# slyforce/MusicStyleTransfer

Measured on AMD Instinct MI355X. Metric: piano-roll frames/s (VAE train step), higher is better.
Workload: dtype bf16; 1 GPU; BASELINE configs[1]: single-track piano-roll VAE train step, T=256, pitch=128, latent=64, batch=64/GPU, bf16; encoder 256x2x8h, decoder 128x1x8h (scripts/train-vae.sh), dropout 0.2; Xavier-initialised weights; global_batch=64, seq_len=256, pitches=128, latent=64, parallelism=dp1, params=1885440

## Files before the change

### include/mst_hip.h

```cpp
#ifndef MST_HIP_H
#define MST_HIP_H

#include <stdint.h>

#ifdef __cplusplus
extern "C" {
#endif

typedef void* mst_stream_t;

enum mst_status {
  MST_OK = 0,
  MST_ERR_INVALID = -1,
  MST_ERR_LAUNCH = -2,
  MST_ERR_UNSUPPORTED = -3
};

enum mst_dtype { MST_BF16 = 0, MST_F16 = 1, MST_F32 = 2 };

enum mst_act { MST_ACT_NONE = 0, MST_ACT_RELU = 1 };

int mst_version(void);
const char* mst_last_error(void);

int mst_graph_begin(mst_stream_t stream);
int mst_graph_end(mst_stream_t stream, void** graph_exec_out);
int mst_graph_end_counted(mst_stream_t stream, void** graph_exec_out, int32_t* nodes_out, int32_t* kernel_nodes_out);
int mst_graph_launch(void* graph_exec, mst_stream_t stream);
int mst_graph_destroy(void* graph_exec);

int mst_event_create(void** ev_out);
int mst_event_record(void* ev, mst_stream_t stream);
int mst_event_sync(void* ev);
int mst_event_elapsed_ms(void* ev_start, void* ev_stop, float* ms_out);
int mst_event_destroy(void* ev);

typedef struct mst_gemm_args {
  int32_t dtype;
  int32_t c_f32;
  int64_t M, N, K;
  const void* A; int64_t lda;
  const void* B; int64_t ldb;
  void* C; int64_t ldc;
  const float* bias;
  const void* resid; int64_t ldr;
  int32_t act;
  const void* gate; int64_t ldg;
  float alpha;
  const float* rowadd; int64_t ldra; int64_t rowadd_period;
  const float* grpadd; int64_t ldga; const int32_t* grp_index;
  int64_t a_rows_per_group, a_group_stride, a_group_offset;
  int64_t c_rows_per_group, c_group_stride, c_group_offset;
  float dropout_p; uint64_t dropout_seed; uint32_t dropout_site;
  int32_t self_resid;
  const uint64_t* dropout_seed_ptr;
  int32_t a_u8;
  int32_t resid_phys;
} mst_gemm_args;

int mst_gemm_nt(const mst_gemm_args* args, mst_stream_t stream);
int mst_gemm_nt_form(const mst_gemm_args* args);

int mst_gemm_nt_pair(const mst_gemm_args* args0, const mst_gemm_args* args1, mst_stream_t stream);

typedef struct mst_bce_args {
  const uint8_t* labels;
  int64_t T;
  float label_smoothing;
  int32_t downweight;
  float* loss;
  void* probs; int64_t ldp;
  void* logits; int64_t ldl;
  float gscale;
  uint64_t* counts;
} mst_bce_args;
#define MST_ROLL_SLOTS 256
int mst_gemm_sigmoid_bce(const mst_gemm_args* args, const mst_bce_args* bce, mst_stream_t stream);

typedef struct mst_ln_args {
  int32_t mode;
  const float* gamma;
  const float* beta;
  float eps;
  void* out; int64_t ld_out;
  float* mean; float* rstd;
  const void* x; int64_t ld_x;
  float* dgamma; float* dbeta;
  int32_t mask_mode;
  float* partials;
} mst_ln_args;

int mst_gemm_nt_ln(const mst_gemm_args* args, const mst_ln_args* ln, mst_stream_t stream);
int mst_gemm_sigmoid_bce_dgrad_ln(const mst_gemm_args* args, const mst_bce_args* bce, const mst_gemm_args* dgrad,
                                  const mst_ln_args* ln, mst_stream_t stream);
int64_t mst_gemm_nt_ln_parts(int64_t M);
int mst_gemm_sigmoid_bce_form(const mst_gemm_args* args, const mst_bce_args* bce, const mst_gemm_args* dgrad, const mst_ln_args* ln,
                              int64_t* form);

int mst_ffn_ln_fwd(const mst_gemm_args* ff1, const mst_gemm_args* ff2, const mst_ln_args* ln, mst_stream_t stream);
int mst_ffn_ln_bwd(const mst_gemm_args* ff2_dgrad, const mst_gemm_args* ff1_dgrad, const mst_ln_args* ln, mst_stream_t stream);
typedef struct mst_ln_bwd_in {
  const void* dy; int64_t ld_dy;
  const void* x;  int64_t ld_x;
  const float* gamma; const float* mean; const float* rstd;
  void* dx; int64_t ld_dx;
  void* dx_masked; int64_t ld_dxm;
  float* dgamma; float* dbeta; float* partials;
  int32_t mask_mode;
  float dropout_p; uint64_t dropout_seed; const uint64_t* dropout_seed_ptr; uint32_t dropout_site;
} mst_ln_bwd_in;
int mst_ffn_ln_bwd_lead(const mst_ln_bwd_in* lead, const mst_gemm_args* ff2_dgrad, const mst_gemm_args* ff1_dgrad,
                        const mst_ln_args* ln, mst_stream_t stream);
int mst_kqv_ffn_ln_bwd(const mst_gemm_args* kqv_dgrad, const mst_ln_bwd_in* lead, const mst_gemm_args* ff2_dgrad,
                       const mst_gemm_args* ff1_dgrad, const mst_ln_args* ln, mst_stream_t stream);
int mst_kqv_ffn_ln_bwd_form(const mst_gemm_args* kqv_dgrad, const mst_gemm_args* ff2_dgrad, const mst_gemm_args* ff1_dgrad,
                            int64_t* form);
int mst_proj_ffn_ln_fwd(const mst_gemm_args* proj, const mst_ln_args* ln1, const mst_gemm_args* ff1, const mst_gemm_args* ff2,
                        const mst_ln_args* ln2, mst_stream_t stream);
int mst_dec_tail_step(const mst_gemm_args* proj, const mst_ln_args* ln1, const mst_gemm_args* ff1, const mst_gemm_args* ff2,
                      const mst_ln_args* ln3, const mst_gemm_args* out, const mst_bce_args* bce, const mst_gemm_args* out_dgrad,
                      const mst_ln_args* ln3_bwd, const mst_gemm_args* ff2_dgrad, const mst_gemm_args* ff1_dgrad,
                      const mst_ln_args* ln1_bwd, mst_stream_t stream);

typedef struct mst_partial_sum {
  const float* src; int64_t n_parts; int64_t stride; int64_t len;
  float* dst; float scale;
} mst_partial_sum;
int mst_partial_sums(const mst_partial_sum* jobs, int n, mst_stream_t stream);

typedef struct mst_wgrad_args {
  int32_t dtype;
  int64_t M, N, K;
  const void* A; int64_t lda;
  const void* B; int64_t ldb;
  float* dW; int64_t ldw;
  float* db;
  float scale;
  int64_t a_rows_per_group, a_group_stride, a_group_offset;
  int64_t b_rows_per_group, b_group_stride, b_group_offset;
  int32_t a_u8;
} mst_wgrad_args;

typedef struct mst_outer_job {
  const float* L; const void* R; int32_t r_dtype; int64_t r_stride;
  int64_t B, J, I;
  float* out; float* obias;
} mst_outer_job;
int mst_outer_jobs(const mst_outer_job* jobs, int n, mst_stream_t stream);
int mst_gemm_wgrad_batch_flush(const mst_wgrad_args* list, int n, float* scratch, int64_t scratch_bytes,
                               const mst_partial_sum* sums, int n_sums, const mst_outer_job* outers, int n_outers,
                               mst_stream_t stream);
int mst_class_table_grad(const int32_t* classes, const float* tvec, float* dcls, int64_t ld_cls, int64_t B, int64_t Dd,
                         mst_stream_t stream);
int mst_gemm_wgrad_batch_flush_cls(const mst_wgrad_args* list, int n, float* scratch, int64_t scratch_bytes,
                                   const mst_partial_sum* sums, int n_sums, const mst_outer_job* outers, int n_outers,
                                   const int32_t* cls_classes, const float* cls_tvec, float* cls_dcls, int64_t cls_ld,
                                   int64_t cls_B, int64_t cls_Dd, mst_stream_t stream);
int mst_gemm_wgrad_plan(const mst_wgrad_args* list, int n, int64_t scratch_bytes, int64_t* plan);

int mst_embed_fwd(int dtype, int64_t B, int64_t T, int64_t D,
                  const int32_t* tokens, const float* table, int64_t ldt,
                  const int32_t* classes, const float* cls_table, int64_t ldc,
// ... 310 lines not shown
```

### musicstyletransfer_amd/csrc/common.hpp

```cpp
#pragma once
#include <hip/hip_runtime.h>
#include <stdint.h>
#include <stdio.h>
#include "../../include/mst_hip.h"

namespace mst {

void set_error(const char* fmt, ...);

#define MST_CHECK_ARG(cond, ...)                 \
  do {                                           \
    if (!(cond)) {                               \
      ::mst::set_error(__VA_ARGS__);             \
      return MST_ERR_INVALID;                    \
    }                                            \
  } while (0)

#define MST_CHECK_LAUNCH(what)                                                   \
  do {                                                                           \
    hipError_t e__ = hipGetLastError();                                          \
    if (e__ != hipSuccess) {                                                     \
      ::mst::set_error("%s: %s", what, hipGetErrorString(e__));                  \
      return MST_ERR_LAUNCH;                                                     \
    }                                                                            \
  } while (0)

static inline int lds_opt_in(const void* fn, size_t lds, size_t* granted, const char* what) {
  if (lds <= *granted) return MST_OK;
  const hipError_t e = hipFuncSetAttribute(fn, hipFuncAttributeMaxDynamicSharedMemorySize, (int)lds);
  if (e != hipSuccess) { set_error("%s: LDS opt-in of %zu bytes: %s", what, lds, hipGetErrorString(e)); return MST_ERR_LAUNCH; }
  *granted = lds;
  return MST_OK;
}

static inline int64_t cdiv(int64_t a, int64_t b) { return (a + b - 1) / b; }
static inline int64_t roundup(int64_t a, int64_t b) { return cdiv(a, b) * b; }

constexpr int WAVE = 64;

typedef __attribute__((ext_vector_type(4))) float f32x4;
typedef __attribute__((ext_vector_type(16))) float f32x16;
typedef __attribute__((ext_vector_type(8))) __bf16 bf16x8;
typedef __attribute__((ext_vector_type(4))) __bf16 bf16x4;
typedef __attribute__((ext_vector_type(8))) _Float16 f16x8;
typedef __attribute__((ext_vector_type(4))) _Float16 f16x4;
typedef __attribute__((ext_vector_type(4))) short i16x4;
typedef __attribute__((ext_vector_type(8))) short i16x8;
typedef __attribute__((ext_vector_type(4))) uint32_t u32x4;
typedef __attribute__((ext_vector_type(2))) uint32_t u32x2;

template <typename T> struct Act;
template <> struct Act<__bf16> {
  typedef bf16x8 vec8;
  typedef bf16x4 vec4;
  static __device__ __forceinline__ f32x4 mfma16(vec8 a, vec8 b, f32x4 c) {
    return __builtin_amdgcn_mfma_f32_16x16x32_bf16(a, b, c, 0, 0, 0);
  }
  static __device__ __forceinline__ f32x16 mfma32(vec8 a, vec8 b, f32x16 c) {
    return __builtin_amdgcn_mfma_f32_32x32x16_bf16(a, b, c, 0, 0, 0);
  }
};
template <> struct Act<_Float16> {
  typedef f16x8 vec8;
  typedef f16x4 vec4;
  static __device__ __forceinline__ f32x4 mfma16(vec8 a, vec8 b, f32x4 c) {
    return __builtin_amdgcn_mfma_f32_16x16x32_f16(a, b, c, 0, 0, 0);
  }
  static __device__ __forceinline__ f32x16 mfma32(vec8 a, vec8 b, f32x16 c) {
    return __builtin_amdgcn_mfma_f32_32x32x16_f16(a, b, c, 0, 0, 0);
  }
};

template <typename T> __device__ __forceinline__ float to_f32(T x) { return (float)x; }
template <typename T> __device__ __forceinline__ T from_f32(float x) { return (T)x; }

union Pack8 {
  u32x4 u;
  uint16_t h[8];
};

template <typename T> __device__ __forceinline__ float bits_to_f32(uint16_t b) {
  T t;
  __builtin_memcpy(&t, &b, 2);
  return (float)t;
}
template <typename T> __device__ __forceinline__ uint16_t f32_to_bits(float f) {
  T t = (T)f;
  uint16_t b;
  __builtin_memcpy(&b, &t, 2);
  return b;
}

template <typename T> __device__ __forceinline__ u32x4 expand_u8x8(u32x2 raw) {
  Pack8 p;
#pragma unroll
  for (int e = 0; e < 8; ++e) p.h[e] = f32_to_bits<T>((float)((raw[e >> 2] >> (8 * (e & 3))) & 0xFFu));
  return p.u;
}

template <int CTRL> __device__ __forceinline__ float dpp_mov(float v) {
  return __builtin_bit_cast(float, __builtin_amdgcn_update_dpp(0, __builtin_bit_cast(int, v), CTRL, 0xF, 0xF, true));
}
__device__ __forceinline__ float lane_xor16(float v) {
  return __builtin_bit_cast(float, __builtin_amdgcn_ds_swizzle(__builtin_bit_cast(int, v), 0x401F));
}
template <int LANES> __device__ __forceinline__ float group_sum(float v) {
  static_assert(LANES == 4 || LANES == 8 || LANES == 16 || LANES == 32 || LANES == 64, "group size");
  v += dpp_mov<0xB1>(v);
  v += dpp_mov<0x4E>(v);
  if constexpr (LANES >= 8) v += dpp_mov<0x141>(v);
  if constexpr (LANES >= 16) v += dpp_mov<0x140>(v);
  if constexpr (LANES >= 32) v += lane_xor16(v);
  if constexpr (LANES >= 64) v += __shfl_xor(v, 32, 64);
  return v;
}
template <int LANES> __device__ __forceinline__ float group_max(float v) {
  v = fmaxf(v, dpp_mov<0xB1>(v));
  v = fmaxf(v, dpp_mov<0x4E>(v));
  if constexpr (LANES >= 8) v = fmaxf(v, dpp_mov<0x141>(v));
  if constexpr (LANES >= 16) v = fmaxf(v, dpp_mov<0x140>(v));
  if constexpr (LANES >= 32) v = fmaxf(v, lane_xor16(v));
  if constexpr (LANES >= 64) v = fmaxf(v, __shfl_xor(v, 32, 64));
  return v;
}
__device__ __forceinline__ float wave_sum(float v) { return group_sum<64>(v); }
__device__ __forceinline__ float wave_max(float v) { return group_max<64>(v); }

__device__ __forceinline__ int64_t xcd_chunk(int64_t bid, int64_t n) {
  const int64_t q = n / 8, r = n % 8, x = bid % 8, y = bid / 8;
  return (x < r ? x * (q + 1) : r * (q + 1) + (x - r) * q) + y;
}

__device__ __forceinline__ int64_t remap_row(int64_t m, int64_t rpg, int64_t stride, int64_t off) {
  return rpg > 0 ? (m / rpg) * stride + off + (m % rpg) : m;
}

__host__ __device__ __forceinline__ uint32_t dropout_hash(uint64_t seed, uint32_t site, uint64_t idx) {
  uint64_t x = seed ^ (0x9E3779B97F4A7C15ull * (uint64_t)(site + 1)) ^ (idx * 0xD1B54A32D192ED03ull);
  x ^= x >> 32; x *= 0xD6E8FEB86659FD93ull;
  x ^= x >> 32; x *= 0xD6E8FEB86659FD93ull;
  x ^= x >> 32;
  return (uint32_t)x;
}
__host__ __device__ __forceinline__ uint32_t dropout_thr(float p) { return (uint32_t)(p * 65536.0f); }
__host__ __device__ __forceinline__ float dropout_inv_keep(float p) {
// ... 75 lines not shown
```

### musicstyletransfer_amd/csrc/dec_tail.hip

```cpp
#include "ffn_ln.hpp"
#include "gemm_bce.hpp"
#include "gemm_checks.hpp"

namespace mst {

template <typename T>
__device__ __forceinline__ void tile128_load_w(const mst_gemm_args& g, u32x4 (&rw)[2][2]) {
  const T* __restrict__ W = reinterpret_cast<const T*>(g.B);
#pragma unroll
  for (int s = 0; s < 2; ++s)
#pragma unroll
    for (int i = 0; i < 2; ++i) {
      const int c = threadIdx.x + i * 512, row = c / 8, ch = c % 8;
      rw[s][i] = *reinterpret_cast<const u32x4*>(W + (int64_t)row * g.ldb + s * 64 + ch * 8);
    }
}
template <typename T>
__device__ __forceinline__ void tile128_gemm(unsigned char* smem, const T* sA, const u32x4 (&rw)[2][2], f32x4 (&acc)[2][2]) {
  constexpr int BN = 128, LDA = BN + 8, CHUNKS = 8, WTM = 32, WTN = 32, TM = 2, TN = 2, WGN = 4;
  typedef typename Act<T>::vec8 vec8;
  u32x4* sB = reinterpret_cast<u32x4*>(smem);
  const int tid = threadIdx.x, lane = tid & 63, wave = tid >> 6;
  const int wm = wave / WGN, wn = wave % WGN, frow = lane & 15, fq = lane >> 4;
#pragma unroll
  for (int s = 0; s < 2; ++s)
#pragma unroll
    for (int i = 0; i < 2; ++i) {
      const int c = tid + i * 512, row = c / CHUNKS, ch = c % CHUNKS;
      sB[s * BN * CHUNKS + row * CHUNKS + (ch ^ (row & 7))] = rw[s][i];
    }
#pragma unroll
  for (int j = 0; j < TN; ++j)
#pragma unroll
    for (int i = 0; i < TM; ++i) acc[j][i] = f32x4{0.f, 0.f, 0.f, 0.f};
  __syncthreads();
#pragma unroll
  for (int s = 0; s < 2; ++s) {
    const u32x4* cB = sB + s * BN * CHUNKS;
#pragma unroll
    for (int ks = 0; ks < 2; ++ks) {
      vec8 xf[TM], wf[TN];
      const int kc = ks * 4 + fq;
#pragma unroll
      for (int i = 0; i < TM; ++i)
        xf[i] = __builtin_bit_cast(vec8, *reinterpret_cast<const u32x4*>(sA + (wm * WTM + i * 16 + frow) * LDA + s * 64 + kc * 8));
#pragma unroll
      for (int j = 0; j < TN; ++j) {
        const int row = wn * WTN + j * 16 + frow;
        wf[j] = __builtin_bit_cast(vec8, cB[row * CHUNKS + (kc ^ (row & 7))]);
      }
#pragma unroll
      for (int j = 0; j < TN; ++j)
#pragma unroll
        for (int i = 0; i < TM; ++i) acc[j][i] = Act<T>::mfma16(wf[j], xf[i], acc[j][i]);
    }
  }
  __syncthreads();
}

constexpr size_t DEC_TAIL_F = 512;
constexpr size_t DEC_TAIL_BODY_LDS = (size_t)2 * 128 * 64 * 2 + (size_t)2 * 64 * (128 + 8) * 2 + DEC_TAIL_F * 4 + (size_t)6 * 128 * 4;
constexpr size_t DEC_TAIL_LDS = DEC_TAIL_BODY_LDS + ((size_t)128 + 3 * 128 + DEC_TAIL_F + 3 * 128) * 4;
static_assert(DEC_TAIL_LDS <= (size_t)48 * 1024 + (size_t)2 * (64 + 128) * 64 * 2 + (size_t)3 * 128 * 4, "no more LDS than the loss launch takes");

template <typename T, bool CNT>
__global__ __launch_bounds__(512) void dec_tail_kernel(mst_gemm_args proj, mst_ln_args ln1, mst_gemm_args ff1, mst_gemm_args ff2, mst_ln_args ln3,
                                                       mst_gemm_args out, mst_bce_args bce, mst_gemm_args odg, mst_ln_args ln3b,
                                                       mst_gemm_args f2d, mst_gemm_args f1d, mst_ln_args ln1b) {
  constexpr int BM = 64, BN = 128, WGM = 2, WGN = 4, LDA = BN + 8, F = (int)DEC_TAIL_F;
  extern __shared__ __attribute__((aligned(16))) unsigned char smem[];
  __shared__ __attribute__((aligned(16))) float red[bce_red_words(CNT)];
  T* sX = reinterpret_cast<T*>(smem + (size_t)2 * BN * 64 * 2 + (size_t)BM * LDA * 2);
  float* sBiasO = reinterpret_cast<float*>(smem + DEC_TAIL_BODY_LDS);
  float* sPar3 = sBiasO + BN;
  float* sPar4 = sPar3 + 3 * BN;
  const int tid = threadIdx.x;
  for (int i = tid; i < BN; i += 512) {
    sBiasO[i] = out.bias ? out.bias[i] : 0.f;
    sPar3[i] = odg.bias ? odg.bias[i] : 0.f;
    sPar3[BN + i] = ln3b.gamma[i];
    sPar3[2 * BN + i] = 0.f;
    sPar4[F + i] = f1d.bias ? f1d.bias[i] : 0.f;
    sPar4[F + BN + i] = ln1b.gamma[i];
    sPar4[F + 2 * BN + i] = 0.f;
  }
  for (int i = tid; i < F; i += 512) sPar4[i] = f2d.bias ? f2d.bias[i] : 0.f;
  const int64_t m0 = xcd_chunk(blockIdx.x, gridDim.x) * BM;
  const mst_ln_bwd_in no_lead = {};
  u32x4 rw[2][2];
  f32x4 acc[2][2];
  ffn_ln_body<T, BN, WGM, WGN, 1, false, true, true, false, true, false>(smem, ff1, ff2, ln3, no_lead, proj, ln1, nullptr,
                                                                         [&] { tile128_load_w<T>(out, rw); });
  __syncthreads();
  tile128_gemm<T>(smem, sX, rw, acc);
  tile128_load_w<T>(odg, rw);
  {
    float bias8[8];
#pragma unroll
    for (int e = 0; e < 8; ++e) bias8[e] = sBiasO[(tid % (BN / 8)) * 8 + e];
    bce_tile_finish<T, BN, 2, CNT>(out, bce, smem, red, reinterpret_cast<u32x4*>(sX), acc, m0, 0, bias8);
  }
  __syncthreads();
  tile128_gemm<T>(smem, sX, rw, acc);
  gemm_epilogue_ln<T, BM, BN, WGM, WGN, 2>(odg, ln3b, smem, acc, m0, nullptr, 0, sX, LDA, sPar3);
  __syncthreads();
  mst_gemm_args no_gemm = {};
  const mst_ln_args no_ln = {};
  ffn_ln_body<T, BN, WGM, WGN, 2, false, true, false, true, false, true>(smem, f2d, f1d, ln1b, no_lead, no_gemm, no_ln, sPar4, [] {});
}

template <typename T, bool CNT>
static int launch_dec_tail(const mst_gemm_args& proj, const mst_ln_args& ln1, const mst_gemm_args& ff1, const mst_gemm_args& ff2,
                           const mst_ln_args& ln3, const mst_gemm_args& out, const mst_bce_args& bce, const mst_gemm_args& odg,
                           const mst_ln_args& ln3b, const mst_gemm_args& f2d, const mst_gemm_args& f1d, const mst_ln_args& ln1b, hipStream_t s) {
  static size_t granted = 64 * 1024;
  if (const int rc = lds_opt_in(reinterpret_cast<const void*>(&dec_tail_kernel<T, CNT>), DEC_TAIL_LDS, &granted, "dec_tail_kernel")) return rc;
  hipLaunchKernelGGL((dec_tail_kernel<T, CNT>), dim3((unsigned)(out.M / 64)), dim3(512), DEC_TAIL_LDS, s, proj, ln1, ff1, ff2, ln3, out, bce, odg,
                     ln3b, f2d, f1d, ln1b);
  MST_CHECK_LAUNCH("dec_tail_kernel");
  return MST_OK;
}

}

using namespace mst;

extern "C" int mst_dec_tail_step(const mst_gemm_args* proj, const mst_ln_args* ln1, const mst_gemm_args* ff1, const mst_gemm_args* ff2,
                                 const mst_ln_args* ln3, const mst_gemm_args* out, const mst_bce_args* bce, const mst_gemm_args* out_dgrad,
                                 const mst_ln_args* ln3_bwd, const mst_gemm_args* ff2_dgrad, const mst_gemm_args* ff1_dgrad,
                                 const mst_ln_args* ln1_bwd, mst_stream_t stream) {
  const char* who = "mst_dec_tail_step";
  MST_CHECK_ARG(proj && ln1 && ff1 && ff2 && ln3 && out && bce && out_dgrad && ln3_bwd && ff2_dgrad && ff1_dgrad && ln1_bwd, "%s: null args", who);
  const mst_gemm_args &o = *out, &g = *out_dgrad, &d2 = *ff2_dgrad;
  const int64_t T = bce->T;
  MST_CHECK_ARG(ff2->N == 128 && ff1->K == 128 && proj->N == 128 && g.N == 128 && ff1_dgrad->N == 128,
                "%s: the model width must be 128 (got %lld)", who, (long long)ff2->N);
  MST_CHECK_ARG(ff1->N == 512 && d2.N == 512, "%s: the hidden width must be 512 (got %lld)", who, (long long)ff1->N);
  MST_CHECK_ARG(o.N == 128 && o.K == 128 && g.K == 128, "%s: the output layer must have 128 pitches (got %lld)", who, (long long)o.N);
  MST_CHECK_ARG(T > 0 && T % 64 == 0, "%s: T must be a multiple of 64 (got %lld)", who, (long long)T);
  MST_CHECK_ARG(o.M > 0 && o.M % 64 == 0 && o.M % T == 0 && ff1->M == o.M && ff2->M == o.M && proj->M == o.M && g.M == o.M && d2.M == o.M &&
                ff1_dgrad->M == o.M, "%s: every part works on the same whole 64-row tiles (M %lld)", who, (long long)o.M);
  auto groups = [&](int64_t rpg, int64_t stride, int64_t off) { return rpg == T && stride == T + 1 && off == 1; };
  MST_CHECK_ARG(groups(ff1->a_rows_per_group, ff1->a_group_stride, ff1->a_group_offset) &&
                groups(o.a_rows_per_group, o.a_group_stride, o.a_group_offset) &&
                groups(g.c_rows_per_group, g.c_group_stride, g.c_group_offset) &&
                groups(d2.a_rows_per_group, d2.a_group_stride, d2.a_group_offset) && g.a_rows_per_group <= 0,
                "%s: row groups must be (T, T + 1, 1) on all three parts", who);
  MST_CHECK_ARG(ln3_bwd->mode == 2 && ln3_bwd->mask_mode == 2, "%s: the LayerNorm-3 backward takes mask mode 2 (got %d)", who, (int)ln3_bwd->mask_mode);
  MST_CHECK_ARG(o.A == ln3->out && o.lda == ln3->ld_out, "%s: the output layer's A operand must be LayerNorm-3's output", who);
  MST_CHECK_ARG(o.C && g.A == o.C && g.lda == o.ldc, "%s: the output dgrad's A operand must be the logit gradient", who);
  MST_CHECK_ARG(d2.A == g.C && d2.lda == g.ldc, "%s: the A operand of the FF2 dgrad must be the output dgrad's dX_out", who);
  MST_CHECK_ARG(proj->dtype == o.dtype && g.dtype == o.dtype && d2.dtype == o.dtype && ff1->dtype == o.dtype && !g.a_u8,
                "%s: every part must share one activation dtype", who);
  int rc = check_ffn_ln(who, ff1, ff2, ln3, 1, nullptr, proj, ln1);
  if (rc == MST_OK) rc = check_gemm_bce(o, *bce);
  if (rc == MST_OK) rc = check_gemm_ln(g, *ln3_bwd);
  if (rc == MST_OK) rc = check_ffn_ln(who, ff2_dgrad, ff1_dgrad, ln1_bwd, 2);
  if (rc) return rc;
  hipStream_t s = (hipStream_t)stream;
  return dispatch_act(o.dtype, [&](auto tag) -> int {
    typedef decltype(tag) T_;
    if (bce->counts) return launch_dec_tail<T_, true>(*proj, *ln1, *ff1, *ff2, *ln3, o, *bce, g, *ln3_bwd, d2, *ff1_dgrad, *ln1_bwd, s);
    return launch_dec_tail<T_, false>(*proj, *ln1, *ff1, *ff2, *ln3, o, *bce, g, *ln3_bwd, d2, *ff1_dgrad, *ln1_bwd, s);
  });
}
```

### musicstyletransfer_amd/csrc/ffn_ln.hip

```cpp
#include "ffn_ln.hpp"
#include "gemm_checks.hpp"

namespace mst {

template <typename T, int BN, int WGM, int WGN, int MODE, bool LEAD, bool FULL, bool EXTRA = false>
__global__ __launch_bounds__(WGM * WGN * 64) void ffn_ln_kernel(mst_gemm_args g1, mst_gemm_args g2, mst_ln_args ln, mst_ln_bwd_in lead,
                                                                mst_gemm_args gx, mst_ln_args lnx) {
  extern __shared__ __attribute__((aligned(16))) unsigned char smem[];
  ffn_ln_body<T, BN, WGM, WGN, MODE, LEAD, FULL, EXTRA>(smem, g1, g2, ln, lead, gx, lnx, nullptr, [] {});
}

template <typename T, int BN>
static int launch_ffn_ln(const mst_gemm_args& g1, const mst_gemm_args& g2, const mst_ln_args& ln, const mst_ln_bwd_in* lead, hipStream_t s,
                         const mst_gemm_args* gx = nullptr, const mst_ln_args* lnx = nullptr) {
  constexpr int BM = 64;
  const int ex = gx ? 1 : 0;
  const size_t lds_loop = (size_t)2 * BN * 64 * 2 + (size_t)2 * BM * (BN + 8) * 2 + (size_t)g1.N * 4 + (size_t)6 * BN * 4;
  const size_t lds_epi = (size_t)BM * (BN + 4) * 4;
  const size_t lds = lds_loop > lds_epi ? lds_loop : lds_epi;
  const int full = g1.M % BM == 0 ? 1 : 0;
  const int mi = ex ? (ln.mode == 2 ? 8 : 6) + full : (lead ? 2 : (ln.mode == 2 ? 1 : 0)) * 2 + full;
  typedef void (*kern_t)(mst_gemm_args, mst_gemm_args, mst_ln_args, mst_ln_bwd_in, mst_gemm_args, mst_ln_args);
  const kern_t fns[10] = {&ffn_ln_kernel<T, BN, 2, 4, 1, false, false>, &ffn_ln_kernel<T, BN, 2, 4, 1, false, true>,
                         &ffn_ln_kernel<T, BN, 2, 4, 2, false, false>, &ffn_ln_kernel<T, BN, 2, 4, 2, false, true>,
                         &ffn_ln_kernel<T, BN, 2, 4, 2, true, false>, &ffn_ln_kernel<T, BN, 2, 4, 2, true, true>,
                         &ffn_ln_kernel<T, BN, 2, 4, 1, false, false, true>, &ffn_ln_kernel<T, BN, 2, 4, 1, false, true, true>,
                          &ffn_ln_kernel<T, BN, 2, 4, 2, true, false, true>, &ffn_ln_kernel<T, BN, 2, 4, 2, true, true, true>};
  static size_t granted[10] = {64 * 1024, 64 * 1024, 64 * 1024, 64 * 1024, 64 * 1024, 64 * 1024, 64 * 1024, 64 * 1024, 64 * 1024, 64 * 1024};
  if (const int rc = lds_opt_in(reinterpret_cast<const void*>(fns[mi]), lds, &granted[mi], "ffn_ln_kernel")) return rc;
  const mst_ln_bwd_in none = {};
  const mst_gemm_args no_gemm = {};
  const mst_ln_args no_ln = {};
  hipLaunchKernelGGL(fns[mi], dim3((unsigned)cdiv(g1.M, BM)), dim3(512), lds, s, g1, g2, ln, lead ? *lead : none,
                     gx ? *gx : no_gemm, lnx ? *lnx : no_ln);
  MST_CHECK_LAUNCH("ffn_ln_kernel");
  return MST_OK;
}

int check_ffn_ln(const char* who, const mst_gemm_args* first, const mst_gemm_args* second, const mst_ln_args* ln, int mode,
                 const mst_ln_bwd_in* lead, const mst_gemm_args* extra, const mst_ln_args* extra_ln) {
  MST_CHECK_ARG(first != nullptr && second != nullptr && ln != nullptr, "%s: null args", who);
  const mst_gemm_args& a = *first;
  const mst_gemm_args& b = *second;
  const mst_ln_args& l = *ln;
  int rc = check_gemm_common(a);
  if (rc) return rc;
  rc = check_gemm_common(b);
  if (rc) return rc;
  MST_CHECK_ARG(a.dtype == b.dtype && a.M == b.M, "%s: the two GEMMs must share dtype and M", who);
  MST_CHECK_ARG((b.N == 256 || b.N == 128) && a.K == b.N, "%s: the model width (first K = second N) must be 128 or 256 (got %lld, %lld)", who,
                (long long)a.K, (long long)b.N);
  MST_CHECK_ARG(a.N == b.K && a.N % b.N == 0, "%s: the hidden width (first N = second K) must be a multiple of the model width", who);
  MST_CHECK_ARG(b.A == a.C && b.lda == a.ldc, "%s: the second GEMM's A operand must be the first one's output (it is consumed on chip)", who);
  MST_CHECK_ARG(!a.c_f32 && !b.c_f32 && !b.gate && !a.rowadd && !b.rowadd && !a.grpadd && !b.grpadd && !a.resid && !a.self_resid &&
                b.act == MST_ACT_NONE && a.c_rows_per_group <= 0 && b.a_rows_per_group <= 0 && b.c_rows_per_group <= 0,
                "%s: fp32 outputs, row-indexed adds, row remaps, a gate or activation on the second GEMM and a residual on the first are not supported", who);
  MST_CHECK_ARG(a.a_rows_per_group <= 0 || (a.a_rows_per_group % 64 == 0 && a.M % a.a_rows_per_group == 0 && a.a_group_offset >= 0 &&
                                            a.a_group_stride >= a.a_rows_per_group + a.a_group_offset && a.M < (1ll << 31)),
                "%s: row groups must be whole 64-row tiles (rows per group %lld, stride %lld, offset %lld, M %lld)", who,
                (long long)a.a_rows_per_group, (long long)a.a_group_stride, (long long)a.a_group_offset, (long long)a.M);
  MST_CHECK_ARG(a.lda % 8 == 0 && a.ldc % 8 == 0 && a.ldc >= a.N && b.ldc % 8 == 0 && b.ldc >= b.N, "%s: leading dimensions must be multiples of 8", who);
  MST_CHECK_ARG((uint64_t)a.N * (uint64_t)a.ldb < (1ull << 32) && (uint64_t)b.N * (uint64_t)b.ldb < (1ull << 32), "%s: weight matrices too large", who);
  MST_CHECK_ARG(!b.resid || (b.ldr % 8 == 0 && b.ldr >= b.N && (uintptr_t)b.resid % 16 == 0), "%s: bad residual layout", who);
  MST_CHECK_ARG(!a.bias || (uintptr_t)a.bias % 16 == 0, "%s: the first GEMM's bias must be 16-byte aligned", who);
  MST_CHECK_ARG(a.dropout_p == 0.f || a.N % 4 == 0, "%s: dropout needs widths that are multiples of 4", who);
  MST_CHECK_ARG(l.mode == mode && l.gamma && l.mean && l.rstd, "%s: LayerNorm arguments of the wrong form", who);
  if (mode == 1) {
    MST_CHECK_ARG(!a.gate, "%s: a gate belongs to the backward form", who);
    MST_CHECK_ARG(l.beta && l.out && l.ld_out % 8 == 0 && l.ld_out >= b.N && (uintptr_t)l.out % 16 == 0,
                  "%s: the LayerNorm arguments are those of mst_gemm_nt_ln's forward form", who);
  } else {
    MST_CHECK_ARG(a.gate && a.ldg % 8 == 0 && a.ldg >= a.N && (uintptr_t)a.gate % 16 == 0, "%s: the first GEMM needs the forward activation as its gate", who);
    MST_CHECK_ARG(a.act == MST_ACT_NONE && a.dropout_p == 0.f && !b.self_resid, "%s: activation / dropout / self_resid belong to the forward form", who);
    MST_CHECK_ARG(l.x && l.ld_x % 8 == 0 && (uintptr_t)l.x % 16 == 0 && (l.partials || (l.dgamma && l.dbeta)) && (uintptr_t)l.partials % 16 == 0,
                  "%s: backward needs x and dgamma + dbeta (or partials)", who);
    MST_CHECK_ARG(l.mask_mode >= 0 && l.mask_mode <= 2 &&
                  (l.mask_mode != 1 || (l.out && l.ld_out % 8 == 0 && l.ld_out >= b.N && (uintptr_t)l.out % 16 == 0)),
                  "%s: mask_mode must be 0, 1 (with out) or 2", who);
  }
  if (lead) {
    const mst_ln_bwd_in& q = *lead;
    MST_CHECK_ARG(mode == 2, "%s: a leading LayerNorm belongs to the backward form", who);
    const bool dy_on_chip = extra != nullptr;
    MST_CHECK_ARG((q.dy || dy_on_chip) && q.x && q.gamma && q.mean && q.rstd && q.dx && (q.partials || (q.dgamma && q.dbeta)),
                  "%s: leading LayerNorm: null pointer", who);
    MST_CHECK_ARG((dy_on_chip || (q.ld_dy % 8 == 0 && q.ld_dy >= b.N)) && q.ld_x % 8 == 0 && q.ld_dx % 8 == 0 && q.ld_x >= b.N && q.ld_dx >= b.N &&
                  ((uintptr_t)q.dy | (uintptr_t)q.x | (uintptr_t)q.dx | (uintptr_t)q.partials) % 16 == 0, "%s: leading LayerNorm: bad layout", who);
    MST_CHECK_ARG(q.mask_mode == 0 || (q.mask_mode == 1 && q.dx_masked && q.ld_dxm % 8 == 0 && q.ld_dxm >= b.N && (uintptr_t)q.dx_masked % 16 == 0),
                  "%s: leading LayerNorm: mask_mode must be 0 or 1 (with dx_masked)", who);
    MST_CHECK_ARG(q.dropout_p >= 0.f && q.dropout_p < 1.f, "%s: leading LayerNorm: dropout_p must be in [0,1)", who);
    const void* tile = q.mask_mode == 1 ? q.dx_masked : q.dx;
    const int64_t tile_ld = q.mask_mode == 1 ? q.ld_dxm : q.ld_dx;
    MST_CHECK_ARG(a.A == tile && a.lda == tile_ld, "%s: the first GEMM's A operand must be the leading LayerNorm's (masked) output", who);
  }
  if (extra && mode == 2) {
  } else if (extra) {
    const mst_gemm_args& x = *extra;
    rc = check_gemm_common(x);
    if (rc) return rc;
    MST_CHECK_ARG(x.dtype == a.dtype && x.M == a.M && x.N == b.N && x.K == b.N, "%s: the extra GEMM is width x width on the same rows", who);
    MST_CHECK_ARG(!x.c_f32 && !x.gate && !x.rowadd && !x.grpadd && x.act == MST_ACT_NONE && x.a_rows_per_group <= 0 && x.c_rows_per_group <= 0 &&
                  x.ldc % 8 == 0 && x.ldc >= x.N && (uint64_t)x.N * (uint64_t)x.ldb < (1ull << 32),
                  "%s: the extra GEMM takes no gate, activation, row-indexed add or row remap", who);
    MST_CHECK_ARG(mode == 1 && extra_ln != nullptr, "%s: the projection (with its LayerNorm) rides in front of the forward form", who);
    const mst_ln_args& q = *extra_ln;
    MST_CHECK_ARG(q.mode == 1 && q.gamma && q.beta && q.mean && q.rstd && q.out == a.A && q.ld_out == a.lda,
                  "%s: the leading LayerNorm's output must be the first GEMM's A operand", who);
    MST_CHECK_ARG(!x.resid || (x.ldr % 8 == 0 && x.ldr >= x.N && (uintptr_t)x.resid % 16 == 0), "%s: bad residual layout", who);
  }
  return MST_OK;
}

}

using namespace mst;

static int ffn_ln_impl(const char* who, const mst_gemm_args* first, const mst_gemm_args* second, const mst_ln_args* ln, int mode,
                       mst_stream_t stream, const mst_ln_bwd_in* lead = nullptr, const mst_gemm_args* extra = nullptr,
                       const mst_ln_args* extra_ln = nullptr) {
  const int rc = check_ffn_ln(who, first, second, ln, mode, lead, extra, extra_ln);
  if (rc) return rc;
  const mst_gemm_args &a = *first, &b = *second;
  const mst_ln_args& l = *ln;
  hipStream_t s = (hipStream_t)stream;
  return dispatch_act(a.dtype, [&](auto tag) -> int {
    typedef decltype(tag) T;
    if (b.N == 256) return launch_ffn_ln<T, 256>(a, b, l, lead, s, extra, extra_ln);
    return launch_ffn_ln<T, 128>(a, b, l, lead, s, extra, extra_ln);
  });
}

extern "C" int mst_proj_ffn_ln_fwd(const mst_gemm_args* proj, const mst_ln_args* ln1, const mst_gemm_args* ff1, const mst_gemm_args* ff2,
                                   const mst_ln_args* ln2, mst_stream_t stream) {
  MST_CHECK_ARG(proj != nullptr && ln1 != nullptr, "mst_proj_ffn_ln_fwd: null args");
  return ffn_ln_impl("mst_proj_ffn_ln_fwd", ff1, ff2, ln2, 1, stream, nullptr, proj, ln1);
}

extern "C" int mst_ffn_ln_bwd_lead(const mst_ln_bwd_in* lead, const mst_gemm_args* ff2_dgrad, const mst_gemm_args* ff1_dgrad,
                                   const mst_ln_args* ln, mst_stream_t stream) {
  MST_CHECK_ARG(lead != nullptr, "mst_ffn_ln_bwd_lead: null args");
  return ffn_ln_impl("mst_ffn_ln_bwd_lead", ff2_dgrad, ff1_dgrad, ln, 2, stream, lead);
}

static int kqv_head_form(const mst_gemm_args& x, const mst_gemm_args& a, const mst_gemm_args& b) {
  const bool shape = (b.N == 256 || b.N == 128) && x.N == b.N && x.K == 3 * b.N && x.M == a.M && x.dtype == a.dtype;
  const bool plain = !x.c_f32 && !x.a_u8 && !x.bias && !x.gate && !x.rowadd && !x.grpadd && x.act == MST_ACT_NONE && x.alpha == 1.f &&
                     x.dropout_p == 0.f && !x.self_resid && x.a_rows_per_group <= 0 && x.c_rows_per_group <= 0 && a.a_rows_per_group <= 0;
  const bool layout = x.resid && ((uintptr_t)x.A | (uintptr_t)x.B | (uintptr_t)x.resid | (uintptr_t)x.C) % 16 == 0 && x.lda % 8 == 0 &&
                      x.lda >= x.K && x.ldb % 8 == 0 && x.ldb >= x.K && x.ldr % 8 == 0 && x.ldr >= x.N &&
                      (!x.C || (x.ldc % 8 == 0 && x.ldc >= x.N)) && (uint64_t)x.N * (uint64_t)x.ldb < (1ull << 32);
  return shape && plain && layout ? 1 : 0;
}

static int check_kqv_head_call(const char* who, const mst_gemm_args* head, const mst_gemm_args* ff2_dgrad, const mst_gemm_args* ff1_dgrad) {
  MST_CHECK_ARG(head != nullptr && ff2_dgrad != nullptr && ff1_dgrad != nullptr, "%s: null args", who);
  MST_CHECK_ARG(head->M > 0 && head->N > 0 && head->K > 0, "%s: the head's M,N,K must be positive (got %lld,%lld,%lld)", who,
                (long long)head->M, (long long)head->N, (long long)head->K);
  MST_CHECK_ARG(head->A && head->B, "%s: the head's A and B operands are missing", who);
  MST_CHECK_ARG(head->M == ff2_dgrad->M && head->N == ff1_dgrad->N, "%s: the head's result is the block's incoming gradient: M x width (got %lld x %lld)",
                who, (long long)head->M, (long long)head->N);
  return MST_OK;
}

extern "C" int mst_kqv_ffn_ln_bwd_form(const mst_gemm_args* kqv_dgrad, const mst_gemm_args* ff2_dgrad, const mst_gemm_args* ff1_dgrad,
                                       int64_t* form) {
  MST_CHECK_ARG(form != nullptr, "mst_kqv_ffn_ln_bwd_form: null form");
  if (const int rc = check_kqv_head_call("mst_kqv_ffn_ln_bwd_form", kqv_dgrad, ff2_dgrad, ff1_dgrad)) return rc;
  form[0] = kqv_head_form(*kqv_dgrad, *ff2_dgrad, *ff1_dgrad);
  return MST_OK;
}

extern "C" int mst_kqv_ffn_ln_bwd(const mst_gemm_args* kqv_dgrad, const mst_ln_bwd_in* lead, const mst_gemm_args* ff2_dgrad,
                                  const mst_gemm_args* ff1_dgrad, const mst_ln_args* ln, mst_stream_t stream) {
  if (const int rc = check_kqv_head_call("mst_kqv_ffn_ln_bwd", kqv_dgrad, ff2_dgrad, ff1_dgrad)) return rc;
  MST_CHECK_ARG(lead != nullptr, "mst_kqv_ffn_ln_bwd: null args");
  MST_CHECK_ARG(lead->dy == kqv_dgrad->C && (!lead->dy || lead->ld_dy == kqv_dgrad->ldc),
                "mst_kqv_ffn_ln_bwd: lead->dy is the head's C (both NULL: the gradient is not stored)");
  if (kqv_head_form(*kqv_dgrad, *ff2_dgrad, *ff1_dgrad))
    return ffn_ln_impl("mst_kqv_ffn_ln_bwd", ff2_dgrad, ff1_dgrad, ln, 2, stream, lead, kqv_dgrad);
  MST_CHECK_ARG(kqv_dgrad->C != nullptr, "mst_kqv_ffn_ln_bwd: this shape runs the GEMM launch first and needs the head's C");
  if (const int rc = check_ffn_ln("mst_kqv_ffn_ln_bwd", ff2_dgrad, ff1_dgrad, ln, 2, lead)) return rc;
  if (const int f = mst_gemm_nt_form(kqv_dgrad); f < 0) return f;
  if (const int rc = mst_gemm_nt(kqv_dgrad, stream)) return rc;
  return ffn_ln_impl("mst_kqv_ffn_ln_bwd", ff2_dgrad, ff1_dgrad, ln, 2, stream, lead);
}

extern "C" int mst_ffn_ln_fwd(const mst_gemm_args* ff1, const mst_gemm_args* ff2, const mst_ln_args* ln, mst_stream_t stream) {
  return ffn_ln_impl("mst_ffn_ln_fwd", ff1, ff2, ln, 1, stream);
}
extern "C" int mst_ffn_ln_bwd(const mst_gemm_args* ff2_dgrad, const mst_gemm_args* ff1_dgrad, const mst_ln_args* ln, mst_stream_t stream) {
  return ffn_ln_impl("mst_ffn_ln_bwd", ff2_dgrad, ff1_dgrad, ln, 2, stream);
}

#ifdef MST_FFN_STAMPS
extern "C" int mst_debug_ffn_stamps(uint64_t* host_out) {
  return hipMemcpyFromSymbol(host_out, HIP_SYMBOL(mst::g_ffn_stamps), sizeof(uint64_t) * (8 + 48 * 4)) == hipSuccess ? 0 : -1;
}
#endif
```

### musicstyletransfer_amd/csrc/ffn_ln.hpp

```cpp
#pragma once
#include <type_traits>
#include "gemm_ln.hpp"

namespace mst {

template <typename T, int BN, int WGM, int WGN, int MODE, bool LEAD, bool FULL, bool EXTRA, bool X_IN_LDS = false, bool KEEP_OUT = false,
          bool PAR_READY = false, typename Hook>
__device__ __forceinline__ void ffn_ln_body(unsigned char* smem, mst_gemm_args g1, mst_gemm_args g2, const mst_ln_args ln,
                                            const mst_ln_bwd_in lead, mst_gemm_args gx, const mst_ln_args lnx, float* par,
                                            Hook&& before_epilogue) {
  constexpr bool HEAD = EXTRA, FHEAD = EXTRA && MODE == 1, BHEAD = EXTRA && MODE == 2;
  static_assert(!(X_IN_LDS && (LEAD || EXTRA)), "a tile left in LDS is the block's own input");
  static_assert(!BHEAD || LEAD, "the backward form's head computes the gradient tile of the leading LayerNorm backward");
  constexpr int BM = 64, BK = 64, CHUNKS = BK / 8;
  constexpr int NT = WGM * WGN * 64;
  constexpr int WTM = BM / WGM, WTN = BN / WGN, TM = WTM / 16, TN = WTN / 16;
  constexpr int B_CH = BN * CHUNKS / NT;
  constexpr int LDA = BN + 8;
  constexpr int KST = BN / BK;
  constexpr int XST = BHEAD ? 3 * KST : KST;
  static_assert(BN * CHUNKS % NT == 0 && (BM * BN / 8) % NT == 0, "tile/threads mismatch");
  typedef typename Act<T>::vec8 vec8;
  u32x4* sB = reinterpret_cast<u32x4*>(smem);
  T* sH = reinterpret_cast<T*>(smem + (size_t)2 * BN * BK * 2);
  T* sX = sH + BM * LDA;
  float* sBias1 = PAR_READY ? par : reinterpret_cast<float*>(sX + BM * LDA);
  float* sPar = sBias1 + g1.N;
  const int tid = threadIdx.x, lane = tid & 63, wave = tid >> 6;
  const int wm = wave / WGN, wn = wave % WGN, frow = lane & 15, fq = lane >> 4;
  int64_t m0 = xcd_chunk(blockIdx.x, gridDim.x) * BM;
  if (g1.a_rows_per_group > 0) {
    const uint32_t grp = (uint32_t)m0 / (uint32_t)g1.a_rows_per_group;
    m0 += (int64_t)grp * (g1.a_group_stride - g1.a_rows_per_group) + g1.a_group_offset;
    g1.M = g2.M = gx.M = (g1.M / g1.a_rows_per_group) * g1.a_group_stride;
  }
  const int64_t F = g1.N;
  FFN_STAMP(0); FFN_RT(190);
  const int64_t Mg = FULL ? (int64_t)1 << 62 : g1.M;
  if constexpr (!PAR_READY)
  for (int i = tid * 4; i < (int)F; i += NT * 4)
    *reinterpret_cast<f32x4*>(sBias1 + i) = g1.bias ? *reinterpret_cast<const f32x4*>(g1.bias + i) : f32x4{0.f, 0.f, 0.f, 0.f};
  const uint64_t seed2 = g2.dropout_seed ^ ((g2.dropout_p > 0.f && g2.dropout_seed_ptr) ? g2.dropout_seed_ptr[0] : 0ull);
  const uint64_t seedx = FHEAD ? gx.dropout_seed ^ ((gx.dropout_p > 0.f && gx.dropout_seed_ptr) ? gx.dropout_seed_ptr[0] : 0ull) : 0ull;
  if constexpr (!PAR_READY)
  for (int i = tid; i < BN; i += NT) {
    sPar[i] = g2.bias ? g2.bias[i] : 0.f;
    sPar[BN + i] = ln.gamma[i];
    sPar[2 * BN + i] = (MODE == 1) ? ln.beta[i] : 0.f;
    if constexpr (FHEAD) {
      sPar[3 * BN + i] = gx.bias ? gx.bias[i] : 0.f;
      sPar[4 * BN + i] = lnx.gamma[i];
      sPar[5 * BN + i] = lnx.beta[i];
    }
  }
  const int n_chunks = (int)(F / BN);
  const int rot = (int)((blockIdx.x / 8) % (unsigned)n_chunks);
  auto phys = [&](int c) { const int pc = c + rot; return pc >= n_chunks ? pc - n_chunks : pc; };
  const T* __restrict__ W1 = reinterpret_cast<const T*>(g1.B);
  const T* __restrict__ W2 = reinterpret_cast<const T*>(g2.B);
  const T* __restrict__ WX = reinterpret_cast<const T*>(gx.B);

  uint32_t off1[B_CH], off2[B_CH], offx[B_CH];
  int b_lds[B_CH];
#pragma unroll
  for (int i = 0; i < B_CH; ++i) {
    const int c = tid + i * NT;
    const int row = c / CHUNKS, ch = c % CHUNKS;
    off1[i] = (uint32_t)row * (uint32_t)g1.ldb + (uint32_t)ch * 8u;
    off2[i] = (uint32_t)row * (uint32_t)g2.ldb + (uint32_t)ch * 8u;
    offx[i] = EXTRA ? (uint32_t)row * (uint32_t)gx.ldb + (uint32_t)ch * 8u : 0u;
    b_lds[i] = row * CHUNKS + (ch ^ (row & 7));
  }
  constexpr int SPC = 2 * KST;
  constexpr int RING = BN >= 256 ? 4 : 2, AHEAD = RING - 1;
  static_assert(SPC % RING == 0, "ring slots must repeat per chunk");
  u32x4 ring[RING][B_CH];
  auto load_stage = [&](int c, int s, u32x4 (&rb)[B_CH]) {
    if (HEAD && c < 0) {
      const T* base = WX + s * BK;
#pragma unroll
      for (int i = 0; i < B_CH; ++i) rb[i] = *reinterpret_cast<const u32x4*>(base + offx[i]);
    } else if (s < KST) {
      const T* base = W1 + (int64_t)phys(c) * BN * g1.ldb + s * BK;
#pragma unroll
      for (int i = 0; i < B_CH; ++i) rb[i] = *reinterpret_cast<const u32x4*>(base + off1[i]);
    } else {
      const T* base = W2 + (int64_t)phys(c) * BN + (s - KST) * BK;
#pragma unroll
      for (int i = 0; i < B_CH; ++i) rb[i] = *reinterpret_cast<const u32x4*>(base + off2[i]);
    }
  };
  auto load_piece = [&](int c, int s, u32x4 (&rb)[B_CH], auto ic) {
    constexpr int i = decltype(ic)::value;
    const T* base;
    uint32_t off;
    if (HEAD && c < 0) { base = WX + s * BK; off = offx[i]; }
    else if (s < KST) { base = W1 + (int64_t)phys(c) * BN * g1.ldb + s * BK; off = off1[i]; }
    else { base = W2 + (int64_t)phys(c) * BN + (s - KST) * BK; off = off2[i]; }
    rb[i] = *reinterpret_cast<const u32x4*>(base + off);
  };
  auto store_stage = [&](int buf, const u32x4 (&rb)[B_CH]) {
#pragma unroll
    for (int i = 0; i < B_CH; ++i) sB[buf * BN * CHUNKS + b_lds[i]] = rb[i];
  };
  {
    auto pro = [&](auto jc) {
      constexpr int j = decltype(jc)::value;
      if constexpr (HEAD) {
        static_assert(!HEAD || AHEAD <= XST, "the head GEMM's stages cover the prologue");
        if (j < AHEAD) load_stage(-1, j, ring[j % RING]);
      } else {
        if (j < AHEAD && (j < SPC || n_chunks > 1)) load_stage(j / SPC, j % SPC, ring[j % RING]);
      }
    };
    pro(std::integral_constant<int, 0>()); pro(std::integral_constant<int, 1>()); pro(std::integral_constant<int, 2>());
    pro(std::integral_constant<int, 3>()); pro(std::integral_constant<int, 4>()); pro(std::integral_constant<int, 5>());
    pro(std::integral_constant<int, 6>());
    static_assert(AHEAD <= 7, "the prologue list covers seven stages");
  }
  constexpr int L_CPR = BN / 8, L_RSTEP = NT / L_CPR, L_ITERS = BM / L_RSTEP;
  const int lnc = (tid % L_CPR) * 8, lrow0 = tid / L_CPR;
  uint32_t ldkey = 0u, ldthr = 0u;
  float linv_keep = 1.f, gam8[8], dg8[8], db8[8];
  u32x4 dyv[L_ITERS], xv[L_ITERS];
  float mean_r[L_ITERS], rstd_r[L_ITERS];
  u32x4 ha2[L_ITERS], hres[L_ITERS];
  auto lead_loads = [&] {
    constexpr int RSTEP = L_RSTEP, ITERS = L_ITERS;
    const int nc = lnc, row0 = lrow0;
    const bool has_drop = lead.dropout_p > 0.f && lead.mask_mode == 1;
    const uint64_t dseed = lead.dropout_seed ^ ((has_drop && lead.dropout_seed_ptr) ? lead.dropout_seed_ptr[0] : 0ull);
    ldkey = dropout_key(dseed, lead.dropout_site); ldthr = dropout_thr(lead.dropout_p);
    linv_keep = dropout_inv_keep(lead.dropout_p);
#pragma unroll
    for (int e = 0; e < 8; ++e) { gam8[e] = lead.gamma[nc + e]; dg8[e] = 0.f; db8[e] = 0.f; }
#pragma unroll
    for (int it = 0; it < ITERS; ++it) {
      const int64_t m = m0 + row0 + it * RSTEP;
      dyv[it] = u32x4{0u, 0u, 0u, 0u}; xv[it] = dyv[it]; mean_r[it] = 0.f; rstd_r[it] = 0.f;
      if (m < Mg) {
        if constexpr (!BHEAD) dyv[it] = *reinterpret_cast<const u32x4*>(reinterpret_cast<const T*>(lead.dy) + m * lead.ld_dy + nc);
        xv[it] = *reinterpret_cast<const u32x4*>(reinterpret_cast<const T*>(lead.x) + m * lead.ld_x + nc);
        mean_r[it] = lead.mean[m];
        rstd_r[it] = lead.rstd[m];
      }
    }
  };
  auto lead_rows = [&] {
    constexpr int CPR = L_CPR, RSTEP = L_RSTEP, ITERS = L_ITERS;
    const int nc = lnc, row0 = lrow0;
    const float inv_n = 1.f / (float)BN;
    const bool has_drop = lead.dropout_p > 0.f && lead.mask_mode == 1;
    const uint32_t dkey = ldkey, dthr = ldthr;
    const float inv_keep = linv_keep;
    if constexpr (BHEAD) {
#pragma unroll
      for (int it = 0; it < ITERS; ++it) {
        const int row = row0 + it * RSTEP;
        const int64_t m = m0 + row;
        if (m < Mg) {
          dyv[it] = *reinterpret_cast<const u32x4*>(sX + row * LDA + nc);
          if (gx.C) *reinterpret_cast<u32x4*>(reinterpret_cast<T*>(gx.C) + m * gx.ldc + nc) = dyv[it];
        }
      }
    }
#pragma unroll
    for (int it = 0; it < ITERS; ++it) {
      const int row = row0 + it * RSTEP;
      const int64_t m = m0 + row;
      Pack8 db, xb;
      db.u = dyv[it]; xb.u = xv[it];
      float xh[8], g[8], s1 = 0.f, s2 = 0.f;
#pragma unroll
      for (int e = 0; e < 8; ++e) {
        const float d = bits_to_f32<T>(db.h[e]);
        xh[e] = (bits_to_f32<T>(xb.h[e]) - mean_r[it]) * rstd_r[it];
        g[e] = d * gam8[e];
        s1 += g[e];
        s2 += g[e] * xh[e];
        dg8[e] += d * xh[e];
        db8[e] += d;
      }
      s1 = row_sum<CPR>(s1) * inv_n;
      s2 = row_sum<CPR>(s2) * inv_n;
      uint32_t keep8 = 0xFFu;
      if (has_drop) {
        const uint64_t w = (uint64_t)(m * BN + nc) >> 2;
        keep8 = dropout_keep4k(dkey, w, dthr) | (dropout_keep4k(dkey, w + 1, dthr) << 4);
      }
      Pack8 ob, mb;
#pragma unroll
      for (int e = 0; e < 8; ++e) {
        const float o = rstd_r[it] * (g[e] - s1 - xh[e] * s2);
        const float k = has_drop ? (((keep8 >> e) & 1u) ? inv_keep : 0.f) : 1.f;
        ob.h[e] = f32_to_bits<T>(o);
        mb.h[e] = f32_to_bits<T>(o * k);
      }
      if (m < Mg) {
        *reinterpret_cast<u32x4*>(reinterpret_cast<T*>(lead.dx) + m * lead.ld_dx + nc) = ob.u;
        if (lead.mask_mode == 1) *reinterpret_cast<u32x4*>(reinterpret_cast<T*>(lead.dx_masked) + m * lead.ld_dxm + nc) = mb.u;
      }
      *reinterpret_cast<u32x4*>(sX + row * LDA + nc) = (m < Mg) ? (lead.mask_mode == 1 ? mb.u : ob.u) : u32x4{0u, 0u, 0u, 0u};
    }
    float* red = reinterpret_cast<float*>(smem);
    static_assert((size_t)2 * RSTEP * BN * 4 <= (size_t)2 * BN * BK * 2, "reduction scratch must fit the weight stages");
#pragma unroll
    for (int e = 0; e < 8; ++e) {
      red[row0 * BN + nc + e] = dg8[e];
      red[(RSTEP + row0) * BN + nc + e] = db8[e];
    }
    __syncthreads();
    for (int c = tid; c < 2 * BN; c += NT) {
      const int which = c / BN, col = c % BN;
      float sm = 0.f;
      for (int r = 0; r < RSTEP; ++r) sm += red[(which * RSTEP + r) * BN + col];
      if (lead.partials) lead.partials[(int64_t)blockIdx.x * 2 * BN + c] = sm;
      else atomicAdd((which ? lead.dbeta : lead.dgamma) + col, sm);
    }
    __syncthreads();
  };
  if constexpr (BHEAD) {
    constexpr int RSTEP = L_RSTEP, ITERS = L_ITERS;
    const T* HA = reinterpret_cast<const T*>(gx.A);
    const T* HR = reinterpret_cast<const T*>(gx.resid);
    u32x4 ha0[ITERS], ha1[ITERS];
#pragma unroll
    for (int it = 0; it < ITERS; ++it) {
      const int64_t m = m0 + lrow0 + it * RSTEP;
      ha0[it] = u32x4{0u, 0u, 0u, 0u}; ha1[it] = ha0[it]; ha2[it] = ha0[it]; hres[it] = ha0[it];
      if (m < Mg) {
        const T* ap = HA + m * gx.lda + lnc;
        ha0[it] = *reinterpret_cast<const u32x4*>(ap);
        ha1[it] = *reinterpret_cast<const u32x4*>(ap + BN);
        ha2[it] = *reinterpret_cast<const u32x4*>(ap + 2 * BN);
        hres[it] = *reinterpret_cast<const u32x4*>(HR + m * gx.ldr + lnc);
      }
    }
    lead_loads();
#pragma unroll
    for (int it = 0; it < ITERS; ++it) {
      const int row = lrow0 + it * RSTEP;
      *reinterpret_cast<u32x4*>(sX + row * LDA + lnc) = ha0[it];
      *reinterpret_cast<u32x4*>(sH + row * LDA + lnc) = ha1[it];
    }
  } else if constexpr (LEAD) {
    lead_loads();
    lead_rows();
  } else if constexpr (!X_IN_LDS)
  {
    const T* X = reinterpret_cast<const T*>(HEAD ? gx.A : g1.A);
    const int64_t ldx = HEAD ? gx.lda : g1.lda;
    constexpr int CPR = BN / 8;
// ... 66 lines not shown
        if constexpr (t < XST) load_stage(cx, t, ring[t % RING]);
        else if constexpr (HEAD) load_stage(0, t - XST, ring[t % RING]);
        mma_stage(acc1, (((s / KST) & 1) ? sH : sX) + (s % KST) * BK, s & 1, ring[s % RING], no_hook);
        if constexpr (s + 1 < XST) store_stage((s + 1) & 1, ring[(s + 1) % RING]);
        __syncthreads();
        if constexpr (BHEAD && (s == KST - 1 || s == 2 * KST - 1)) {
#pragma unroll
          for (int it = 0; it < L_ITERS; ++it)
            *reinterpret_cast<u32x4*>((s == KST - 1 ? sX : sH) + (lrow0 + it * L_RSTEP) * LDA + lnc) = s == KST - 1 ? ha2[it] : hres[it];
        }
      }
    };
    static_assert(!EXTRA || (XST <= 12 && XST % RING == 0 && XST % 2 == 0), "the extra GEMM stage list / ring slots");
    xstage(std::integral_constant<int, 0>()); xstage(std::integral_constant<int, 1>());
    xstage(std::integral_constant<int, 2>()); xstage(std::integral_constant<int, 3>());
    xstage(std::integral_constant<int, 4>()); xstage(std::integral_constant<int, 5>());
    xstage(std::integral_constant<int, 6>()); xstage(std::integral_constant<int, 7>());
    xstage(std::integral_constant<int, 8>()); xstage(std::integral_constant<int, 9>());
    xstage(std::integral_constant<int, 10>()); xstage(std::integral_constant<int, 11>());
  };
  if constexpr (BHEAD) {
    extra_gemm(-1);
#pragma unroll
    for (int j = 0; j < TN; ++j)
#pragma unroll
      for (int i = 0; i < TM; ++i) {
        const int row = wm * WTM + i * 16 + frow, n = wn * WTN + j * 16 + fq * 4;
        const u32x2 rb = *reinterpret_cast<const u32x2*>(sH + row * LDA + n);
        uint16_t hb[4];
#pragma unroll
        for (int e = 0; e < 4; ++e)
          hb[e] = f32_to_bits<T>(acc1[j][i][e] + bits_to_f32<T>((uint16_t)(rb[e >> 1] >> ((e & 1) * 16))));
        *reinterpret_cast<u32x2*>(sX + row * LDA + n) =
            u32x2{(uint32_t)hb[0] | ((uint32_t)hb[1] << 16), (uint32_t)hb[2] | ((uint32_t)hb[3] << 16)};
      }
    __syncthreads();
    lead_rows();
  }
  if constexpr (FHEAD) {
    extra_gemm(-1);
    gemm_epilogue_ln<T, BM, BN, WGM, WGN, 1>(gx, lnx, smem, acc1, m0, nullptr, 0, sX, LDA, sPar + 3 * BN, &seedx);
    __syncthreads();
  }
  store_stage(0, ring[0]);
  __syncthreads();
  FFN_STAMP(1);
  for (int c = 0; c < n_chunks; ++c) {
    const int pc = phys(c);
#pragma unroll
    for (int j = 0; j < TN; ++j)
#pragma unroll
      for (int i = 0; i < TM; ++i) acc1[j][i] = f32x4{0.f, 0.f, 0.f, 0.f};
    constexpr int OUT_CH = BM * (BN / 8) / NT;
    u32x4 gv[OUT_CH];
    if constexpr (MODE == 2) {
      const T* G = reinterpret_cast<const T*>(g1.gate);
#pragma unroll
      for (int i = 0; i < OUT_CH; ++i) {
        const int cc = tid + i * NT, row = cc / (BN / 8), ch = cc % (BN / 8);
        gv[i] = u32x4{0u, 0u, 0u, 0u};
        if (m0 + row < Mg) gv[i] = *reinterpret_cast<const u32x4*>(G + (m0 + row) * g1.ldg + (int64_t)pc * BN + ch * 8);
      }
    }
    auto stage = [&](auto sc) {
      constexpr int s = decltype(sc)::value;
      if constexpr (s < SPC) {
        constexpr bool IL = BN >= 256 && B_CH <= 2 * TN;
        constexpr int t = s + AHEAD;
        const int tc = t < SPC ? c : (c + 1 < n_chunks ? c + 1 : c);
        const bool more = s + 1 < SPC || c + 1 < n_chunks;
        auto piece = [&](auto kc) {
          constexpr int k = decltype(kc)::value;
          if constexpr (IL && k < B_CH) {
            __builtin_amdgcn_sched_barrier(0);
            load_piece(tc, t % SPC, ring[t % RING], kc);
            if (more) sB[((s + 1) & 1) * BN * CHUNKS + b_lds[k]] = ring[(s + 1) % RING][k];
            __builtin_amdgcn_sched_barrier(0);
          }
        };
        if constexpr (!IL) load_stage(tc, t % SPC, ring[t % RING]);
        FFN_STAMP(8 + (c * SPC + s) * 4);
        if constexpr (s < KST) mma_stage(acc1, sX + s * BK, s & 1, ring[s % RING], piece);
        else mma_stage(acc2, sH + (s - KST) * BK, s & 1, ring[s % RING], piece);
        FFN_STAMP(8 + (c * SPC + s) * 4 + 1);
        if constexpr (s == KST - 1) {
          auto chunk_epilogue = [&](auto step_form) {
            constexpr bool STEP = decltype(step_form)::value;
            const uint32_t cmul = ((uint32_t)pc * (BN / 2) + (uint32_t)((wn * WTN + fq * 4) / 2)) * DROPOUT_MUL;
#pragma unroll
            for (int j = 0; j < TN; ++j) {
              const int n = wn * WTN + j * 16 + fq * 4;
              const int64_t col = (int64_t)pc * BN + n;
              const f32x4 b4 = *reinterpret_cast<const f32x4*>(sBias1 + col);
#pragma unroll
              for (int i = 0; i < TM; ++i) {
                const int row = wm * WTM + i * 16 + frow;
                float tv[4];
                if constexpr (STEP) {
#pragma unroll
                  for (int e = 0; e < 4; ++e) tv[e] = fmaxf(acc1[j][i][e] + b4[e], 0.f);
                  dropout_apply4_pre(dkey1, rowmul[i] + cmul + (uint32_t)(j * 8) * DROPOUT_MUL, dthr1, inv_keep1, tv);
                } else {
#pragma unroll
                  for (int e = 0; e < 4; ++e) {
                    tv[e] = (acc1[j][i][e] + b4[e]) * g1.alpha;
                    if (relu1) tv[e] = fmaxf(tv[e], 0.f);
                  }
                  if (drop1) dropout_apply4(dkey1, (uint64_t)((m0 + row) * F + col) >> 2, dthr1, inv_keep1, tv);
                }
                uint16_t hb[4];
#pragma unroll
                for (int e = 0; e < 4; ++e) hb[e] = f32_to_bits<T>(tv[e]);
                *reinterpret_cast<u32x2*>(sH + row * LDA + n) =
                    u32x2{(uint32_t)hb[0] | ((uint32_t)hb[1] << 16), (uint32_t)hb[2] | ((uint32_t)hb[3] << 16)};
              }
            }
          };
          if (step_form1) chunk_epilogue(std::true_type()); else chunk_epilogue(std::false_type());
        }
        if (!IL && more) store_stage((s + 1) & 1, ring[(s + 1) % RING]);
        FFN_STAMP(8 + (c * SPC + s) * 4 + 2);
        __syncthreads();
        FFN_STAMP(8 + (c * SPC + s) * 4 + 3);
        if constexpr (s == KST - 1) {
          constexpr int CPR = BN / 8;
#pragma unroll
          for (int i = 0; i < BM * CPR / NT; ++i) {
            const int cc = tid + i * NT, row = cc / CPR, ch = cc % CPR;
            u32x4 v = *reinterpret_cast<const u32x4*>(sH + row * LDA + ch * 8);
            if constexpr (MODE == 2) {
              Pack8 pv, pg;
              pv.u = v; pg.u = gv[i];
#pragma unroll
              for (int e = 0; e < 8; ++e)
                if (!(bits_to_f32<T>(pg.h[e]) > 0.f)) pv.h[e] = 0;
              v = pv.u;
              *reinterpret_cast<u32x4*>(sH + row * LDA + ch * 8) = v;
            }
            if (m0 + row < Mg) *reinterpret_cast<u32x4*>(Aout + (m0 + row) * g1.ldc + (int64_t)pc * BN + ch * 8) = v;
          }
          if constexpr (MODE == 2) __syncthreads();
        }
      }
    };
    static_assert(SPC <= 8, "the stage list below covers eight stages per chunk");
    stage(std::integral_constant<int, 0>()); stage(std::integral_constant<int, 1>());
    stage(std::integral_constant<int, 2>()); stage(std::integral_constant<int, 3>());
    stage(std::integral_constant<int, 4>()); stage(std::integral_constant<int, 5>());
    stage(std::integral_constant<int, 6>()); stage(std::integral_constant<int, 7>());
  }
  const bool resid_is_x = g2.resid == g1.A && g2.ldr == g1.lda;
  FFN_STAMP(2);
  before_epilogue();
  gemm_epilogue_ln<T, BM, BN, WGM, WGN, MODE>(g2, ln, smem, acc2, m0, resid_is_x ? sX : nullptr, LDA, KEEP_OUT ? sX : nullptr, KEEP_OUT ? LDA : 0,
                                              sPar, &seed2);
  FFN_STAMP(3); FFN_RT(191);
}

}
```

### musicstyletransfer_amd/csrc/gemm_bce.hip

```cpp
#include "gemm_bce.hpp"
#include "gemm_ln.hpp"
#include "gemm_checks.hpp"

namespace mst {

template <typename T, int BN, bool CNT>
__global__ __launch_bounds__(512) void gemm_bce_kernel(mst_gemm_args a, mst_bce_args q) {
  extern __shared__ __attribute__((aligned(16))) unsigned char smem[];
  __shared__ __attribute__((aligned(16))) float red[bce_red_words(CNT)];
  gemm_bce_tile<T, BN, false, CNT>(a, q, smem, red, nullptr);
}

template <typename T, bool CNT>
__global__ __launch_bounds__(512) void gemm_bce_dgrad_ln_kernel(mst_gemm_args a, mst_bce_args q, mst_gemm_args g2, mst_ln_args l) {
  constexpr int BM = 64, BN = 128, WGM = 2, WGN = 4;
  constexpr size_t OFF2 = 48 * 1024, END2 = OFF2 + (size_t)2 * (BM + BN) * 64 * 2;
  extern __shared__ __attribute__((aligned(16))) unsigned char smem[];
  __shared__ __attribute__((aligned(16))) float red[bce_red_words(CNT)];
  float* sPar = reinterpret_cast<float*>(smem + END2);
  for (int i = threadIdx.x; i < BN; i += 512) {
    sPar[i] = g2.bias ? g2.bias[i] : 0.f;
    sPar[BN + i] = l.gamma[i];
    sPar[2 * BN + i] = 0.f;
  }
  gemm_bce_tile<T, BN, true, CNT>(a, q, smem, red, reinterpret_cast<u32x4*>(smem + OFF2));
  __syncthreads();
  f32x4 acc[(BN / WGN) / 16][(BM / WGM) / 16];
  int64_t m0, n0;
  gemm_mainloop<T, BM, BN, WGM, WGN, 64, true, false, true>(g2, smem + OFF2, acc, m0, n0);
  gemm_epilogue_ln<T, BM, BN, WGM, WGN, 2>(g2, l, smem, acc, m0, nullptr, 0, nullptr, 0, sPar);
}

template <typename T, bool CNT>
static int launch_gemm_bce_dgrad_ln(const mst_gemm_args& a, const mst_bce_args& q, const mst_gemm_args& g2, const mst_ln_args& l, hipStream_t s) {
  const size_t lds = (size_t)48 * 1024 + (size_t)2 * (64 + 128) * 64 * 2 + (size_t)3 * 128 * 4;
  static size_t granted = 64 * 1024;
  if (const int rc = lds_opt_in(reinterpret_cast<const void*>(&gemm_bce_dgrad_ln_kernel<T, CNT>), lds, &granted, "gemm_bce_dgrad_ln_kernel")) return rc;
  hipLaunchKernelGGL((gemm_bce_dgrad_ln_kernel<T, CNT>), dim3((unsigned)cdiv(a.M, 64)), dim3(512), lds, s, a, q, g2, l);
  MST_CHECK_LAUNCH("gemm_bce_dgrad_ln_kernel");
  return MST_OK;
}

template <typename T, int BN, bool CNT>
static int launch_gemm_bce(const mst_gemm_args& a, const mst_bce_args& q, hipStream_t s) {
  const size_t lds_loop = (size_t)2 * (64 + BN) * 64 * 2, lds_epi = (size_t)64 * (BN + 4) * 4;
  const size_t lds = lds_loop > lds_epi ? lds_loop : lds_epi;
  static size_t granted = 64 * 1024;
  if (const int rc = lds_opt_in(reinterpret_cast<const void*>(&gemm_bce_kernel<T, BN, CNT>), lds, &granted, "gemm_bce_kernel")) return rc;
  hipLaunchKernelGGL((gemm_bce_kernel<T, BN, CNT>), dim3((unsigned)(cdiv(a.M, 64) * (a.N / BN))), dim3(512), lds, s, a, q);
  MST_CHECK_LAUNCH("gemm_bce_kernel");
  return MST_OK;
}

int check_gemm_bce(const mst_gemm_args& a, const mst_bce_args& q) {
  MST_CHECK_ARG(a.M > 0 && a.K > 0 && a.K % 8 == 0 && a.lda % 8 == 0 && a.ldb % 8 == 0 && a.A && a.B,
                "mst_gemm_sigmoid_bce: bad GEMM operands");
  MST_CHECK_ARG(((uintptr_t)a.A % 16 == 0) && ((uintptr_t)a.B % 16 == 0), "mst_gemm_sigmoid_bce: operands must be 16-byte aligned");
  MST_CHECK_ARG(a.N == 128 || (a.N > 0 && a.N % 256 == 0), "mst_gemm_sigmoid_bce: the row of pitches must be 128 or a multiple of 256 wide (got %lld): use "
                "mst_gemm_nt + mst_sigmoid_bce for other widths", (long long)a.N);
  MST_CHECK_ARG(a.N <= 256 || !q.downweight, "mst_gemm_sigmoid_bce: the label down-weighting counts a sample's positives in every workgroup — rows wider than "
                "one tile (256) take mst_gemm_nt + mst_sigmoid_bce");
  MST_CHECK_ARG(q.T > 0 && q.T % 64 == 0 && a.M % q.T == 0, "mst_gemm_sigmoid_bce: T must be a multiple of 64 and divide M (a tile holds one sample's rows)");
  MST_CHECK_ARG(!a.c_f32 && !a.resid && !a.gate && !a.rowadd && !a.grpadd && a.act == MST_ACT_NONE && a.dropout_p == 0.f && !a.self_resid &&
                a.c_rows_per_group <= 0 && !a.a_u8, "mst_gemm_sigmoid_bce: only bias, alpha and an A row remap are supported");
  MST_CHECK_ARG(q.labels && q.loss && (uintptr_t)q.labels % 8 == 0, "mst_gemm_sigmoid_bce: labels / loss missing or labels not 8-byte aligned");
  MST_CHECK_ARG(!a.C || (a.ldc % 8 == 0 && a.ldc >= a.N && (uintptr_t)a.C % 16 == 0), "mst_gemm_sigmoid_bce: bad dlogits layout");
  MST_CHECK_ARG(!q.probs || (q.ldp % 8 == 0 && q.ldp >= a.N && (uintptr_t)q.probs % 16 == 0), "mst_gemm_sigmoid_bce: bad probs layout");
  MST_CHECK_ARG(!q.logits || (q.ldl % 8 == 0 && q.ldl >= a.N && (uintptr_t)q.logits % 16 == 0), "mst_gemm_sigmoid_bce: bad logits layout");
  MST_CHECK_ARG((uintptr_t)q.counts % 16 == 0, "mst_gemm_sigmoid_bce: counts must be 16-byte aligned");
  return MST_OK;
}

static bool bce_dgrad_ln_one_launch(const mst_gemm_args& a, const mst_gemm_args& g2, const mst_ln_args& l) {
  return a.N == 128 && g2.N == 128 && g2.K == 128 && g2.M == a.M && a.M % 64 == 0 && l.mode == 2 && a.C && g2.A == a.C &&
         g2.lda == a.ldc && g2.dtype == a.dtype && g2.a_rows_per_group <= 0 && !g2.a_u8;
}

}

using namespace mst;

extern "C" int mst_gemm_sigmoid_bce_form(const mst_gemm_args* args, const mst_bce_args* bce, const mst_gemm_args* dgrad,
                                         const mst_ln_args* ln, int64_t* form) {
  MST_CHECK_ARG(form != nullptr, "mst_gemm_sigmoid_bce_form: null form");
  const bool pair = dgrad != nullptr || ln != nullptr;
  if (pair) MST_CHECK_ARG(args != nullptr && bce != nullptr && dgrad != nullptr && ln != nullptr, "mst_gemm_sigmoid_bce_dgrad_ln: null args");
  else MST_CHECK_ARG(args != nullptr && bce != nullptr, "mst_gemm_sigmoid_bce: null args");
  int rc = check_gemm_bce(*args, *bce);
  if (rc == MST_OK && pair) rc = check_gemm_ln(*dgrad, *ln);
  if (rc) return rc;
  return dispatch_act(args->dtype, [&](auto) -> int {
    const int64_t BN = args->N % 256 == 0 ? 256 : 128;
    form[0] = BN;
    form[1] = args->N / BN;
    form[2] = !pair ? 0 : bce_dgrad_ln_one_launch(*args, *dgrad, *ln) ? 1 : 2;
    return MST_OK;
  });
}

extern "C" int mst_gemm_sigmoid_bce(const mst_gemm_args* args, const mst_bce_args* bce, mst_stream_t stream) {
  MST_CHECK_ARG(args != nullptr && bce != nullptr, "mst_gemm_sigmoid_bce: null args");
  const mst_gemm_args& a = *args;
  const mst_bce_args& q = *bce;
  int rc = check_gemm_bce(a, q);
  if (rc) return rc;
  hipStream_t s = (hipStream_t)stream;
  return dispatch_act(a.dtype, [&](auto tag) -> int {
    typedef decltype(tag) T;
    if (q.counts) return a.N % 256 == 0 ? launch_gemm_bce<T, 256, true>(a, q, s) : launch_gemm_bce<T, 128, true>(a, q, s);
    return a.N % 256 == 0 ? launch_gemm_bce<T, 256, false>(a, q, s) : launch_gemm_bce<T, 128, false>(a, q, s);
  });
}

extern "C" int mst_gemm_sigmoid_bce_dgrad_ln(const mst_gemm_args* args, const mst_bce_args* bce, const mst_gemm_args* dgrad,
                                             const mst_ln_args* ln, mst_stream_t stream) {
  MST_CHECK_ARG(args != nullptr && bce != nullptr && dgrad != nullptr && ln != nullptr, "mst_gemm_sigmoid_bce_dgrad_ln: null args");
// ... 17 lines not shown
```

### musicstyletransfer_amd/csrc/gemm_checks.hpp

```cpp
#pragma once
#include "common.hpp"

namespace mst {

int check_gemm_common(const mst_gemm_args& a);
int check_gemm_ln(const mst_gemm_args& a, const mst_ln_args& l);
int check_gemm_bce(const mst_gemm_args& a, const mst_bce_args& q);
int check_ffn_ln(const char* who, const mst_gemm_args* first, const mst_gemm_args* second, const mst_ln_args* ln, int mode,
                 const mst_ln_bwd_in* lead = nullptr, const mst_gemm_args* extra = nullptr, const mst_ln_args* extra_ln = nullptr);

}
```

### musicstyletransfer_amd/csrc/gemm_ln.hpp

```cpp
#pragma once
#include <math.h>
#include "common.hpp"
#include "gemm_tile.hpp"

namespace mst {

#ifdef MST_FFN_STAMPS
static __device__ uint64_t g_ffn_stamps[8 + 48 * 4];
#define FFN_STAMP(slot) do { if (blockIdx.x == 64 && threadIdx.x == 0 && (slot) < 8 + 48 * 4) g_ffn_stamps[slot] = __builtin_amdgcn_s_memtime(); } while (0)
#define FFN_RT(slot) do { if (blockIdx.x == 64 && threadIdx.x == 0) g_ffn_stamps[slot] = __builtin_amdgcn_s_memrealtime(); } while (0)
#else
#define FFN_STAMP(slot) do { } while (0)
#define FFN_RT(slot) do { } while (0)
#endif

template <int LANES>
__device__ __forceinline__ float row_sum(float v) { return group_sum<LANES>(v); }

template <typename T, int BM, int BN, int WGM, int WGN, int MODE>
__device__ __forceinline__ void gemm_epilogue_ln(const mst_gemm_args& a, const mst_ln_args& l, unsigned char* smem,
                                                 f32x4 (&acc)[(BN / WGN) / 16][(BM / WGM) / 16], int64_t m0,
                                                 const T* lds_resid = nullptr, int lds_resid_ld = 0,
                                                 T* lds_out = nullptr, int lds_out_ld = 0, const float* lds_par = nullptr,
                                                 const uint64_t* dseed_pre = nullptr ) {
  constexpr int NT = WGM * WGN * 64;
  constexpr int WTM = BM / WGM, WTN = BN / WGN;
  constexpr int TM = WTM / 16, TN = WTN / 16;
  constexpr int LDS_F = BN + 4, CPR = BN / 8, RSTEP = NT / CPR, ITERS = BM / RSTEP;
  static_assert(CPR == 32 || CPR == 16, "a row must be a 32- or 16-lane group");
  static_assert(BM % RSTEP == 0, "rows per thread must be whole");
  const int tid = threadIdx.x, lane = tid & 63, wave = tid >> 6;
  const int wm = wave / WGN, wn = wave % WGN;
  const int frow = lane & 15, fq = lane >> 4;
  float* sF = reinterpret_cast<float*>(smem);
#pragma unroll
  for (int i = 0; i < TM; ++i)
#pragma unroll
    for (int j = 0; j < TN; ++j)
      *reinterpret_cast<f32x4*>(sF + (wm * WTM + i * 16 + frow) * LDS_F + wn * WTN + j * 16 + fq * 4) = acc[j][i];
  __syncthreads();
  FFN_STAMP(5);

  const int ch = tid % CPR, nc = ch * 8, row0 = tid / CPR;
  const float inv_n = 1.f / (float)BN;
  const float inv_keep = dropout_inv_keep(a.dropout_p);
  const bool has_drop = a.dropout_p > 0.f;
  const uint64_t dseed = dseed_pre ? *dseed_pre : a.dropout_seed ^ ((has_drop && a.dropout_seed_ptr) ? a.dropout_seed_ptr[0] : 0ull);
  const uint32_t dkey = dropout_key(dseed, a.dropout_site), dthr = dropout_thr(a.dropout_p);
  const T* resid = reinterpret_cast<const T*>(a.resid);
  float bias8[8], gam8[8], bet8[8];
#pragma unroll
  for (int e = 0; e < 8; ++e) {
    if (lds_par) {
      bias8[e] = lds_par[nc + e];
      gam8[e] = lds_par[BN + nc + e];
      bet8[e] = (MODE == 1) ? lds_par[2 * BN + nc + e] : 0.f;
    } else {
      bias8[e] = a.bias ? a.bias[nc + e] : 0.f;
      gam8[e] = l.gamma[nc + e];
      bet8[e] = (MODE == 1) ? l.beta[nc + e] : 0.f;
    }
  }
  float dg8[8], db8[8];
#pragma unroll
  for (int e = 0; e < 8; ++e) { dg8[e] = 0.f; db8[e] = 0.f; }

  u32x4 rv[ITERS], xv[ITERS];
  float mean_r[ITERS], rstd_r[ITERS];
  const bool tile_remap = a.c_rows_per_group <= 0 || a.c_rows_per_group % BM == 0;
  const int64_t pm0 = remap_row(m0, a.c_rows_per_group, a.c_group_stride, a.c_group_offset);
  auto phys_row = [&](int64_t m) { return tile_remap ? pm0 + (m - m0) : remap_row(m, a.c_rows_per_group, a.c_group_stride, a.c_group_offset); };
#pragma unroll
  for (int it = 0; it < ITERS; ++it) {
    const int64_t m = m0 + row0 + it * RSTEP;
    rv[it] = u32x4{0u, 0u, 0u, 0u}; xv[it] = rv[it]; mean_r[it] = 0.f; rstd_r[it] = 0.f;
    if (m < a.M) {
      const int64_t pm = phys_row(m);
      if (lds_resid) rv[it] = *reinterpret_cast<const u32x4*>(lds_resid + (row0 + it * RSTEP) * lds_resid_ld + nc);
      else if (resid) rv[it] = *reinterpret_cast<const u32x4*>(resid + m * a.ldr + nc);
      if (MODE == 2) {
        xv[it] = *reinterpret_cast<const u32x4*>(reinterpret_cast<const T*>(l.x) + pm * l.ld_x + nc);
        mean_r[it] = l.mean[pm];
        rstd_r[it] = l.rstd[pm];
      }
    }
  }
  FFN_STAMP(6);
#pragma unroll
  for (int it = 0; it < ITERS; ++it) {
    const int row = row0 + it * RSTEP;
    const int64_t m = m0 + row;
    if (m < a.M) {
      const int64_t pm = phys_row(m);
      const f32x4 v0 = *reinterpret_cast<const f32x4*>(sF + row * LDS_F + nc);
      const f32x4 v1 = *reinterpret_cast<const f32x4*>(sF + row * LDS_F + nc + 4);
      float t[8] = {v0[0], v0[1], v0[2], v0[3], v1[0], v1[1], v1[2], v1[3]};
#pragma unroll
      for (int e = 0; e < 8; ++e) t[e] = (t[e] + bias8[e]) * a.alpha;
      if (MODE == 1 && (has_drop || a.self_resid)) {
        float u0[4] = {t[0], t[1], t[2], t[3]}, u1[4] = {t[4], t[5], t[6], t[7]};
        if (has_drop) {
          const uint64_t w = (uint64_t)(pm * a.N + nc) >> 2;
          dropout_apply4(dkey, w, dthr, inv_keep, u0);
          dropout_apply4(dkey, w + 1, dthr, inv_keep, u1);
        }
#pragma unroll
        for (int e = 0; e < 4; ++e) {
          t[e] = a.self_resid ? t[e] + u0[e] : u0[e];
          t[4 + e] = a.self_resid ? t[4 + e] + u1[e] : u1[e];
        }
      }
      if (resid || lds_resid) {
        Pack8 p8; p8.u = rv[it];
#pragma unroll
        for (int e = 0; e < 8; ++e) t[e] += bits_to_f32<T>(p8.h[e]);
      }
      Pack8 hb;
#pragma unroll
      for (int e = 0; e < 8; ++e) { hb.h[e] = f32_to_bits<T>(t[e]); t[e] = bits_to_f32<T>(hb.h[e]); }
      if (MODE == 1) {
        *reinterpret_cast<u32x4*>(reinterpret_cast<T*>(a.C) + pm * a.ldc + nc) = hb.u;
        float s = 0.f;
#pragma unroll
        for (int e = 0; e < 8; ++e) s += t[e];
        const float mean = row_sum<CPR>(s) * inv_n;
        float ss = 0.f;
#pragma unroll
        for (int e = 0; e < 8; ++e) { t[e] -= mean; ss += t[e] * t[e]; }
        const float rstd = 1.f / sqrtf(row_sum<CPR>(ss) * inv_n + l.eps);
        Pack8 yb;
#pragma unroll
        for (int e = 0; e < 8; ++e) yb.h[e] = f32_to_bits<T>(t[e] * rstd * gam8[e] + bet8[e]);
        *reinterpret_cast<u32x4*>(reinterpret_cast<T*>(l.out) + pm * l.ld_out + nc) = yb.u;
        if (lds_out) *reinterpret_cast<u32x4*>(lds_out + row * lds_out_ld + nc) = yb.u;
        if (ch == 0) { l.mean[pm] = mean; l.rstd[pm] = rstd; }
      } else {
        const int64_t rid = pm;
        const float mean = mean_r[it], rstd = rstd_r[it];
        Pack8 xb; xb.u = xv[it];
        float xh[8], g[8], s1 = 0.f, s2 = 0.f;
#pragma unroll
        for (int e = 0; e < 8; ++e) {
          xh[e] = (bits_to_f32<T>(xb.h[e]) - mean) * rstd;
          g[e] = t[e] * gam8[e];
          s1 += g[e];
          s2 += g[e] * xh[e];
          dg8[e] += t[e] * xh[e];
          db8[e] += t[e];
        }
        s1 = row_sum<CPR>(s1) * inv_n;
        s2 = row_sum<CPR>(s2) * inv_n;
        uint32_t keep8 = 0xFFu;
        if (l.mask_mode != 0 && has_drop) {
          const uint64_t w = (uint64_t)(rid * BN + nc) >> 2;
          keep8 = dropout_keep4k(dkey, w, dthr) | (dropout_keep4k(dkey, w + 1, dthr) << 4);
        }
        Pack8 ob, mb;
#pragma unroll
        for (int e = 0; e < 8; ++e) {
          float o = rstd * (g[e] - s1 - xh[e] * s2);
          float om = 0.f;
          if (l.mask_mode != 0) {
            const float k = has_drop ? (((keep8 >> e) & 1u) ? inv_keep : 0.f) : 1.f;
            if (l.mask_mode == 1) om = o * k; else o = o * (1.f + k);
          }
// ... 33 lines not shown
```

### musicstyletransfer_amd/csrc/gemm_nt.hip

```cpp
#include <math.h>
#include "common.hpp"
#include "gemm_tile.hpp"
#include "gemm_checks.hpp"
#include "step_begin.hpp"
#include "shadows.hpp"

namespace mst {

template <typename T, int BM, int BN, int WGM, int WGN, bool C_F32, int BK, bool ROWOPS, int PATH, bool DROP, bool AU8 = false>
__global__ __launch_bounds__(WGM * WGN * 64) void gemm_nt_kernel(mst_gemm_args a) {
  extern __shared__ __attribute__((aligned(16))) unsigned char smem[];
  f32x4 acc[(BN / WGN) / 16][(BM / WGM) / 16];
  int64_t m0, n0;
  float bias_pre[8];
  gemm_bias_preload<BM, BN>(a, bias_pre);
  gemm_mainloop<T, BM, BN, WGM, WGN, BK, ROWOPS, AU8, false, PATH == 1 || PATH == 4>(a, smem, acc, m0, n0);
  gemm_epilogue<T, BM, BN, WGM, WGN, C_F32, ROWOPS, PATH, DROP>(a, smem, acc, m0, n0, bias_pre);
}

template <typename T, int BM, int BN, int WGM, int WGN, int BK, int PATH>
__global__ __launch_bounds__(WGM * WGN * 64) void gemm_nt_pair_kernel(mst_gemm_args a0, mst_gemm_args a1, int tiles0, int tiles1, StepBegin sb,
                                                                       int n_begin) {
  extern __shared__ __attribute__((aligned(16))) unsigned char smem[];
  if ((int)blockIdx.x < n_begin) {
// ... 39 lines not shown
}

template <int BM, int BN>
static bool gemm_fast_form(const mst_gemm_args& a) {
  const bool rowops = a.rowadd || a.grpadd || a.a_rows_per_group > 0 || a.c_rows_per_group > 0;
  const int64_t phys_rows = a.c_rows_per_group > 0 ? (a.M / a.c_rows_per_group + 1) * a.c_group_stride + a.c_group_offset : a.M;
  return !a.c_f32 && a.M % BM == 0 && a.N % BN == 0 && a.ldc % 8 == 0 &&
         (a.c_rows_per_group <= 0 || a.c_rows_per_group % BM == 0) &&
         (uint64_t)phys_rows * (uint64_t)a.N < (1ull << 32) &&
         (!a.resid || (a.ldr % 8 == 0 && (uintptr_t)a.resid % 16 == 0)) &&
         (!a.gate || (a.ldg % 8 == 0 && (uintptr_t)a.gate % 16 == 0)) &&
         (!rowops || (a.rowadd_period % BM == 0 && (!a.rowadd || (a.ldra % 4 == 0 && (uintptr_t)a.rowadd % 16 == 0)) &&
                      (!a.grpadd || (a.ldga % 4 == 0 && (uintptr_t)a.grpadd % 16 == 0))));
}

template <int BM, int BN, int BK>
static int gemm_variant(const mst_gemm_args& a) {
  const bool rowops = a.rowadd || a.grpadd || a.a_rows_per_group > 0 || a.c_rows_per_group > 0;
  const bool fast = gemm_fast_form<BM, BN>(a) && a.K % BK == 0;
  const bool drop = a.dropout_p > 0.f || a.self_resid;
  return a.a_u8 ? (fast ? 8 : 9) : (a.c_f32 ? 3 : (fast ? (drop ? 1 : 0) : 2)) + (rowops ? 4 : 0);
}

static int gemm_nt_form(const mst_gemm_args& a) {
  const int64_t big_tiles = cdiv(a.M, 128) * cdiv(a.N, 128);
  const int64_t last_round = big_tiles % 512;
  const bool stub_round = big_tiles > 512 && last_round > 0 && last_round < 128;
  const bool ragged128 = a.M % 128 != 0 && a.M % 64 == 0 && a.N % 128 == 0 && !a.c_f32;
  if (big_tiles > 512 && big_tiles <= 768 && a.N >= 128 && !ragged128 && gemm_3cu_form(a)) return 3 * 16;
  if (big_tiles >= 384 && a.N >= 128 && !stub_round && !ragged128) return 2 * 16 + gemm_variant<128, 128, 64>(a);
  if (a.M <= 64 && a.K >= 512 && a.K % 256 == 0) return 1 * 16 + gemm_variant<64, 64, 256>(a);
  return gemm_variant<64, 64, 64>(a);
}

template <typename T, int BM, int BN, int WGM, int WGN, int BK = 64>
static int launch_gemm(const mst_gemm_args& a, int variant, hipStream_t s) {
  const int64_t tiles = cdiv(a.M, BM) * cdiv(a.N, BN);
  const size_t lds_loop = (size_t)2 * (BM + BN) * BK * 2, lds_epi = (size_t)BM * (BN + 4) * 4;
  const size_t lds = lds_loop > lds_epi ? lds_loop : lds_epi;
  dim3 grid((unsigned)tiles), block(WGM * WGN * 64);
  typedef void (*kern_t)(mst_gemm_args);
  const kern_t fns[10] = {&gemm_nt_kernel<T, BM, BN, WGM, WGN, false, BK, false, 1, false>, &gemm_nt_kernel<T, BM, BN, WGM, WGN, false, BK, false, 1, true>,
                         &gemm_nt_kernel<T, BM, BN, WGM, WGN, false, BK, false, 2, true>, &gemm_nt_kernel<T, BM, BN, WGM, WGN, true, BK, false, 2, true>,
                         &gemm_nt_kernel<T, BM, BN, WGM, WGN, false, BK, true, 1, false>, &gemm_nt_kernel<T, BM, BN, WGM, WGN, false, BK, true, 1, true>,
                         &gemm_nt_kernel<T, BM, BN, WGM, WGN, false, BK, true, 2, true>, &gemm_nt_kernel<T, BM, BN, WGM, WGN, true, BK, true, 2, true>,
                         &gemm_nt_kernel<T, BM, BN, WGM, WGN, false, BK, true, 1, false, true>, &gemm_nt_kernel<T, BM, BN, WGM, WGN, false, BK, true, 2, false, true>};
  static size_t granted[10] = {64 * 1024, 64 * 1024, 64 * 1024, 64 * 1024, 64 * 1024, 64 * 1024, 64 * 1024, 64 * 1024, 64 * 1024, 64 * 1024};
  if (const int rc = lds_opt_in(reinterpret_cast<const void*>(fns[variant]), lds, &granted[variant], "gemm_nt_kernel")) return rc;
  hipLaunchKernelGGL(fns[variant], grid, block, lds, s, a);
  MST_CHECK_LAUNCH("gemm_nt_kernel");
  return MST_OK;
}

int check_gemm_common(const mst_gemm_args& a) {
  MST_CHECK_ARG(a.M > 0 && a.N > 0 && a.K > 0, "mst_gemm_nt: M,N,K must be positive (got %lld,%lld,%lld)",
                (long long)a.M, (long long)a.N, (long long)a.K);
  MST_CHECK_ARG(a.K % 8 == 0 && a.lda % 8 == 0 && a.ldb % 8 == 0,
                "mst_gemm_nt: K, lda, ldb must be multiples of 8 (got %lld,%lld,%lld)", (long long)a.K,
                (long long)a.lda, (long long)a.ldb);
  MST_CHECK_ARG(a.A && a.B && a.C, "mst_gemm_nt: null operand");
  MST_CHECK_ARG(a.dropout_p >= 0.f && a.dropout_p < 1.f, "mst_gemm_nt: dropout_p must be in [0,1)");
  MST_CHECK_ARG(((uintptr_t)a.A % 16 == 0) && ((uintptr_t)a.B % 16 == 0) && ((uintptr_t)a.C % 16 == 0),
                "mst_gemm_nt: operands must be 16-byte aligned");
  return MST_OK;
}

}

using namespace mst;

static int check_gemm_nt(const mst_gemm_args* args) {
  MST_CHECK_ARG(args != nullptr, "mst_gemm_nt: null args");
  const mst_gemm_args& a = *args;
  MST_CHECK_ARG(a.M > 0 && a.N > 0 && a.K > 0, "mst_gemm_nt: M,N,K must be positive (got %lld,%lld,%lld)",
                (long long)a.M, (long long)a.N, (long long)a.K);
  MST_CHECK_ARG(a.K % 8 == 0 && a.lda % 8 == 0 && a.ldb % 8 == 0,
                "mst_gemm_nt: K, lda, ldb must be multiples of 8 (got %lld,%lld,%lld)", (long long)a.K,
                (long long)a.lda, (long long)a.ldb);
  MST_CHECK_ARG(a.ldc % 4 == 0 && a.ldc >= a.N, "mst_gemm_nt: ldc must be a multiple of 4 and >= N");
  MST_CHECK_ARG(a.A && a.B && a.C, "mst_gemm_nt: null operand");
  MST_CHECK_ARG(!a.resid || (a.ldr % 4 == 0 && a.ldr >= a.N), "mst_gemm_nt: ldr must be a multiple of 4 and >= N");
  MST_CHECK_ARG(!a.gate || (a.ldg % 4 == 0 && a.ldg >= a.N), "mst_gemm_nt: ldg must be a multiple of 4 and >= N");
  MST_CHECK_ARG((!a.rowadd && !a.grpadd) || a.rowadd_period > 0, "mst_gemm_nt: rowadd_period must be > 0");
  MST_CHECK_ARG(!a.grpadd || a.grp_index, "mst_gemm_nt: grpadd needs grp_index");
  MST_CHECK_ARG(a.dropout_p >= 0.f && a.dropout_p < 1.f, "mst_gemm_nt: dropout_p must be in [0,1)");
  MST_CHECK_ARG(a.dropout_p == 0.f || a.N % 4 == 0, "mst_gemm_nt: dropout needs N to be a multiple of 4");
  MST_CHECK_ARG(((uintptr_t)a.A % 16 == 0) && ((uintptr_t)a.B % 16 == 0) && ((uintptr_t)a.C % 16 == 0),
                "mst_gemm_nt: operands must be 16-byte aligned");
  MST_CHECK_ARG(!a.a_u8 || (!a.c_f32 && a.dropout_p == 0.f && !a.self_resid),
                "mst_gemm_nt: a uint8 A operand comes with a 16-bit C and without dropout / self_resid");
  if (a.dtype != MST_BF16 && a.dtype != MST_F16) return dispatch_act(a.dtype, [](auto) { return 0; });
  return MST_OK;
}

extern "C" int mst_gemm_nt_form(const mst_gemm_args* args) {
  const int rc = check_gemm_nt(args);
  return rc != MST_OK ? rc : gemm_nt_form(*args);
}

extern "C" int mst_gemm_nt(const mst_gemm_args* args, mst_stream_t stream) {
  const int rc = check_gemm_nt(args);
  if (rc != MST_OK) return rc;
  const mst_gemm_args& a = *args;
  const int form = gemm_nt_form(a), variant = form & 15;
  hipStream_t s = (hipStream_t)stream;
  return dispatch_act(a.dtype, [&](auto tag) -> int {
    typedef decltype(tag) T;
    switch (form >> 4) {
      case 3: return launch_gemm_3cu<T>(a, s);
      case 2: return launch_gemm<T, 128, 128, 2, 2>(a, variant, s);
      case 1: return launch_gemm<T, 64, 64, 2, 2, 256>(a, variant, s);
      default: return launch_gemm<T, 64, 64, 2, 2>(a, variant, s);
    }
  });
}

extern "C" int mst_gemm_nt_pair(const mst_gemm_args* args0, const mst_gemm_args* args1, mst_stream_t stream) {
  return mst_gemm_nt_pair_begin(args0, args1, nullptr, stream);
}

extern "C" int mst_gemm_nt_pair_begin(const mst_gemm_args* args0, const mst_gemm_args* args1, const mst_step_begin_args* begin,
                                      mst_stream_t stream) {
  MST_CHECK_ARG(args0 != nullptr && args1 != nullptr, "mst_gemm_nt_pair: null args");
  const mst_gemm_args &a0 = *args0, &a1 = *args1;
  auto plain = [](const mst_gemm_args& a) {
    return a.a_u8 && !a.c_f32 && a.M > 0 && a.N > 0 && a.K > 0 && a.K % 8 == 0 && a.lda % 8 == 0 && a.ldb % 8 == 0 && a.ldc >= a.N &&
           a.A && a.B && a.C && (uintptr_t)a.A % 16 == 0 && (uintptr_t)a.B % 16 == 0 && (uintptr_t)a.C % 16 == 0 && !a.resid && !a.gate &&
           a.act == 0 && a.dropout_p == 0.f && !a.self_resid && ((!a.rowadd && !a.grpadd) || a.rowadd_period > 0) &&
           (!a.grpadd || a.grp_index) && gemm_fast_form<64, 64>(a) && a.K % 64 == 0 && cdiv(a.M, 64) * cdiv(a.N, 64) < (1 << 20);
  };
  if (a0.dtype != a1.dtype || !plain(a0) || !plain(a1) || (begin && begin->sh_w && begin->sh_dtype != a0.dtype)) {
    int rc = begin ? mst_step_begin(begin, stream) : MST_OK;
    if (rc == MST_OK) rc = mst_gemm_nt(args0, stream);
    return rc != MST_OK ? rc : mst_gemm_nt(args1, stream);
  }
  StepBegin sb = {};
  int n_begin = 0;
  if (begin) {
    int64_t grid = 0;
    int rc = pack_step_begin(*begin, sb, &grid);
    if (rc) return rc;
    if (begin->in_keep) {
      mst_step_begin_args own = *begin;
      own.sh_w = nullptr;
      if ((rc = mst_step_begin(&own, stream)) != MST_OK) return rc;
      StepBegin sh = {};
      sh.sh_w = sb.sh_w; sh.sh_wt16 = sb.sh_wt16; sh.sh_desc = sb.sh_desc; sh.sh_prefix = sb.sh_prefix; sh.sh_n_mat = sb.sh_n_mat; sh.sh_tiles = sb.sh_tiles;
      sb = sh;
    } else {
      n_begin = (int)((grid + 7) / 8 * 8);
    }
  }
  hipStream_t s = (hipStream_t)stream;
  return dispatch_act(a0.dtype, [&](auto tag) -> int {
    typedef decltype(tag) T;
    const int64_t sh_tiles = sb.sh_w ? sb.sh_tiles : 0;
    if (a0.K >= 1024 && a1.K >= 1024 && gemm_fast_form<128, 128>(a0) && gemm_fast_form<128, 128>(a1)) {
      const int t0 = (int)((a0.M / 128) * (a0.N / 128)), t1 = (int)((a1.M / 128) * (a1.N / 128));
      const size_t lds_b = (size_t)2 * (128 + 128) * 64 * 2;
      static size_t granted = 64 * 1024;
      if (const int rc = lds_opt_in(reinterpret_cast<const void*>(&gemm_nt_pair_kernel<T, 128, 128, 2, 2, 64, 4>), lds_b, &granted, "gemm_nt_pair_kernel")) return rc;
      hipLaunchKernelGGL((gemm_nt_pair_kernel<T, 128, 128, 2, 2, 64, 4>), dim3((unsigned)(n_begin + t0 + t1 + sh_tiles)), dim3(256), lds_b, s, a0, a1,
                         t0, t1, sb, n_begin);
      MST_CHECK_LAUNCH("gemm_nt_pair_kernel");
      return MST_OK;
    }
    const int tiles0 = (int)((a0.M / 64) * (a0.N / 64)), tiles1 = (int)((a1.M / 64) * (a1.N / 64));
    const size_t lds = (size_t)2 * (64 + 64) * 64 * 2;
    hipLaunchKernelGGL((gemm_nt_pair_kernel<T, 64, 64, 2, 2, 64, 1>), dim3((unsigned)(n_begin + tiles0 + tiles1 + sh_tiles)), dim3(256), lds, s, a0,
                       a1, tiles0, tiles1, sb, n_begin);
    MST_CHECK_LAUNCH("gemm_nt_pair_kernel");
    return MST_OK;
  });
}
```

### musicstyletransfer_amd/csrc/row_tail.hip

```cpp
#include <math.h>
#include "common.hpp"
#include "gemm_tile.hpp"
#include "shadows.hpp"

namespace mst {

#ifndef MST_TAIL_SPIN_TICKS
#define MST_TAIL_SPIN_TICKS 20000000ull
#endif

__device__ __forceinline__ void grid_sync(uint32_t* ctr, uint32_t target, uint32_t* status, uint32_t spin_bit) {
  asm volatile("s_waitcnt vmcnt(0)" ::: "memory");
  __syncthreads();
  if (threadIdx.x == 0) {
    __hip_atomic_fetch_add(ctr, 1u, __ATOMIC_RELAXED, __HIP_MEMORY_SCOPE_AGENT);
    const uint64_t t0 = __builtin_amdgcn_s_memrealtime();
    uint32_t spins = 0;
    while (__hip_atomic_load(ctr, __ATOMIC_RELAXED, __HIP_MEMORY_SCOPE_AGENT) < target) {
      __builtin_amdgcn_s_sleep(1);
      if ((++spins & 255u) == 0u) {
        if (status && __hip_atomic_load(status, __ATOMIC_RELAXED, __HIP_MEMORY_SCOPE_AGENT) != 0u) break;
        if (__builtin_amdgcn_s_memrealtime() - t0 > MST_TAIL_SPIN_TICKS) {
          if (status) __hip_atomic_fetch_or(status, spin_bit, __ATOMIC_RELAXED, __HIP_MEMORY_SCOPE_AGENT);
          break;
// ... 628 lines not shown
  uint32_t ride_seen = 0u;
  if constexpr (RIDE != 0) { if (tid == 0) load4_sc1_nowait(ride_seen, ride_queue); }

  {
    raw_t rdy[RPW], rx[RPW];
#pragma unroll
    for (int i = 0; i < RPW; ++i) {
      const int r = wave + TAIL_WAVES * i, rc = r < B ? r : B - 1;
      if constexpr (E == 4) load8_l2_nowait(rdy[i], dx1 + (int64_t)rc * q.rs_c + lane * 4);
      else load4_l2_nowait(rdy[i], dx1 + (int64_t)rc * q.rs_c + lane * 2);
      rx[i] = *reinterpret_cast<const raw_t*>(h1 + (int64_t)rc * q.rs_d + lane * E);
    }
    l2_wait(rdy);
    ln_bwd_rows(rdy, rx, q.mean1, q.rstd1, sGam + D, q.site0, dh1, q.rs_dh1, false, dh1m, q.rs_c, q.dg1, q.db1);
  }
  TAIL_STAMP(6);
  {
    f32x4 part = {0.f, 0.f, 0.f, 0.f};
#pragma unroll
    for (int ks = 0; ks < KQ1; ++ks) {
      const vec8 xf = __builtin_bit_cast(vec8, *reinterpret_cast<const u32x4*>(sA + m * LDX + 32 * (KQ1 * wq + ks) + 8 * lq));
      part = Act<T>::mfma16(wpf[ks], xf, part);
    }
    const f32x4 acc = quarter_sum(sP, part, wq, m, lq);
    if (wq == 0 && m_ok) {
      uint16_t hb[4];
#pragma unroll
      for (int e = 0; e < 4; ++e) hb[e] = f32_to_bits<T>(acc[e]);
      *reinterpret_cast<u32x2*>(datt + (int64_t)m * q.rs_datt + n2 + 4 * lq) =
          u32x2{(uint32_t)hb[0] | ((uint32_t)hb[1] << 16), (uint32_t)hb[2] | ((uint32_t)hb[3] << 16)};
    }
  }
  TAIL_STAMP(7);
  if constexpr (RIDE != 0) {
    __syncthreads();
    tail_drain<T, RIDE>(ride, ride_tiles, ride_queue, ride_seen, tail_smem, TailShadow{});
  }
}

}

using namespace mst;

#ifdef MST_TAIL_STAMPS
extern "C" int mst_debug_tail_stamps(uint32_t* host_out) {
  return hipMemcpyFromSymbol(host_out, HIP_SYMBOL(mst::g_tail_stamps), sizeof(uint32_t) * 32) == hipSuccess ? 0 : -1;
}
#endif

static int check_rider(const char* who, const mst_gemm_args& g, int dtype) {
  MST_CHECK_ARG(g.dtype == dtype && g.M > 0 && g.N > 0 && g.K > 0 && g.A && g.B && g.C, "%s: rider: bad GEMM", who);
  MST_CHECK_ARG(g.M % 128 == 0 && g.N % 128 == 0 && g.K % 64 == 0 && g.lda % 8 == 0 && g.ldb % 8 == 0 && g.ldc % 8 == 0 && g.M * (g.N / 128) < (1ll << 30),
                "%s: rider: M and N must be multiples of 128, K of 64 (got %lld, %lld, %lld)", who, (long long)g.M, (long long)g.N, (long long)g.K);
  MST_CHECK_ARG(!g.c_f32 && !g.a_u8 && !g.gate && !g.rowadd && !g.grpadd && g.act == MST_ACT_NONE && g.dropout_p == 0.f && !g.self_resid,
                "%s: rider: bias, alpha, a residual and row remaps only", who);
  MST_CHECK_ARG((g.a_rows_per_group <= 0 || g.a_rows_per_group % 128 == 0) && (g.c_rows_per_group <= 0 || g.c_rows_per_group % 128 == 0),
                "%s: rider: row-remap groups must be whole 128-row tiles", who);
  const int64_t phys_rows = g.c_rows_per_group > 0 ? (g.M / g.c_rows_per_group) * g.c_group_stride + g.c_group_offset : g.M;
  MST_CHECK_ARG((uint64_t)phys_rows * (uint64_t)g.N < (1ull << 32) && (!g.resid || (g.ldr % 8 == 0 && (uintptr_t)g.resid % 16 == 0)) &&
                ((uintptr_t)g.A | (uintptr_t)g.B | (uintptr_t)g.C) % 16 == 0 && (!g.bias || (uintptr_t)g.bias % 16 == 0),
                "%s: rider: operands must be 16-byte aligned and the output below 2^32 elements", who);
  return MST_OK;
}
static unsigned ride_grid(int64_t G, int tiles) {
  int64_t over = (((int64_t)tiles * 8 + 6) / 7 + G - 1) / G + 1;
  if (over < 9) over = 9;
  if (over > 16) over = 16;
  return (unsigned)(G * over);
}
static void ride_shape(const mst_gemm_args& g, int& tiles_signed, size_t& lds) {
  const int64_t t128 = (g.M / 128) * (g.N / 128);
  const bool big = t128 > 7 * 32 - 16 && g.M % 256 == 0 && (g.a_rows_per_group <= 0 || g.a_rows_per_group % 256 == 0) &&
                   (g.c_rows_per_group <= 0 || g.c_rows_per_group % 256 == 0);
  if (big) { tiles_signed = -(int)((g.M / 256) * (g.N / 128)); lds = (size_t)2 * (256 + 128) * 64 * 2; }
  else { tiles_signed = (int)t128; lds = (size_t)128 * (128 + 4) * 4; }
}

struct TailForm { int kernel, ride_rows, tiles; unsigned grid; size_t lds; int tickets; };
static int tail_form_common(const char* who, const char* who_ride, int dtype, int64_t D, const mst_gemm_args* rider, TailForm& f) {
  MST_CHECK_ARG(D == 128 || D == 256, "%s: width must be 128 or 256 (got %lld)", who, (long long)D);
  if (const int rc = dispatch_act(dtype, [](auto) -> int { return MST_OK; })) return rc;
  f = TailForm{D == 256 ? 0 : 1, 0, 0, (unsigned)((D / 16) * TAIL_OVERSUBSCRIBE), 0, 0};
  if (rider) {
    if (const int rc = check_rider(who_ride, *rider, dtype)) return rc;
    int tiles;
    ride_shape(*rider, tiles, f.lds);
    f.ride_rows = tiles < 0 ? 256 : 128;
    f.tiles = tiles < 0 ? -tiles : tiles;
    f.kernel += tiles < 0 ? 4 : 2;
    f.grid = ride_grid(D / 16, f.tiles);
  }
  return MST_OK;
}
static int row_tail_fwd_form(int dtype, int64_t D, const mst_gemm_args* rider, int64_t sh_tiles, TailForm& f) {
  if (const int rc = tail_form_common("mst_row_tail_fwd", "mst_row_tail_fwd_ride", dtype, D, rider, f)) return rc;
  MST_CHECK_ARG(sh_tiles == 0 || (rider && sh_tiles > 0 && sh_tiles < (1ll << 30)), "mst_row_tail_fwd_ride_shadows: shadow tiles need a rider (got %lld)",
                (long long)sh_tiles);
  f.tickets = (int)((sh_tiles + 15) / 16);
  if (f.tickets > 0 && f.lds < (size_t)16 * 32 * 33 * 4) f.lds = (size_t)16 * 32 * 33 * 4;
  return MST_OK;
}
static int row_tail_bwd_form(int dtype, int64_t D, const mst_gemm_args* rider, TailForm& f) {
  if (const int rc = tail_form_common("mst_row_tail_bwd", "mst_row_tail_bwd_ride", dtype, D, rider, f)) return rc;
  const size_t lds = (size_t)2 * 64 * ((size_t)D + 8) * 2 + (size_t)16 * 2 * D * 4 + (size_t)4 * 64 * 16 * 4 + (size_t)2 * D * 4;
  if (lds > f.lds) f.lds = lds;
  return MST_OK;
}
// ... 93 lines not shown
```

### musicstyletransfer_amd/csrc/runtime.hip

```cpp
#include <stdarg.h>
#include <string.h>
#include "common.hpp"

namespace mst {
static thread_local char g_err[512] = "";
void set_error(const char* fmt, ...) {
  va_list ap;
  va_start(ap, fmt);
  vsnprintf(g_err, sizeof(g_err), fmt, ap);
  va_end(ap);
}
}

using namespace mst;

extern "C" int mst_version(void) { return 122; }
extern "C" const char* mst_last_error(void) { return g_err; }

#define HIP_TRY(expr)                                             \
  do {                                                            \
    hipError_t e__ = (expr);                                      \
    if (e__ != hipSuccess) {                                      \
      set_error("%s: %s", #expr, hipGetErrorString(e__));         \
      return MST_ERR_LAUNCH;                                      \
    }                                                             \
  } while (0)

extern "C" int mst_graph_begin(mst_stream_t stream) {
  HIP_TRY(hipStreamBeginCapture((hipStream_t)stream, hipStreamCaptureModeThreadLocal));
  return MST_OK;
}
static hipError_t count_nodes(hipGraph_t g, int32_t* nodes_out, int32_t* kernel_nodes_out) {
  size_t n = 0;
  hipError_t e = hipGraphGetNodes(g, nullptr, &n);
  if (e != hipSuccess) return e;
  int32_t kernels = 0;
  if (n > 0 && kernel_nodes_out) {
    hipGraphNode_t* nodes = new hipGraphNode_t[n];
    e = hipGraphGetNodes(g, nodes, &n);
    for (size_t i = 0; e == hipSuccess && i < n; ++i) {
      hipGraphNodeType t;
      e = hipGraphNodeGetType(nodes[i], &t);
      kernels += (e == hipSuccess && t == hipGraphNodeTypeKernel);
    }
    delete[] nodes;
    if (e != hipSuccess) return e;
  }
  if (nodes_out) *nodes_out = (int32_t)n;
  if (kernel_nodes_out) *kernel_nodes_out = kernels;
  return hipSuccess;
}

extern "C" int mst_graph_end(mst_stream_t stream, void** graph_exec_out) {
  return mst_graph_end_counted(stream, graph_exec_out, nullptr, nullptr);
}
extern "C" int mst_graph_end_counted(mst_stream_t stream, void** graph_exec_out, int32_t* nodes_out, int32_t* kernel_nodes_out) {
  MST_CHECK_ARG(graph_exec_out != nullptr, "mst_graph_end: null output");
  hipGraph_t g = nullptr;
  HIP_TRY(hipStreamEndCapture((hipStream_t)stream, &g));
  hipError_t ec = (nodes_out || kernel_nodes_out) ? count_nodes(g, nodes_out, kernel_nodes_out) : hipSuccess;
  if (ec != hipSuccess) {
    (void)hipGraphDestroy(g);
    set_error("hipGraphGetNodes: %s", hipGetErrorString(ec));
    return MST_ERR_LAUNCH;
  }
  hipGraphExec_t ge = nullptr;
  hipError_t e = hipGraphInstantiate(&ge, g, nullptr, nullptr, 0);
  (void)hipGraphDestroy(g);
  if (e != hipSuccess) {
// ... 138 lines not shown
```

### musicstyletransfer_amd/engine.py

```python
import contextlib
import math
import os
import warnings
from collections import OrderedDict, namedtuple

import numpy as np
import torch

from . import ops as o
from ._lib import CE_MAX_WORKGROUPS, ROLL_SLOTS
from .ops import roundup


class VAEConfig:

    def __init__(self, kind, in_dim, out_dim, num_classes, latent_dim, e_model, e_layers, e_heads, d_model, d_layers,
                 d_heads, e_dropout=0.0, d_dropout=0.0, d_causal=False):
        assert kind in ("token", "pianoroll")
        assert e_model % e_heads == 0 and d_model % d_heads == 0
        self.kind = kind
        self.in_dim, self.out_dim = in_dim, out_dim
        self.num_classes, self.latent_dim = num_classes, latent_dim
        self.e_model, self.e_layers, self.e_heads = e_model, e_layers, e_heads
        self.d_model, self.d_layers, self.d_heads = d_model, d_layers, d_heads
# ... 352 lines not shown
                names.add(key)
        return names

    def as_consumed_numpy(self):
        w = self.to_numpy("w")
        w16 = self.w16.detach().float().cpu().numpy()
        for n in self.shadowed_names():
            s = self.shapes[n]
            w[n] = w16[self.offsets[n]: self.offsets[n] + int(np.prod(s))].reshape(s).copy()
        return w

    def load_ema_numpy(self, params_np=None):
        self.enable_ema()
        if params_np is None:
            self.ema.copy_(self.w)
            return
        host = np.zeros(self.n, np.float32)
        for name, shape in self.shapes.items():
            a = np.asarray(params_np[name], np.float32)
            assert tuple(a.shape) == tuple(shape), f"{name}: expected {shape}, got {a.shape}"
            host[self.offsets[name]: self.offsets[name] + a.size] = a.reshape(-1)
        self.ema.copy_(torch.from_numpy(host))

    def refresh_shadows(self):
        o.cast_to_act(self.w, self.w16)
        o.transpose_shadows(self.w, self.wt16, self.t_desc, self.t_prefix, len(self.t_specs), self.t_tiles)


class _Layer:
    pass


Dense = namedtuple("Dense", "w b t dw db")
Norm = namedtuple("Norm", "gamma beta dgamma dbeta site")
LayerParams = namedtuple("LayerParams", "kqv proj ff1 ff2 ln1 ln2 self_resid mask_mode")

Rows = namedtuple("Rows", "view c_remap ln")
ALL_ROWS = Rows(lambda buf: buf, (0, 0, 0), {})


def position0_rows(B, S):
    return Rows(lambda buf: buf.view(B, S, -1)[:, 0, :], (1, S, 0), dict(M=B, row_id_stride=S))


class Dropout(namedtuple("Dropout", "p seed_ptr site0")):

    def at(self, k):
        return dict(dropout_p=self.p, dropout_site=self.site0 + k, dropout_seed_ptr=self.seed_ptr) if self.p > 0 else {}


NO_DROPOUT = Dropout(0.0, None, 0)


def row_block_fwd(P, L, x_in, rows, drop, form, row_groups=None, tail=None, launch=True):
    D, v = P.proj.w.shape[0], rows.view
    if form == "tail":
        o.row_tail_fwd(v(L.att), v(x_in), P.proj.w, P.proj.b, P.ln1.gamma, P.ln1.beta, P.ff1.w, P.ff1.b, P.ff2.w, P.ff2.b, P.ln2.gamma,
                       P.ln2.beta, v(L.h1), v(L.x1), v(L.a), v(L.h2), v(L.x2), L.mean1, L.rstd1, L.mean2, L.rstd2, dropout_p=drop.p,
                       dropout_seed_ptr=drop.seed_ptr, site0=drop.site0, **tail)
        return L.x2
    proj = dict(N=D, K=D, bias=P.proj.b, resid=v(x_in), **drop.at(0))
    ff1 = dict(K=D, bias=P.ff1.b, act=o.ACT_RELU, **drop.at(1))
    ff2 = dict(K=4 * D, bias=P.ff2.b, **drop.at(2))
    ff2.update(dict(self_resid=True) if P.self_resid else dict(resid=v(L.x1)))
    if form == "fused":
        head = dict(att=L.att, W=P.proj.w, h1=L.h1, gamma=P.ln1.gamma, beta=P.ln1.beta, mean=L.mean1, rstd=L.rstd1, **proj)
        kw = dict(x=L.x1, W1=P.ff1.w, a_out=L.a, W2=P.ff2.w, h_out=L.h2, gamma=P.ln2.gamma, beta=P.ln2.beta, y_out=L.x2, mean=L.mean2,
                  rstd=L.rstd2, ff1=ff1, ff2=ff2, proj=head, row_groups=row_groups)
        if not launch:
            return kw
        o.ffn_ln_fwd(**kw)
        return L.x2
    o.gemm_nt(v(L.att), P.proj.w, L.h1, c_remap=rows.c_remap, **proj)
    o.layernorm_fwd(v(L.h1), P.ln1.gamma, P.ln1.beta, v(L.x1), L.mean1, L.rstd1, D=D, **rows.ln)
    o.gemm_nt(v(L.x1), P.ff1.w, L.a, c_remap=rows.c_remap, **ff1)
    o.gemm_nt(v(L.a), P.ff2.w, L.h2, c_remap=rows.c_remap, **ff2)
    o.layernorm_fwd(v(L.h2), P.ln2.gamma, P.ln2.beta, v(L.x2), L.mean2, L.rstd2, D=D, **rows.ln)
    return L.x2


def _lead_mask(P, t, drop):
    if P.mask_mode == 2:
        return dict(mask_mode=2, **drop.at(2))
    return dict(mask_mode=1, dx_masked=t.dhm, **drop.at(2)) if drop.p > 0 else {}


def no_partials(norm, parts):
    return None


def ffn_bwd_parts(L, row_groups=None):
    M = L.h1.shape[0]
    return o.gemm_nt_ln_parts(M if row_groups is None else M // row_groups[1] * row_groups[0])


def ffn_bwd_kw(P, L, t, drop, partials_buf, row_groups=None):
    dff = t.dhm if (drop.p > 0 and not P.self_resid) else t.dh
    ln1 = dict(dx_masked=t.dh1m, mask_mode=1, **drop.at(0)) if drop.p > 0 else {}
    return dict(dff=dff, W2t=P.ff2.t, dpre_out=t.dpre, gate=L.a, W1t=P.ff1.t, dx_out=t.dh1, x=L.h1, gamma=P.ln1.gamma, mean=L.mean1,
                rstd=L.rstd1, dgamma=P.ln1.dgamma, dbeta=P.ln1.dbeta, alpha=1.0 / (1.0 - drop.p) if drop.p > 0 else 1.0,
                resid=None if P.self_resid else t.dh, partials=partials_buf, row_groups=row_groups, **ln1)


def row_block_bwd(P, L, t, dy, rows, drop, form, partials, dy_done=False, row_groups=None, tail=None, launch=True, proj_dgrad=True,
                  head=None):
    D, v = P.proj.w.shape[0], rows.view
    if form == "tail":
        o.row_tail_bwd(v(dy), v(L.h2), v(L.h1), v(L.a), L.mean1, L.rstd1, L.mean2, L.rstd2, P.ln1.gamma, P.ln2.gamma, P.ff2.t, P.ff1.t,
                       P.proj.t, t.dh, t.dhm, t.dx1, t.dh1m, t.dpre, v(t.dh1), v(t.datt), P.ln1.dgamma, P.ln1.dbeta, P.ln2.dgamma,
                       P.ln2.dbeta, dropout_p=drop.p, dropout_seed_ptr=drop.seed_ptr, site0=drop.site0, **tail)
        return t.dhm, t.dh1m
    M = L.h1.shape[0]
    lead = None
    if not dy_done and form == "fused" and P.mask_mode == 1:
        lead = dict(dy=None if head is not None else dy, x=L.h2, gamma=P.ln2.gamma, mean=L.mean2, rstd=L.rstd2, dx=t.dh,
                    dgamma=P.ln2.dgamma, dbeta=P.ln2.dbeta,
                    partials=partials(P.ln2, o.gemm_nt_ln_parts(M)), **_lead_mask(P, t, drop))
    elif not dy_done:
        mask = _lead_mask(P, t, drop)
        if P.mask_mode == 2:
            mask["dropout_site"] = drop.site0 + 2
        o.layernorm_bwd(v(L.h2), P.ln2.gamma, L.mean2, L.rstd2, v(dy), t.dh, P.ln2.dgamma, P.ln2.dbeta, D=D,
                        partials=partials(P.ln2, o.layernorm_bwd_parts(M, D)), **rows.ln, **mask)
    dff = t.dhm if (drop.p > 0 and not P.self_resid) else t.dh
    resid_ff = None if P.self_resid else t.dh
    inv_keep = 1.0 / (1.0 - drop.p) if drop.p > 0 else 1.0
    ln1 = dict(dx_masked=t.dh1m, mask_mode=1, **drop.at(0)) if drop.p > 0 else {}
    if form == "fused":
        buf = partials(P.ln1, ffn_bwd_parts(L, row_groups))
        if head is not None and (lead is None or not launch):
            raise ValueError("row_block_bwd(head=) needs the one launch that starts with the leading LayerNorm backward")
        if launch:
            o.ffn_ln_bwd(lead=lead, head=head, **ffn_bwd_kw(P, L, t, drop, buf, row_groups))
        elif lead is not None:
            raise ValueError("row_block_bwd(launch=False) needs dy_done: the block that ran elsewhere has no leading LayerNorm backward")
    else:
        o.gemm_nt(dff, P.ff2.t, t.dpre, N=4 * D, K=D, gate=v(L.a), alpha=inv_keep)
        if form == "ln_fused":
            o.gemm_nt_ln_bwd(t.dpre, P.ff1.t, t.dh1, L.h1, P.ln1.gamma, L.mean1, L.rstd1, P.ln1.dgamma, P.ln1.dbeta, N=D, K=4 * D,
                             resid=resid_ff, partials=partials(P.ln1, o.gemm_nt_ln_parts(M)), **ln1)
        else:
            o.gemm_nt(t.dpre, P.ff1.t, t.dx1, N=D, K=4 * D, resid=resid_ff)
            o.layernorm_bwd(v(L.h1), P.ln1.gamma, L.mean1, L.rstd1, t.dx1, v(t.dh1), P.ln1.dgamma, P.ln1.dbeta, D=D,
                            partials=partials(P.ln1, o.layernorm_bwd_parts(M, D)), **rows.ln, **ln1)
    dproj = t.dh1m if drop.p > 0 else v(t.dh1)
    if proj_dgrad:
        o.gemm_nt(dproj, P.proj.t, t.datt, N=D, K=D, c_remap=rows.c_remap)
    return dff, dproj


def layer_wgrads(P, L, t, x_in, dff, dproj, rows):
    D, v = P.proj.w.shape[0], rows.view
    return [o.wgrad_problem(dff, v(L.a), P.ff2.dw, P.ff2.db, N=D, K=4 * D),
            o.wgrad_problem(t.dpre, v(L.x1), P.ff1.dw, P.ff1.db, N=4 * D, K=D),
            o.wgrad_problem(dproj, v(L.att), P.proj.dw, P.proj.db, N=D, K=D),
            o.wgrad_problem(t.dqkv, x_in, P.kqv.dw, P.kqv.db, N=3 * D, K=D)]


def row_tail_selfcheck(store, B=64, S=2):
    store.tail_checked = True
    cfg, dev, adt = store.cfg, store.device, store.act_dtype
    D, F = cfg.e_model, 4 * cfg.e_model
    if not (o.can_row_tail(B, D) and store.tail_fused and cfg.e_layers >= 1):
        return True
    f32 = dict(dtype=torch.float32, device=dev)
    P = store.layer("encoder", cfg.e_layers - 1)
    scratch = lambda n: n._replace(dgamma=torch.zeros(D, **f32), dbeta=torch.zeros(D, **f32))
    P = P._replace(ln1=scratch(P.ln1), ln2=scratch(P.ln2))

    def rnd(n, width, site):
        a = torch.zeros(n, width, **f32)
        o.randn(a, seed=0x7A11, site=site)
        t = torch.zeros(n, width, dtype=adt, device=dev)
        o.cast_to_act(a, t)
        return t

    z = lambda n, w: torch.zeros(n, w, dtype=adt, device=dev)
    att, xin = rnd(B * S, D, 1), rnd(B * S, D, 2)
    status = torch.zeros(2, dtype=torch.int32, device=dev)
    sync = torch.zeros(8, dtype=torch.int32, device=dev)
    rows = position0_rows(B, S)

    def fbufs():
        L = _Layer()
        L.att, L.h1, L.x1, L.a, L.h2, L.x2 = att, z(B * S, D), z(B * S, D), z(B * S, F), z(B * S, D), z(B * S, D)
        L.mean1, L.rstd1, L.mean2, L.rstd2 = (torch.zeros(B * S, **f32) for _ in range(4))
        return L

    u, f = fbufs(), fbufs()
    tail = dict(stat_stride=S, phys_stride=S, status=status[0:1])
    row_block_fwd(P, u, xin, rows, NO_DROPOUT, "launches")
    row_block_fwd(P, f, xin, rows, NO_DROPOUT, "tail", tail=dict(tail, sync=sync[0:3]))
    dy = rnd(B * S, D, 3)

    def bbufs():
        t = _Layer()
        t.dh, t.dhm, t.dx1, t.dh1m, t.dpre, t.dh1, t.datt = z(B, D), z(B, D), z(B, D), z(B, D), z(B, F), z(B * S, D), z(B * S, D)
        return t

    ub, fb = bbufs(), bbufs()
    row_block_bwd(P, u, ub, dy, rows, NO_DROPOUT, "launches", no_partials)
    row_block_bwd(P, u, fb, dy, rows, NO_DROPOUT, "tail", no_partials, tail=dict(tail, sync=sync[4:7]))
    torch.cuda.current_stream().synchronize()
    want_f, want_b = o.row_tail_barriers(D)
    sy, stv = sync.cpu().tolist(), status.cpu().tolist()
    why = []
    if stv[0]:
        why.append(f"status flags {stv[0]:#x}")
    if sy[0] != want_f or sy[4] != want_b:
        why.append(f"barrier counters {sy[0]} / {sy[4]} instead of {want_f} / {want_b}")
    ulp = 2.0 ** -7 if adt == torch.bfloat16 else 2.0 ** -10
    host = lambda t: t.float().cpu().numpy()
    for k in ("h1", "x1", "a", "h2", "x2"):
        a, b = host(rows.view(getattr(f, k))), host(rows.view(getattr(u, k)))
        if not np.all(np.abs(a - b) <= 4 * ulp * np.maximum(np.abs(b), 1.0)):
            why.append(f"forward {k}: max difference {np.abs(a - b).max():.3g}")
    for k in ("dh", "dpre", "dx1", "dh1", "datt"):
        a, b = host(getattr(fb, k)), host(getattr(ub, k))
        if not np.abs(a - b).max() <= 4 * ulp * max(float(np.abs(b).max()), 1e-6) + 1e-6:
            why.append(f"backward {k}: max difference {np.abs(a - b).max():.3g} (scale {np.abs(b).max():.3g})")
    if why:
        store.tail_fused = False
        warnings.warn("the one-launch position-0 tail failed its start-up check on this device (" + "; ".join(why) +
                      "): using the five-launch form", RuntimeWarning)
    return not why


Forms = namedtuple("Forms", "tails riders shadows fuse_bce bce_dgrad skip_row0 cls_fold ffn_e ffn_d ln_bwd_e ln_bwd_d sched dec_tail gnorm ema "
                            "attn_proj_e attn_proj_d kqv_head_e in_drop")


def roll_scores(tp, pred, pos, cells):
    nan = float("nan")
    return dict(precision=tp / pred if pred else nan, recall=tp / pos if pos else nan,
                f1=2 * tp / (pred + pos) if pred + pos else nan,
                cell_acc=(cells - pred - pos + 2 * tp) / cells if cells else nan)


def latent_scores(acc, threshold=0.01):
    acc = np.asarray(acc, np.float64)
    if acc.ndim != 3 or acc.shape[1] != 5:
        raise ValueError(f"latent_scores takes [C, 5, Z] sums, not {acc.shape}")
    nan = float("nan")
    with np.errstate(divide="ignore", invalid="ignore"):
        n_c = acc[:, 0]
        n, s_mu, s_mu2, s_s2, s_kl = acc.sum(0)
        m = s_mu / n
        var = s_mu2 / n - m * m
        kl_dims = s_kl / n
        active = var > threshold
        m_c = acc[:, 1] / n_c
        between = np.where(n_c > 0, n_c / n * (m_c - m) ** 2, 0.0).sum(0)
        eta2 = np.minimum(between / var, 1.0)
    seen = n > 0
    classes_seen = int((n_c.sum(1) > 0).sum())
    leak = float(eta2[active].max()) if active.any() and classes_seen >= 2 else nan
    return dict(active_units=int(active.sum()), kl_dims=kl_dims, kl_dim_max=float(kl_dims[seen].max()) if seen.any() else nan,
                kl_dims_used=int((kl_dims > threshold).sum()),
                sigma_rms=float(np.sqrt((s_s2[seen] / n[seen]).mean())) if seen.any() else nan, class_leak=leak)


def iw_scores(acc, cells):
    acc = np.asarray(acc, np.float64).reshape(-1)
    if acc.size != 6:
        raise ValueError(f"iw_scores takes the six sums of mst_iw_finish, not {acc.size} values")
    if not cells > 0:
        raise ValueError(f"cells per piece must be positive, not {cells!r}")
    pieces, nan = acc[4], float("nan")
    nll = -acc[0] / pieces if pieces > 0 else nan
    elbo_nll = -acc[1] / pieces if pieces > 0 else nan
    return dict(iw_nll=float(nll), iw_elbo_nll=float(elbo_nll), iw_gap=float(elbo_nll - nll),
                iw_ess=float(acc[2] / pieces) if pieces > 0 else nan, iw_bits_per_cell=float(nll / (cells * math.log(2.0))),
                iw_invalid=int(acc[5]))


def check_iw(samples):
    if isinstance(samples, bool) or not isinstance(samples, (int, np.integer)) or samples < 1:
        raise ValueError(f"iw_samples must be an integer >= 1, not {samples!r}")


def check_schedule(kl_warmup_steps=0, kl_cycle_steps=0, kl_free_bits=0.0, lr_warmup_steps=0):
    for name, val in (("kl_warmup_steps", kl_warmup_steps), ("kl_cycle_steps", kl_cycle_steps), ("lr_warmup_steps", lr_warmup_steps)):
# ... 50 lines not shown

class StepPlan:

    def __init__(self, store, B, T, lr=3e-4, clip_gradient=1.0, kl_weight=1.0, label_smoothing=0.0,
                 negative_label_downscaling=False, global_batch=None, gscale=None, want_probs=False, seed=0,
                 internal_eps=False, optimizer_params=None, sample_offset=0, site_base=0,
                 kl_warmup_steps=0, kl_cycle_steps=0, kl_free_bits=0.0, lr_warmup_steps=0, clip_global_norm=0.0, ema_decay=0.0,
                 d_input_dropout=0.0):
        cfg = store.cfg
        self.store, self.cfg, self.B, self.T = store, cfg, B, T
        self.dev, self.adt = store.device, store.act_dtype
        self.lr, self.clip, self.kl_weight = lr, clip_gradient, kl_weight
        check_schedule(kl_warmup_steps, kl_cycle_steps, kl_free_bits, lr_warmup_steps)
        self.schedule = dict(kl_warmup_steps=int(kl_warmup_steps), kl_cycle_steps=int(kl_cycle_steps), kl_free_bits=float(kl_free_bits),
                             lr_warmup_steps=int(lr_warmup_steps))
        self.scheduled = any(self.schedule.values())
        check_clip(clip_global_norm)
        self.clip_global_norm = float(clip_global_norm)
        self.grad_parts = store.grad_parts() if self.clip_global_norm > 0 else None
        check_ema(ema_decay)
        self.ema_decay = float(ema_decay)
        if self.ema_decay > 0:
            store.enable_ema()
        check_input_dropout(d_input_dropout)
        self.d_input_dropout = float(d_input_dropout)
        self._infer = self._tick_adam = False
        self.ls, self.nld = label_smoothing, negative_label_downscaling
        self.global_batch = global_batch or B
        self.sample_offset, self.site_base = int(sample_offset), int(site_base)
        if (self.sample_offset * cfg.latent_dim) % 2:
            raise ValueError("sample_offset * latent_dim must be even (eps is drawn in Box-Muller pairs)")
        self.gscale = gscale if gscale is not None else (1024.0 if self.adt == torch.float16 else 1.0)
        self.gscale_enc = 1.0
        self.want_probs, self.internal_eps = want_probs, internal_eps
        self.opt = dict(beta1=0.9, beta2=0.999, eps=1e-8, wd=0.0)
        if optimizer_params:
            for k_src, k_dst in (("beta1", "beta1"), ("beta2", "beta2"), ("epsilon", "eps"), ("wd", "wd")):
                if k_src in optimizer_params:
                    self.opt[k_dst] = float(optimizer_params[k_src])
        dev, adt = self.dev, self.adt
        De, Dd, Z = cfg.e_model, cfg.d_model, cfg.latent_dim
        Se, Sd = T, T + 1
        self.Me, self.Md = B * Se, B * Sd
        f32 = dict(dtype=torch.float32, device=dev)

        def act(rows, width):
            return torch.zeros(rows, roundup(width, 8), dtype=adt, device=dev)

        self.ride = (cfg.kind != "token" and cfg.d_layers >= 1 and cfg.e_layers >= 1 and Dd in (128, 256) and
                     o.can_ride(B * T, 3 * Dd, Dd, T) and o.can_ride(B * T, Dd, 3 * Dd, T))
        self.shadows_on_tail = True
        self.dec_tail = True
        self.kqv_head = True
        self.n_cu = torch.cuda.get_device_properties(self.dev).multi_processor_count if self.dev.type == "cuda" else 0
        self.forms = self._resolve_forms()
        if cfg.kind == "token":
            seg = [("tokens", B * T * 4), ("labels", B * T * 4)]
        else:
            self.ld_roll = roundup(cfg.in_dim + (cfg.num_classes if self.forms.cls_fold else 0), 8)
            seg = [("roll", B * T * self.ld_roll), ("labels", B * T * cfg.out_dim)]
        seg += [("seq_lens", B * 4), ("classes", B * 4)]
        self.in_layout, off = {}, 0
        for name, nbytes in seg:
            self.in_layout[name] = (off, nbytes)
            off = roundup(off + nbytes, 16)
        self.own_inbuf = torch.zeros(off, dtype=torch.uint8, device=dev)
        self.bind_inputs(self.own_inbuf)
        self.in_keep = self.roll_d = None
        if self.d_input_dropout > 0:
            self.in_keep = torch.zeros(B * T, dtype=torch.uint8, device=dev)
            if cfg.kind != "token":
                self.roll_d = torch.zeros(B * T, roundup(cfg.in_dim, 8), dtype=torch.uint8, device=dev)
        self.eps = torch.zeros(B, Z, **f32)
        self.rng_state = store.rng_state(seed)
        self._outers = []
        self._cls_job = None

        self.pos_e = torch.from_numpy(positional_table(De, Se)).to(dev)
        self.pos_d = torch.from_numpy(positional_table(Dd, Sd)).to(dev)
        self.keymask_e = torch.zeros(B, Se, dtype=torch.uint8, device=dev)
        self.keymask_d = torch.zeros(B, Sd, dtype=torch.uint8, device=dev)

        def layers(n, M, D, H, S):
            out = []
            for _ in range(n):
                L = _Layer()
                L.qkv, L.att, L.h1, L.x1 = act(M, 3 * D), act(M, D), act(M, D), act(M, D)
                L.a, L.h2, L.x2 = act(M, 4 * D), act(M, D), act(M, D)
                L.lse = torch.zeros(2, B, H, S, **f32)
                L.mean1, L.rstd1 = torch.zeros(M, **f32), torch.zeros(M, **f32)
                L.mean2, L.rstd2 = torch.zeros(M, **f32), torch.zeros(M, **f32)
                out.append(L)
            return out

        self.x0_e = act(self.Me, De)
        self.enc = layers(cfg.e_layers, self.Me, De, cfg.e_heads, Se)
        self.x0_d = act(self.Md, Dd)
        self.dec = layers(cfg.d_layers, self.Md, Dd, cfg.d_heads, Sd)
        self.mu, self.sigma, self.z = torch.zeros(B, Z, **f32), torch.zeros(B, Z, **f32), torch.zeros(B, Z, **f32)
        self.kl, self.total = torch.zeros(B, **f32), torch.zeros(B, **f32)
        nb4 = (B + 3) // 4 * 4
        self._recon_buf = torch.zeros(nb4 + 8 + 24 + 64, **f32)
        self.recon = self._recon_buf[:B]
        self.sync_words = self._recon_buf[nb4: nb4 + 8].view(torch.int32)
        self.ride_queues = self._recon_buf[nb4 + 32:].view(torch.int32)
        self.metric_acc = store.metric_acc
        self.track_token_metrics = False
        self.track_roll_metrics = False
        self.track_latent_stats = False
        self.logits =None if self.forms.fuse_bce else act(B * T, cfg.out_dim)
        self.dlogits = act(B * T, cfg.out_dim)
        if cfg.kind == "token":
            self.probs = torch.zeros(B * T, cfg.out_dim, **f32) if want_probs else None
        else:
            self.probs = act(B * T, cfg.out_dim) if want_probs else None
        self.npos = torch.zeros(B, dtype=torch.int32, device=dev)

        def bwd_bufs(M, D, H, S):
            t = _Layer()
            t.dx_a, t.dx_b = act(M, D), act(M, D)
            t.dh, t.dhm = act(M, D), act(M, D)
            t.dh1, t.dh1m = act(M, D), act(M, D)
            t.dpre, t.dx1 = act(M, 4 * D), act(M, D)
            t.datt, t.dqkv = act(M, D), act(M, 3 * D)
            t.delta = torch.zeros(B, H, S, **f32)
            return t

        self.be_l = [bwd_bufs(self.Me, De, cfg.e_heads, Se) for _ in range(cfg.e_layers)]
        self.bd_l = [bwd_bufs(self.Md, Dd, cfg.d_heads, Sd) for _ in range(cfg.d_layers)]
        self._wgrads = []
        self.wgrad_scratch = store.wgrad_scratch()
        self._ln_part, self._psums = {}, []
        for side, n_l, M, D in (("encoder", cfg.e_layers, self.Me, De), ("decoder", cfg.d_layers, self.Md, Dd)):
            rows = max(o.layernorm_bwd_parts(M, D), o.gemm_nt_ln_parts(M))
            for i in range(n_l):
                for ln in ("ln1", "ln2" if side == "encoder" else "ln3"):
                    self._ln_part[f"{side}.layer{i}.{ln}"] = torch.zeros(rows, 2 * D, **f32)
        self.lat_scratch = torch.zeros(B * (Dd + 2 * Z), **f32)
        self.d_dec_out = act(self.Md, Dd)
        self.d_enc_out = act(self.Me, De)
        c = _Layer()
        c.dh, c.dhm, c.dx1, c.dh1m = act(B, De), act(B, De), act(B, De), act(B, De)
        c.dpre = act(B, 4 * De)
        self.sp_dh1 = c.dh1 = act(self.Me, De)
        self.sp_datt = c.datt = act(self.Me, De)
        c.dqkv, c.delta = self.be_l[-1].dqkv, self.be_l[-1].delta
        self.top = c
        self.graph = None
        self.graph_late = None
        self.graph_opt = None
        self._tick_adam = False
        self._infer = False
        self._tail_used = dict(fwd=False, bwd=False)
        if o.can_row_tail(B, De) and store.tail_fused and not store.tail_checked:
            row_tail_selfcheck(store)

    @property
    def e_p(self):
        return 0.0 if self._infer else self.cfg.e_dropout

    @property
    def d_p(self):
        return 0.0 if self._infer else self.cfg.d_dropout

    def _resolve_forms(self, with_grad=False):
        cfg, st, B, T = self.cfg, self.store, self.B, self.T
        De, Dd = cfg.e_model, cfg.d_model
        roll = cfg.kind == "pianoroll"
        tails = bool(o.can_row_tail(B, De) and st.tail_fused)
        riders = bool(self.ride and tails)
        shadows = "own" if not st.shadows_deferred else ("tail" if self.shadows_on_tail and riders else "begin")
        fuse_bce = roll and o.can_fuse_bce(cfg.out_dim, T, self.nld) and o.bce_fusion_pays(cfg.out_dim)
        ffn_d, ln_bwd_d = o.ffn_fusion_pays(Dd, 4 * Dd), o.ln_bwd_fusion_pays(Dd)
        bce_dgrad = fuse_bce and ln_bwd_d
        skip_row0 = cfg.d_layers > 0 and T % 64 == 0 and ffn_d
        return Forms(
            tails=tails, riders=riders, shadows=shadows, fuse_bce=fuse_bce,
            bce_dgrad=bce_dgrad,
            skip_row0=skip_row0,
            dec_tail=bool(with_grad and not self._infer and self.dec_tail and bce_dgrad and ffn_d and skip_row0 and
                          o.dec_tail_pays(Dd, 4 * Dd, cfg.out_dim, T, B * T // 64, self.n_cu)),
            cls_fold=(roll and cfg.in_dim % 8 == 0 and roundup(cfg.in_dim + cfg.num_classes, 256) == roundup(cfg.in_dim, 256) and
                      st.offsets["encoder.class2hid.weight"] == st.offsets["encoder.embedding.weight"] + cfg.in_dim * De),
            ffn_e=o.ffn_fusion_pays(De, 4 * De), ffn_d=ffn_d, ln_bwd_e=o.ln_bwd_fusion_pays(De), ln_bwd_d=ln_bwd_d,
            sched=self.scheduled,
            gnorm=self.clip_global_norm > 0,
            ema=self.ema_decay > 0,
            attn_proj_e=self._attn_proj(T, cfg.e_heads, De), attn_proj_d=not cfg.d_causal and self._attn_proj(T + 1, cfg.d_heads, Dd),
            kqv_head_e=bool(self.kqv_head and cfg.e_layers >= 2 and o.ffn_fusion_pays(De, 4 * De) and not o.ln_bwd_fusion_pays(De) and
                            o.kqv_head_pays(self.adt, B * T, De)),
            in_drop=self.d_input_dropout > 0 and self._tick_adam and not self._infer)

    def _attn_proj(self, S, H, D):
        return bool(o.attn_bwd_form(self.adt, self.B, S, H, D // H, 0, D, 2 * D, 3 * D, D, 3 * D, proj=True)["proj"])

    def _guard(self):
        fwd, bwd = o.row_tail_barriers(self.cfg.e_model)
        exp = []
        if self._tail_used["fwd"]:
            exp.append((self.sync_words[0:1], fwd))
        if self._tail_used["bwd"]:
            exp.append((self.sync_words[4:5], bwd))
        g = dict(status=self.store.step_status, expect=exp)
        if self.global_batch == self.B:
            g["finite"] = (self.recon, self.kl)
        return g

    def bind_inputs(self, buf):
        cfg, B, T = self.cfg, self.B, self.T
        need = max(a + n for a, n in self.in_layout.values())
        if not (buf.dtype == torch.uint8 and buf.is_contiguous() and buf.is_cuda and buf.data_ptr() % 16 == 0 and buf.numel() >= need):
            raise ValueError("bind_inputs: need a contiguous, 16-byte aligned device uint8 blob of pack_batch()'s size")
        self.inbuf = buf

        def inview(name, dtype, *shape):
            a, n = self.in_layout[name]
            return buf[a: a + n].view(dtype).view(*shape)

        if cfg.kind == "token":
            self.tokens = inview("tokens", torch.int32, B, T)
            self.labels = inview("labels", torch.int32, B, T)
        else:
            self.roll_cls = inview("roll", torch.uint8, B * T, self.ld_roll)
            self.roll = self.roll_cls[:, : roundup(cfg.in_dim, 8)]
            self.labels = inview("labels", torch.uint8, B * T, cfg.out_dim)
        self.seq_lens = inview("seq_lens", torch.int32, B)
        self.classes = inview("classes", torch.int32, B)

    def load_batch(self, x, seq_lens, classes, labels, eps=None):
        def dev(a, dtype):
            t = torch.as_tensor(np.asarray(a)) if not torch.is_tensor(a) else a
            return t.to(device=self.dev, dtype=dtype, non_blocking=True)

        cfg, B, T = self.cfg, self.B, self.T
        if cfg.kind == "token":
            self.tokens.copy_(dev(x, torch.int32).view(B, T))
            self.labels.copy_(dev(labels, torch.int32).view(B, T))
        else:
            self.roll[:, : cfg.in_dim].copy_(dev(x, torch.uint8).view(B * T, cfg.in_dim))
            self.labels.copy_(dev(labels, torch.uint8).view(B * T, cfg.out_dim))
        self.seq_lens.copy_(dev(seq_lens, torch.int32))
# ... 43 lines not shown

    def _drop(self, p, site):
        return dict(dropout_p=p, dropout_site=site, dropout_seed_ptr=self.rng_state) if p > 0 else {}

    def _dropout(self, p, site0):
        return Dropout(p, self.rng_state if p > 0 else None, site0)

    def _site_e(self, i):
        return self.site_base + 3 * i

    def _site_d(self, i):
        return self.site_base + 3 * (self.cfg.e_layers + i)

    def _late_shadows(self):
        st = self.store
        return dict(w=st.w, wt16=st.wt16, desc=st.t_desc_late, prefix=st.t_prefix_late, n_mat=st.t_n_late, tiles=st.t_tiles_late)

    def _top_encoder_layer_fwd(self, i, L, x_in):
        cfg, st, B, S, F = self.cfg, self.store, self.B, self.T, self.forms
        D, H = cfg.e_model, cfg.e_heads
        P = st.layer("encoder", i)
        o.attn_qkv_fwd(x_in, P.kqv.w, P.kqv.b, L.qkv, self.keymask_e, L.lse, L.att, B, S, H, D // H, 0, D, 2 * D, q_limit=1)
        self._tail_used["fwd"] = F.tails
        tail = None
        if F.tails:
            tail = dict(sync=self.sync_words[0:3], stat_stride=S, phys_stride=S, status=st.step_status[0:1], queue=self.ride_queues[0:1])
            if F.riders:
                Pd, Dd, Sd = st.layer("decoder", 0), cfg.d_model, S + 1
                tail["rider"] = dict(A=self.x0_d, B=Pd.kqv.w, C_out=self.dec[0].qkv, M=B * S, N=3 * Dd, K=Dd, bias=Pd.kqv.b,
                                     a_remap=(S, Sd, 1), c_remap=(S, Sd, 1))
                if F.shadows == "tail":
                    tail["shadows"] = self._late_shadows()
        return row_block_fwd(P, L, x_in, position0_rows(B, S), self._dropout(self.e_p, self._site_e(i)),
                             "tail" if F.tails else "launches", tail=tail)

    def _layer_fwd(self, side, i, L, x_in, keymask, D, H, S, p, site0):
        F = self.forms
        dh = D // H
        if side == "encoder" and i == self.cfg.e_layers - 1:
            return self._top_encoder_layer_fwd(i, L, x_in)
        P = self.store.layer(side, i)
        causal = side == "decoder" and self.cfg.d_causal
        if side == "decoder" and i == 0 and F.riders:
            (o.attn_causal_fwd if causal else o.attn_fwd)(L.qkv, keymask, L.lse, L.att, self.B, S, H, dh, 0, D, 2 * D)
        elif causal:
            o.gemm_nt(x_in, P.kqv.w, L.qkv, N=3 * D, K=D, bias=P.kqv.b)
            o.attn_causal_fwd(L.qkv, keymask, L.lse, L.att, self.B, S, H, dh, 0, D, 2 * D)
        else:
            o.attn_qkv_fwd(x_in, P.kqv.w, P.kqv.b, L.qkv, keymask, L.lse, L.att, self.B, S, H, dh, 0, D, 2 * D)
        fused = F.ffn_e if side == "encoder" else F.ffn_d
        if F.dec_tail and side == "decoder" and i == self.cfg.d_layers - 1:
            return L.x2
        return row_block_fwd(P, L, x_in, ALL_ROWS, self._dropout(p, site0), "fused" if fused else "launches",
                             row_groups=self._row0_groups(side, i))

    def _row0_groups(self, side, i):
        if side == "decoder" and i == self.cfg.d_layers - 1 and self.forms.skip_row0:
            return (self.T, self.T + 1, 1)
        return None

    def forward(self, inference=False, upto=None, with_grad=False, start=None):
        if with_grad and (inference or upto or start):
            raise ValueError("forward(with_grad=True) is the forward pass of a training step")
        if start not in (None, "latent") or (start and (not inference or upto)):
            raise ValueError("forward(start=...) takes 'latent', in inference mode and without upto")
        if start and getattr(self, "enc_out", None) is None:
            raise RuntimeError("forward(start='latent') needs the encoder output of a preceding full forward(inference=True) of this plan")
        if upto not in (None, "latent") or (upto and not inference):
            raise ValueError("forward(upto=...) takes 'latent', in inference mode only")
        cfg, st, B, T = self.cfg, self.store, self.B, self.T
        self._infer = bool(inference)
        F = self.forms = self._resolve_forms(with_grad)
        self._tail_used = dict(fwd=False, bwd=False)
        De, Dd = cfg.e_model, cfg.d_model
        Se, Sd = T, T + 1
        sq_e, sq_d = math.sqrt(float(De)), math.sqrt(float(Dd))
        self._wgrads, self._psums, self._outers, self._cls_job = [], [], [], None
        need_rng = self.e_p > 0 or self.d_p > 0 or self.internal_eps or F.in_drop
        rng = st.rng_state_inference() if self._infer else self.rng_state
        tick = self._tick_adam and not self._infer
        begin = dict(rng_state=rng if need_rng else None,
                     adam_state=st.step_state if tick else None, lr=self.lr, beta1=self.opt["beta1"],
                     beta2=self.opt["beta2"], eps_out=self.eps if self.internal_eps else None,
                     eps_index0=self.sample_offset * cfg.latent_dim, lens=self.seq_lens,
                     mask_e=self.keymask_e if cfg.kind != "token" else None, add_e=0, mask_d=self.keymask_d, add_d=1,
                     zero_a=self._recon_buf, zero_b=st.g if tick else None)
        if F.shadows == "begin":
            begin["shadows"] = self._late_shadows()
        if F.sched and tick:
            begin["schedule"] = dict(block=st.sched, kl_weight=self.kl_weight, **self.schedule)
        roll_d = keep_d = None
        if F.in_drop:
            begin["input_drop"] = dict(keep=self.in_keep, p=self.d_input_dropout, index0=self.sample_offset * T)
            keep_d = self.in_keep
            if cfg.kind != "token":
                roll_d = self.roll_d
                begin["input_drop"].update(src=self.roll, dst=roll_d)
        ride = cfg.kind != "token" and not start
        if start:
            o.step_begin(rng_state=begin["rng_state"], eps_out=begin["eps_out"], eps_index0=begin["eps_index0"], zero_a=self._recon_buf)
        elif not ride:
            o.step_begin(**begin)
        if start:
            pass
        elif cfg.kind == "token":
            o.embed_fwd(self.tokens, st.p("encoder.embedding.weight"), self.pos_e, self.x0_e.view(B, Se, -1), 0, sq_e,
                        classes=self.classes, cls_table=st.p("encoder.class2hid.weight"), keymask=self.keymask_e)
# ... 54 lines not shown
                             **self._out_ln_bwd("decoder", last, self.dec[last], cfg.d_dropout, self._site_d(0) + 3 * last,
                                                self.bd_l[last], B * T))
            loss = dict(A=self.dec_out, B=self.store.h("decoder.output_layer.weight"), labels=self.labels, loss=self.recon, T=T,
                        dlogits=dl, probs=self.probs, label_smoothing=ls, downweight=nld, gscale=self.gscale, M=B * T,
                        K=cfg.d_model, bias=self.store.p("decoder.output_layer.bias"), a_remap=(T, T + 1, 1), counts=counts)
            if F.dec_tail:
                L, t, P = self.dec[last], self.bd_l[last], self.store.layer("decoder", last)
                drop, groups = self._dropout(self.d_p, self._site_d(0) + 3 * last), self._row0_groups("decoder", last)
                x_in = self.dec[last - 1].x2 if last > 0 else self.x0_d
                o.dec_tail_step(row_block_fwd(P, L, x_in, ALL_ROWS, drop, "fused", row_groups=groups, launch=False), loss, dgrad,
                                ffn_bwd_kw(P, L, t, drop, self._ln_partials_buf(P.ln1, ffn_bwd_parts(L, groups)), groups))
            else:
                o.gemm_sigmoid_bce(dgrad=dgrad, **loss)
        else:
            o.sigmoid_bce(self.logits, self.labels, self.recon, B, T, cfg.out_dim, label_smoothing=ls,
                          downweight=nld, npos=self.npos, probs=self.probs, dlogits=dl, gscale=self.gscale,
                          pre_zeroed=True, counts=counts)
        if combine:
            o.loss_combine(self.recon, self.kl, self.kl_weight, self.total, self.metric_acc, guard=self._guard())

    LN_PARTIALS_MIN = 32

    def _ln_partials_buf(self, norm, parts):
        return self._ln_part[norm.site] if parts >= self.LN_PARTIALS_MIN else None

    def _ln_partials(self, norm, parts):
        buf, dg, db = self._ln_partials_buf(norm, parts), norm.dgamma, norm.dbeta
        if buf is None:
            return None
        D = dg.numel()
        if db.data_ptr() == dg.data_ptr() + 4 * D:
            self._psums.append(o.partial_sum_job(buf, parts, dg, length=2 * D))
        else:
            self._psums += [o.partial_sum_job(buf, parts, dg, length=D), o.partial_sum_job(buf, parts, db, col_off=D, length=D)]
        return buf

    def _flush_grads(self):
        o.gemm_wgrad_batch(self._wgrads, scratch=self.wgrad_scratch, sums=self._psums, outers=self._outers, cls=self._cls_job)
        self.last_wgrad_launch = (self._wgrads, self._psums)
        self._wgrads, self._psums, self._outers, self._cls_job = [], [], [], None

    def _out_ln_bwd(self, side, i, L, p, site0, t, M):
        P = self.store.layer(side, i)
        return dict(x=L.h2, gamma=P.ln2.gamma, mean=L.mean2, rstd=L.rstd2, dgamma=P.ln2.dgamma, dbeta=P.ln2.dbeta,
                    partials=self._ln_partials(P.ln2, o.gemm_nt_ln_parts(M)), **_lead_mask(P, t, self._dropout(p, site0)))

    def _layer_bwd(self, side, i, L, x_in, dy, dx_in, keymask, D, H, S, p, site0, t, dy_done=False, next_ln=None, ride=False, head=None):
        F, P = self.forms, self.store.layer(side, i)
        ffn, ln = (F.ffn_e, F.ln_bwd_e) if side == "encoder" else (F.ffn_d, F.ln_bwd_d)
        in_loss = F.dec_tail and side == "decoder" and i == self.cfg.d_layers - 1
        proj = F.attn_proj_e if side == "encoder" else F.attn_proj_d
        dff, dproj = row_block_bwd(P, L, t, dy, ALL_ROWS, self._dropout(p, site0), "fused" if ffn else ("ln_fused" if ln else "launches"),
                                   self._ln_partials, dy_done=dy_done, row_groups=self._row0_groups(side, i), launch=not in_loss,
                                   proj_dgrad=not proj, head=head)
        if side == "decoder" and self.cfg.d_causal:
            o.attn_causal_bwd(L.qkv, keymask, L.lse, t.datt, t.dqkv, t.delta, self.B, S, H, D // H, 0, D, 2 * D)
        elif proj:
            o.attn_proj_bwd(L.qkv, keymask, L.lse, dproj, P.proj.t, t.dqkv, t.delta, self.B, S, H, D // H, 0, D, 2 * D)
        else:
            o.attn_bwd(L.qkv, keymask, L.lse, t.datt, t.dqkv, t.delta, self.B, S, H, D // H, 0, D, 2 * D)
        handed = None
        if next_ln is not None:
            kw, t_below = next_ln
            o.gemm_nt_ln_bwd(t.dqkv, P.kqv.t, t_below.dh, N=D, K=3 * D, resid=t.dh1, **kw)
        elif side == "encoder" and i > 0 and F.kqv_head_e:
            handed = dict(A=t.dqkv, B=P.kqv.t, resid=t.dh1, N=D, K=3 * D)
        elif ride:
            T_ = self.T
            handed = (dict(A=t.dqkv, B=P.kqv.t, C_out=dx_in, M=self.B * T_, N=D, K=3 * D, resid=t.dh1, resid_phys=True,
                           a_remap=(T_, T_ + 1, 1), c_remap=(T_, T_ + 1, 1)),
                      (t.dqkv.view(self.B, S, -1), P.kqv.t, t.dh1.view(self.B, S, -1)))
        else:
            o.gemm_nt(t.dqkv, P.kqv.t, dx_in, N=D, K=3 * D, resid=t.dh1)
        self._wgrads += layer_wgrads(P, L, t, x_in, dff, dproj, ALL_ROWS)
        return handed

    def _top_encoder_layer_bwd(self, i, L, x_in, dx_in, next_ln=None, rider=None):
        cfg, st, B, S, F = self.cfg, self.store, self.B, self.T, self.forms
        D, H = cfg.e_model, cfg.e_heads
        self._kqv_head = None
        P, c, rows = st.layer("encoder", i), self.top, position0_rows(B, S)
        self._tail_used["bwd"] = F.tails
        tail = None
        if F.tails:
            tail = dict(sync=self.sync_words[4:7], stat_stride=S, phys_stride=S, status=st.step_status[0:1], rider=rider,
                        queue=self.ride_queues[32:33])
        dff, dproj = row_block_bwd(P, L, c, self.d_enc_out, rows, self._dropout(cfg.e_dropout, self._site_e(i)),
                                   "tail" if F.tails else "launches", no_partials, tail=tail)
        o.attn_bwd(L.qkv, self.keymask_e, L.lse, c.datt, c.dqkv, c.delta, B, S, H, D // H, 0, D, 2 * D, q_limit=1)
        if next_ln is not None:
            kw, t_below = next_ln
            o.gemm_nt_ln_bwd(c.dqkv, P.kqv.t, t_below.dh, N=D, K=3 * D, resid=c.dh1, **kw)
        elif i > 0 and F.kqv_head_e:
            self._kqv_head = dict(A=c.dqkv, B=P.kqv.t, resid=c.dh1, N=D, K=3 * D)
        else:
            o.gemm_nt(c.dqkv, P.kqv.t, dx_in, N=D, K=3 * D, resid=c.dh1)
        self._wgrads += layer_wgrads(P, L, c, x_in, dff, dproj, rows)

    def backward(self):
        self.backward_early(flush=False)
        self.backward_late()

    def grad_cut(self):
        cfg, st = self.cfg, self.store
        if cfg.e_layers < 2:
            return 0
        return st.offsets[f"encoder.layer{cfg.e_layers - 1}.att.W_k.weight"]
# ... 269 lines not shown
```

### musicstyletransfer_amd/ops.py

```python
import ctypes as C
import math

import torch

from . import _lib
from ._lib import LnArgs, LnBwdIn, PartialSum, OuterJob, StepBeginArgs, StepMetrics, ACT_NONE, ACT_RELU, MST_BF16, MST_F16, GemmArgs, WgradArgs, call

_DT = {torch.bfloat16: MST_BF16, torch.float16: MST_F16}


def dt(x):
    try:
        return _DT[x if isinstance(x, torch.dtype) else x.dtype]
    except KeyError:
        raise TypeError(f"activation dtype must be bfloat16 or float16, got {x}") from None


def ptr(t):
    if t is None:
        return None
    assert t.is_cuda, "mst ops need device tensors (there is no CPU fallback)"
    if t.device.index != torch.cuda.current_device():
        raise RuntimeError(f"tensor on cuda:{t.device.index} but the current device is cuda:{torch.cuda.current_device()}: "
                           "call torch.cuda.set_device() for this rank's GPU first")
# ... 154 lines not shown
    q.logits, q.ldl = ptr(logits), (ld(logits) if logits is not None else 0)
    q.gscale = gscale
    q.counts = _roll_counts(counts)
    return g, q


def gemm_sigmoid_bce(A, B, labels, loss, T, dgrad=None, **kw):
    g, q = _gemm_bce_args(A, B, labels, loss, T, **kw)
    if dgrad is None:
        call("mst_gemm_sigmoid_bce", C.byref(g), C.byref(q), stream())
    else:
        g2, l = _gemm_ln_bwd_args(**dgrad)
        call("mst_gemm_sigmoid_bce_dgrad_ln", C.byref(g), C.byref(q), C.byref(g2), C.byref(l), stream())


def gemm_sigmoid_bce_form(g, q, g2=None, l=None):
    form = (C.c_int64 * 4)()
    call("mst_gemm_sigmoid_bce_form", C.byref(g), C.byref(q), C.byref(g2) if g2 is not None else None, C.byref(l) if l is not None else None,
         form)
    return dict(BN=form[0], col_tiles=form[1], launches=form[2])


def can_fuse_ln(D):
    return D in (128, 256)


def ln_bwd_fusion_pays(D):
    return D == 128


def gemm_nt_ln_fwd(A, B, H_out, gamma, beta, Y_out, mean, rstd, eps=1e-5, **kw):
    g = _gemm_args(A, B, H_out, **kw)
    l = LnArgs()
    l.mode, l.gamma, l.beta, l.eps = 1, ptr(gamma), ptr(beta), eps
    l.out, l.ld_out = ptr(Y_out), ld(Y_out)
    l.mean, l.rstd = ptr(mean), ptr(rstd)
    call("mst_gemm_nt_ln", C.byref(g), C.byref(l), stream())


def can_fuse_ffn(D, F):
    return D in (128, 256) and F % D == 0


def ffn_fusion_pays(D, F):
    return can_fuse_ffn(D, F)


def _row_groups(n_rows, row_groups):
    rpg, stride, off = row_groups
    assert n_rows % stride == 0 and rpg % 64 == 0 and off + rpg <= stride
    return (n_rows // stride) * rpg, (rpg, stride, off)


def ffn_ln_fwd(x, W1, a_out, W2, h_out, gamma, beta, y_out, mean, rstd, eps=1e-5, ff1=None, ff2=None, proj=None, row_groups=None):
    g0, l0, g1, g2, l = _ffn_ln_fwd_args(x, W1, a_out, W2, h_out, gamma, beta, y_out, mean, rstd, eps, ff1, ff2, proj, row_groups)
    if proj is None:
        call("mst_ffn_ln_fwd", C.byref(g1), C.byref(g2), C.byref(l), stream())
    else:
        call("mst_proj_ffn_ln_fwd", C.byref(g0), C.byref(l0), C.byref(g1), C.byref(g2), C.byref(l), stream())


def _ffn_ln_fwd_args(x, W1, a_out, W2, h_out, gamma, beta, y_out, mean, rstd, eps=1e-5, ff1=None, ff2=None, proj=None, row_groups=None):
    ff1, ff2 = dict(ff1 or {}), dict(ff2 or {})
    if row_groups is not None:
        M, remap = _row_groups(x.shape[0], row_groups)
        ff1.update(M=M, a_remap=remap)
        ff2.update(M=M)
        if proj is not None:
            proj = dict(proj, M=M)
    g1 = _gemm_args(x, W1, a_out, **ff1)
    g2 = _gemm_args(a_out, W2, h_out, **ff2)
    l = LnArgs()
    l.mode, l.gamma, l.beta, l.eps = 1, ptr(gamma), ptr(beta), eps
    l.out, l.ld_out = ptr(y_out), ld(y_out)
    l.mean, l.rstd = ptr(mean), ptr(rstd)
    if proj is None:
        return None, None, g1, g2, l
    kw = {k: v for k, v in proj.items() if k not in ("att", "W", "h1", "gamma", "beta", "mean", "rstd")}
    g0 = _gemm_args(proj["att"], proj["W"], proj["h1"], **kw)
    l0 = LnArgs()
    l0.mode, l0.gamma, l0.beta, l0.eps = 1, ptr(proj["gamma"]), ptr(proj["beta"]), eps
    l0.out, l0.ld_out = ptr(x), ld(x)
    l0.mean, l0.rstd = ptr(proj["mean"]), ptr(proj["rstd"])
    return g0, l0, g1, g2, l


def _ffn_ln_bwd_args(dff, W2t, dpre_out, gate, W1t, dx_out, x, gamma, mean, rstd, dgamma, dbeta, alpha=1.0, dx_masked=None, mask_mode=0,
                     partials=None, row_groups=None, **kw):
    rg = {}
    if row_groups is not None:
        M, remap = _row_groups(dff.shape[0], row_groups)
        rg, kw = dict(M=M, a_remap=remap), dict(kw, M=M)
    g1 = _gemm_args(dff, W2t, dpre_out, gate=gate, alpha=alpha, **rg)
    g2 = _gemm_args(dpre_out, W1t, dx_out, **kw)
    l = LnArgs()
    l.mode, l.gamma = 2, ptr(gamma)
    l.mean, l.rstd = ptr(mean), ptr(rstd)
    l.x, l.ld_x = ptr(x), ld(x)
    l.dgamma, l.dbeta = ptr(dgamma), ptr(dbeta)
    l.out, l.ld_out = ptr(dx_masked), (ld(dx_masked) if dx_masked is not None else 0)
    l.mask_mode = mask_mode
    l.partials = ptr(partials)
    if partials is not None:
        assert partials.shape[0] >= gemm_nt_ln_parts(g1.M) and partials.shape[1] == 2 * g2.N and partials.is_contiguous()
    return g1, g2, l


def can_dec_tail(D, F, P, T):
    return D == 128 and F == 512 and P == 128 and T > 0 and T % 64 == 0


def dec_tail_pays(D, F, P, T, tiles, n_cu=256):
    return can_dec_tail(D, F, P, T) and 0 < tiles <= n_cu


def dec_tail_step(fwd, loss, dgrad, bwd):
    g0, l0, g1, g2, l3 = _ffn_ln_fwd_args(**fwd)
    go, q = _gemm_bce_args(**loss)
    gd, l3b = _gemm_ln_bwd_args(**dgrad)
    b1, b2, l1b = _ffn_ln_bwd_args(**bwd)
    call("mst_dec_tail_step", C.byref(g0), C.byref(l0), C.byref(g1), C.byref(g2), C.byref(l3), C.byref(go), C.byref(q), C.byref(gd),
         C.byref(l3b), C.byref(b1), C.byref(b2), C.byref(l1b), stream())


def _kqv_head_args(A, B, C_out=None, **kw):
    g = _gemm_args(A, B, A if C_out is None else C_out, **kw)
    if C_out is None:
        g.C, g.ldc = None, 0
    return g


def ffn_ln_bwd_head_form(head, dff, W2t, dpre_out, gate, W1t, dx_out, row_groups=None):
    rg = {}
    if row_groups is not None:
        M, remap = _row_groups(dff.shape[0], row_groups)
        rg = dict(M=M, a_remap=remap)
    g1 = _gemm_args(dff, W2t, dpre_out, gate=gate, **rg)
    g2 = _gemm_args(dpre_out, W1t, dx_out, **({"M": rg["M"]} if rg else {}))
    form = (C.c_int64 * 1)()
    call("mst_kqv_ffn_ln_bwd_form", C.byref(_kqv_head_args(**head)), C.byref(g1), C.byref(g2), form)
    return int(form[0])


def kqv_head_pays(dtype, M, D):
    g = lambda m, n, k, lda, ldb, ldc: _plain_gemm_args(dtype, m, n, k, lda, ldb, ldc)
    head = g(M, D, 3 * D, 3 * D, 3 * D, 0)
    head.C, head.resid, head.ldr = None, 4096, D
    form = (C.c_int64 * 1)()
    call("mst_kqv_ffn_ln_bwd_form", C.byref(head), C.byref(g(M, 4 * D, D, D, D, 4 * D)), C.byref(g(M, D, 4 * D, 4 * D, 4 * D, D)), form)
    return bool(form[0])


def _plain_gemm_args(dtype, M, N, K, lda, ldb, ldc):
    g = GemmArgs()
    g.dtype, g.M, g.N, g.K, g.alpha = dt(dtype), M, N, K, 1.0
    g.A, g.lda, g.B, g.ldb, g.C, g.ldc = 4096, lda, 4096, ldb, 4096, ldc
    return g


def ffn_ln_bwd(dff, W2t, dpre_out, gate, W1t, dx_out, x, gamma, mean, rstd, dgamma, dbeta, alpha=1.0, dx_masked=None, mask_mode=0,
               partials=None, lead=None, row_groups=None, head=None, **kw):
    g1, g2, l = _ffn_ln_bwd_args(dff, W2t, dpre_out, gate, W1t, dx_out, x, gamma, mean, rstd, dgamma, dbeta, alpha, dx_masked, mask_mode,
                                 partials, row_groups, **kw)
    if lead is None:
        if head is not None:
            raise ValueError("ffn_ln_bwd(head=) computes lead's incoming gradient: it needs lead=")
        call("mst_ffn_ln_bwd", C.byref(g1), C.byref(g2), C.byref(l), stream())
        return
    q = LnBwdIn()
    dy = lead.get("dy") if head is None else head.get("C_out")
    q.dy, q.ld_dy = ptr(dy), (ld(dy) if dy is not None else 0)
    q.x, q.ld_x = ptr(lead["x"]), ld(lead["x"])
    q.gamma, q.mean, q.rstd = ptr(lead["gamma"]), ptr(lead["mean"]), ptr(lead["rstd"])
    q.dx, q.ld_dx = ptr(lead["dx"]), ld(lead["dx"])
    dxm = lead.get("dx_masked")
    q.dx_masked, q.ld_dxm = ptr(dxm), (ld(dxm) if dxm is not None else 0)
    q.dgamma, q.dbeta, q.partials = ptr(lead.get("dgamma")), ptr(lead.get("dbeta")), ptr(lead.get("partials"))
    q.mask_mode = 1 if dxm is not None else 0
    q.dropout_p, q.dropout_seed = lead.get("dropout_p", 0.0), lead.get("dropout_seed", 0)
    q.dropout_seed_ptr, q.dropout_site = ptr(lead.get("dropout_seed_ptr")), lead.get("dropout_site", 0)
    if lead.get("partials") is not None:
        assert lead["partials"].shape[0] >= gemm_nt_ln_parts(g1.M) and lead["partials"].shape[1] == 2 * g2.N
    if head is not None:
        call("mst_kqv_ffn_ln_bwd", C.byref(_kqv_head_args(**head)), C.byref(q), C.byref(g1), C.byref(g2), C.byref(l), stream())
        return
    call("mst_ffn_ln_bwd_lead", C.byref(q), C.byref(g1), C.byref(g2), C.byref(l), stream())


def gemm_nt_ln_bwd(A, B, dX_out, x, gamma, mean, rstd, dgamma, dbeta, dx_masked=None, mask_mode=0, partials=None, **kw):
    g, l = _gemm_ln_bwd_args(A, B, dX_out, x, gamma, mean, rstd, dgamma, dbeta, dx_masked, mask_mode, partials, **kw)
    call("mst_gemm_nt_ln", C.byref(g), C.byref(l), stream())


def _gemm_ln_bwd_args(A, B, dX_out, x, gamma, mean, rstd, dgamma, dbeta, dx_masked=None, mask_mode=0, partials=None, **kw):
    g = _gemm_args(A, B, dX_out, **kw)
    l = LnArgs()
    l.mode, l.gamma = 2, ptr(gamma)
    l.mean, l.rstd = ptr(mean), ptr(rstd)
    l.x, l.ld_x = ptr(x), ld(x)
    l.dgamma, l.dbeta = ptr(dgamma), ptr(dbeta)
    l.out, l.ld_out = ptr(dx_masked), (ld(dx_masked) if dx_masked is not None else 0)
    l.mask_mode = mask_mode
    l.partials = ptr(partials)
    if partials is not None:
        assert partials.shape[0] >= gemm_nt_ln_parts(g.M) and partials.shape[1] == 2 * g.N and partials.is_contiguous()
    return g, l


def gemm_nt_ln_parts(M):
    return int(_lib.load().mst_gemm_nt_ln_parts(M))


def layernorm_bwd_parts(M, D):
    return int(_lib.load().mst_layernorm_bwd_parts(M, D))


def layernorm_form(backward, dtype, M, D):
    form = (C.c_int64 * 5)()
    call("mst_layernorm_form", 1 if backward else 0, dt(dtype), M, D, form)
    return dict(nv=form[0], r=form[1], grid=form[2], waves=form[3], lds=form[4])


PARTIAL_SUM_MAX_JOBS = 20


def partial_sum_job(src, n_parts, dst, scale=1.0, col_off=0, length=None):
    j = PartialSum()
# ... 632 lines not shown
```

Before: 27.38 million frames/s.

## Store FFN ReLU gate as packed bits and keep lead dx in registers

The fused FFN forward now packs the ReLU gate (sign/nonzero of the FF1 activation) into one bit per element, written to a new per-layer uint8 buffer or kept in LDS for the decoder tail. The backward reads these bits instead of re-reading the bf16 activation as the gate, which cuts gate traffic by roughly 16x. A second change lets the leading LayerNorm backward keep its dx tile in registers and reuse it as the residual, skipping the dx global write and re-read when a masked copy exists. This adds kernel variants, an LDS bit buffer and more argument checks, and it raises register pressure.

```diff
diff --git a/include/mst_hip.h b/include/mst_hip.h
--- a/include/mst_hip.h
+++ b/include/mst_hip.h
@@ -56,6 +56,7 @@
   const uint64_t* dropout_seed_ptr;
   int32_t a_u8;
   int32_t resid_phys;
+  uint8_t* gate_bits; int64_t ldgb;
 } mst_gemm_args;
 
 int mst_gemm_nt(const mst_gemm_args* args, mst_stream_t stream);
@@ -108,6 +109,7 @@
   float* dgamma; float* dbeta; float* partials;
   int32_t mask_mode;
   float dropout_p; uint64_t dropout_seed; const uint64_t* dropout_seed_ptr; uint32_t dropout_site;
+  int32_t resid_is_dx;
 } mst_ln_bwd_in;
 int mst_ffn_ln_bwd_lead(const mst_ln_bwd_in* lead, const mst_gemm_args* ff2_dgrad, const mst_gemm_args* ff1_dgrad,
                         const mst_ln_args* ln, mst_stream_t stream);
diff --git a/musicstyletransfer_amd/csrc/common.hpp b/musicstyletransfer_amd/csrc/common.hpp
--- a/musicstyletransfer_amd/csrc/common.hpp
+++ b/musicstyletransfer_amd/csrc/common.hpp
@@ -2,6 +2,7 @@
 #include <hip/hip_runtime.h>
 #include <stdint.h>
 #include <stdio.h>
+#include <type_traits>
 #include "../../include/mst_hip.h"
 
 namespace mst {
@@ -91,6 +92,18 @@
   return b;
 }
 
+template <typename T> __device__ __forceinline__ uint32_t gate_byte(const u32x4& v) {
+  constexpr uint32_t INF = std::is_same<T, __bf16>::value ? 0x7F80u : 0x7C00u, NAN_ADD = (0x7FFFu - INF) * 0x00010001u;
+  uint32_t f[4];
+#pragma unroll
+  for (int k = 0; k < 4; ++k) {
+    const uint32_t m = v[k] & 0x7FFF7FFFu, z = m + 0x7FFF7FFFu;
+    f[k] = z & ~((m + NAN_ADD) | v[k]);
+  }
+  const uint32_t lo = __builtin_amdgcn_perm(f[1], f[0], 0x07050301u) & 0x80808080u, hi = __builtin_amdgcn_perm(f[3], f[2], 0x07050301u) & 0x80808080u;
+  return __builtin_amdgcn_udot4(hi, 0x80402010u, __builtin_amdgcn_udot4(lo, 0x08040201u, 0u, false), false) >> 7;
+}
+
 template <typename T> __device__ __forceinline__ u32x4 expand_u8x8(u32x2 raw) {
   Pack8 p;
 #pragma unroll
diff --git a/musicstyletransfer_amd/csrc/dec_tail.hip b/musicstyletransfer_amd/csrc/dec_tail.hip
--- a/musicstyletransfer_amd/csrc/dec_tail.hip
+++ b/musicstyletransfer_amd/csrc/dec_tail.hip
@@ -60,7 +60,9 @@
 
 constexpr size_t DEC_TAIL_F = 512;
 constexpr size_t DEC_TAIL_BODY_LDS = (size_t)2 * 128 * 64 * 2 + (size_t)2 * 64 * (128 + 8) * 2 + DEC_TAIL_F * 4 + (size_t)6 * 128 * 4;
-constexpr size_t DEC_TAIL_LDS = DEC_TAIL_BODY_LDS + ((size_t)128 + 3 * 128 + DEC_TAIL_F + 3 * 128) * 4;
+constexpr size_t DEC_TAIL_PAR_LDS = ((size_t)128 + 3 * 128 + DEC_TAIL_F + 3 * 128) * 4;
+constexpr size_t DEC_TAIL_BITS_LDS = (size_t)64 * DEC_TAIL_F / 8;
+constexpr size_t DEC_TAIL_LDS = DEC_TAIL_BODY_LDS + DEC_TAIL_PAR_LDS + DEC_TAIL_BITS_LDS;
 static_assert(DEC_TAIL_LDS <= (size_t)48 * 1024 + (size_t)2 * (64 + 128) * 64 * 2 + (size_t)3 * 128 * 4, "no more LDS than the loss launch takes");
 
 template <typename T, bool CNT>
@@ -74,6 +76,7 @@
   float* sBiasO = reinterpret_cast<float*>(smem + DEC_TAIL_BODY_LDS);
   float* sPar3 = sBiasO + BN;
   float* sPar4 = sPar3 + 3 * BN;
+  unsigned char* sBits = smem + DEC_TAIL_BODY_LDS + DEC_TAIL_PAR_LDS;
   const int tid = threadIdx.x;
   for (int i = tid; i < BN; i += 512) {
     sBiasO[i] = out.bias ? out.bias[i] : 0.f;
@@ -89,8 +92,8 @@
   const mst_ln_bwd_in no_lead = {};
   u32x4 rw[2][2];
   f32x4 acc[2][2];
-  ffn_ln_body<T, BN, WGM, WGN, 1, false, true, true, false, true, false>(smem, ff1, ff2, ln3, no_lead, proj, ln1, nullptr,
-                                                                         [&] { tile128_load_w<T>(out, rw); });
+  ffn_ln_body<T, BN, WGM, WGN, 1, false, true, true, false, true, false, 2>(smem, ff1, ff2, ln3, no_lead, proj, ln1, nullptr,
+                                                                            [&] { tile128_load_w<T>(out, rw); }, sBits);
   __syncthreads();
   tile128_gemm<T>(smem, sX, rw, acc);
   tile128_load_w<T>(odg, rw);
@@ -106,7 +109,7 @@
   __syncthreads();
   mst_gemm_args no_gemm = {};
   const mst_ln_args no_ln = {};
-  ffn_ln_body<T, BN, WGM, WGN, 2, false, true, false, true, false, true>(smem, f2d, f1d, ln1b, no_lead, no_gemm, no_ln, sPar4, [] {});
+  ffn_ln_body<T, BN, WGM, WGN, 2, false, true, false, true, false, true, 2>(smem, f2d, f1d, ln1b, no_lead, no_gemm, no_ln, sPar4, [] {}, sBits);
 }
 
 template <typename T, bool CNT>
@@ -146,6 +149,7 @@
                 groups(g.c_rows_per_group, g.c_group_stride, g.c_group_offset) &&
                 groups(d2.a_rows_per_group, d2.a_group_stride, d2.a_group_offset) && g.a_rows_per_group <= 0,
                 "%s: row groups must be (T, T + 1, 1) on all three parts", who);
+  MST_CHECK_ARG(!ff1->gate_bits && !d2.gate_bits, "%s: the gate bits stay on chip here: gate_bits must be NULL", who);
   MST_CHECK_ARG(ln3_bwd->mode == 2 && ln3_bwd->mask_mode == 2, "%s: the LayerNorm-3 backward takes mask mode 2 (got %d)", who, (int)ln3_bwd->mask_mode);
   MST_CHECK_ARG(o.A == ln3->out && o.lda == ln3->ld_out, "%s: the output layer's A operand must be LayerNorm-3's output", who);
   MST_CHECK_ARG(o.C && g.A == o.C && g.lda == o.ldc, "%s: the output dgrad's A operand must be the logit gradient", who);
diff --git a/musicstyletransfer_amd/csrc/ffn_ln.hip b/musicstyletransfer_amd/csrc/ffn_ln.hip
--- a/musicstyletransfer_amd/csrc/ffn_ln.hip
+++ b/musicstyletransfer_amd/csrc/ffn_ln.hip
@@ -3,11 +3,11 @@
 
 namespace mst {
 
-template <typename T, int BN, int WGM, int WGN, int MODE, bool LEAD, bool FULL, bool EXTRA = false>
+template <typename T, int BN, int WGM, int WGN, int MODE, bool LEAD, bool FULL, bool EXTRA = false, int GB = 0>
 __global__ __launch_bounds__(WGM * WGN * 64) void ffn_ln_kernel(mst_gemm_args g1, mst_gemm_args g2, mst_ln_args ln, mst_ln_bwd_in lead,
                                                                 mst_gemm_args gx, mst_ln_args lnx) {
   extern __shared__ __attribute__((aligned(16))) unsigned char smem[];
-  ffn_ln_body<T, BN, WGM, WGN, MODE, LEAD, FULL, EXTRA>(smem, g1, g2, ln, lead, gx, lnx, nullptr, [] {});
+  ffn_ln_body<T, BN, WGM, WGN, MODE, LEAD, FULL, EXTRA, false, false, false, GB>(smem, g1, g2, ln, lead, gx, lnx, nullptr, [] {});
 }
 
 template <typename T, int BN>
@@ -15,18 +15,25 @@
                          const mst_gemm_args* gx = nullptr, const mst_ln_args* lnx = nullptr) {
   constexpr int BM = 64;
   const int ex = gx ? 1 : 0;
-  const size_t lds_loop = (size_t)2 * BN * 64 * 2 + (size_t)2 * BM * (BN + 8) * 2 + (size_t)g1.N * 4 + (size_t)6 * BN * 4;
+  const size_t lds_loop = (size_t)2 * BN * 64 * 2 + (size_t)2 * BM * (BN + 8) * 2 + (size_t)g1.N * 4 + (size_t)6 * BN * 4 +
+                          (g1.gate_bits && ln.mode == 1 ? (size_t)BM * g1.N / 8 : 0);
   const size_t lds_epi = (size_t)BM * (BN + 4) * 4;
   const size_t lds = lds_loop > lds_epi ? lds_loop : lds_epi;
   const int full = g1.M % BM == 0 ? 1 : 0;
-  const int mi = ex ? (ln.mode == 2 ? 8 : 6) + full : (lead ? 2 : (ln.mode == 2 ? 1 : 0)) * 2 + full;
+  const int mi = (ex ? (ln.mode == 2 ? 8 : 6) + full : (lead ? 2 : (ln.mode == 2 ? 1 : 0)) * 2 + full) + (g1.gate_bits ? 10 : 0);
   typedef void (*kern_t)(mst_gemm_args, mst_gemm_args, mst_ln_args, mst_ln_bwd_in, mst_gemm_args, mst_ln_args);
-  const kern_t fns[10] = {&ffn_ln_kernel<T, BN, 2, 4, 1, false, false>, &ffn_ln_kernel<T, BN, 2, 4, 1, false, true>,
+  const kern_t fns[20] = {&ffn_ln_kernel<T, BN, 2, 4, 1, false, false>, &ffn_ln_kernel<T, BN, 2, 4, 1, false, true>,
                          &ffn_ln_kernel<T, BN, 2, 4, 2, false, false>, &ffn_ln_kernel<T, BN, 2, 4, 2, false, true>,
                          &ffn_ln_kernel<T, BN, 2, 4, 2, true, false>, &ffn_ln_kernel<T, BN, 2, 4, 2, true, true>,
                          &ffn_ln_kernel<T, BN, 2, 4, 1, false, false, true>, &ffn_ln_kernel<T, BN, 2, 4, 1, false, true, true>,
-                          &ffn_ln_kernel<T, BN, 2, 4, 2, true, false, true>, &ffn_ln_kernel<T, BN, 2, 4, 2, true, true, true>};
-  static size_t granted[10] = {64 * 1024, 64 * 1024, 64 * 1024, 64 * 1024, 64 * 1024, 64 * 1024, 64 * 1024, 64 * 1024, 64 * 1024, 64 * 1024};
+                         &ffn_ln_kernel<T, BN, 2, 4, 2, true, false, true>, &ffn_ln_kernel<T, BN, 2, 4, 2, true, true, true>,
+                         &ffn_ln_kernel<T, BN, 2, 4, 1, false, false, false, 1>, &ffn_ln_kernel<T, BN, 2, 4, 1, false, true, false, 1>,
+                         &ffn_ln_kernel<T, BN, 2, 4, 2, false, false, false, 1>, &ffn_ln_kernel<T, BN, 2, 4, 2, false, true, false, 1>,
+                         &ffn_ln_kernel<T, BN, 2, 4, 2, true, false, false, 1>, &ffn_ln_kernel<T, BN, 2, 4, 2, true, true, false, 1>,
+                         &ffn_ln_kernel<T, BN, 2, 4, 1, false, false, true, 1>, &ffn_ln_kernel<T, BN, 2, 4, 1, false, true, true, 1>,
+                         &ffn_ln_kernel<T, BN, 2, 4, 2, true, false, true, 1>, &ffn_ln_kernel<T, BN, 2, 4, 2, true, true, true, 1>};
+  static size_t granted[20] = {64 * 1024, 64 * 1024, 64 * 1024, 64 * 1024, 64 * 1024, 64 * 1024, 64 * 1024, 64 * 1024, 64 * 1024, 64 * 1024,
+                               64 * 1024, 64 * 1024, 64 * 1024, 64 * 1024, 64 * 1024, 64 * 1024, 64 * 1024, 64 * 1024, 64 * 1024, 64 * 1024};
   if (const int rc = lds_opt_in(reinterpret_cast<const void*>(fns[mi]), lds, &granted[mi], "ffn_ln_kernel")) return rc;
   const mst_ln_bwd_in none = {};
   const mst_gemm_args no_gemm = {};
@@ -43,10 +50,12 @@
   const mst_gemm_args& a = *first;
   const mst_gemm_args& b = *second;
   const mst_ln_args& l = *ln;
-  int rc = check_gemm_common(a);
+  int rc = check_gemm_common(a, true);
   if (rc) return rc;
   rc = check_gemm_common(b);
   if (rc) return rc;
+  MST_CHECK_ARG(!a.gate_bits || (a.ldgb >= a.N / 8 && a.ldgb % 16 == 0 && (uintptr_t)a.gate_bits % 16 == 0),
+                "%s: gate_bits holds a row's N / 8 bytes in 16-byte pieces (ldgb %lld, N %lld)", who, (long long)a.ldgb, (long long)a.N);
   MST_CHECK_ARG(a.dtype == b.dtype && a.M == b.M, "%s: the two GEMMs must share dtype and M", who);
   MST_CHECK_ARG((b.N == 256 || b.N == 128) && a.K == b.N, "%s: the model width (first K = second N) must be 128 or 256 (got %lld, %lld)", who,
                 (long long)a.K, (long long)b.N);
@@ -82,9 +91,12 @@
     const mst_ln_bwd_in& q = *lead;
     MST_CHECK_ARG(mode == 2, "%s: a leading LayerNorm belongs to the backward form", who);
     const bool dy_on_chip = extra != nullptr;
-    MST_CHECK_ARG((q.dy || dy_on_chip) && q.x && q.gamma && q.mean && q.rstd && q.dx && (q.partials || (q.dgamma && q.dbeta)),
+    MST_CHECK_ARG((q.dy || dy_on_chip) && q.x && q.gamma && q.mean && q.rstd && (q.dx || q.resid_is_dx) && (q.partials || (q.dgamma && q.dbeta)),
                   "%s: leading LayerNorm: null pointer", who);
-    MST_CHECK_ARG((dy_on_chip || (q.ld_dy % 8 == 0 && q.ld_dy >= b.N)) && q.ld_x % 8 == 0 && q.ld_dx % 8 == 0 && q.ld_x >= b.N && q.ld_dx >= b.N &&
+    MST_CHECK_ARG(!q.resid_is_dx || (a.gate_bits && a.M % 64 == 0 && !b.self_resid && (b.resid ? (b.resid == q.dx && b.ldr == q.ld_dx) : true) &&
+                                     (q.dx || q.mask_mode == 1)),
+                  "%s: leading LayerNorm: resid_is_dx needs gate_bits, whole 64-row tiles, a residual that is NULL or dx itself, and (dx NULL) the masked copy", who);
+    MST_CHECK_ARG((dy_on_chip || (q.ld_dy % 8 == 0 && q.ld_dy >= b.N)) && q.ld_x % 8 == 0 && q.ld_x >= b.N && (!q.dx || (q.ld_dx % 8 == 0 && q.ld_dx >= b.N)) &&
                   ((uintptr_t)q.dy | (uintptr_t)q.x | (uintptr_t)q.dx | (uintptr_t)q.partials) % 16 == 0, "%s: leading LayerNorm: bad layout", who);
     MST_CHECK_ARG(q.mask_mode == 0 || (q.mask_mode == 1 && q.dx_masked && q.ld_dxm % 8 == 0 && q.ld_dxm >= b.N && (uintptr_t)q.dx_masked % 16 == 0),
                   "%s: leading LayerNorm: mask_mode must be 0 or 1 (with dx_masked)", who);
@@ -145,7 +157,7 @@
 static int kqv_head_form(const mst_gemm_args& x, const mst_gemm_args& a, const mst_gemm_args& b) {
   const bool shape = (b.N == 256 || b.N == 128) && x.N == b.N && x.K == 3 * b.N && x.M == a.M && x.dtype == a.dtype;
   const bool plain = !x.c_f32 && !x.a_u8 && !x.bias && !x.gate && !x.rowadd && !x.grpadd && x.act == MST_ACT_NONE && x.alpha == 1.f &&
-                     x.dropout_p == 0.f && !x.self_resid && x.a_rows_per_group <= 0 && x.c_rows_per_group <= 0 && a.a_rows_per_group <= 0;
+                     x.dropout_p == 0.f && !x.self_resid && !x.gate_bits && x.a_rows_per_group <= 0 && x.c_rows_per_group <= 0 && a.a_rows_per_group <= 0;
   const bool layout = x.resid && ((uintptr_t)x.A | (uintptr_t)x.B | (uintptr_t)x.resid | (uintptr_t)x.C) % 16 == 0 && x.lda % 8 == 0 &&
                       x.lda >= x.K && x.ldb % 8 == 0 && x.ldb >= x.K && x.ldr % 8 == 0 && x.ldr >= x.N &&
                       (!x.C || (x.ldc % 8 == 0 && x.ldc >= x.N)) && (uint64_t)x.N * (uint64_t)x.ldb < (1ull << 32);
diff --git a/musicstyletransfer_amd/csrc/ffn_ln.hpp b/musicstyletransfer_amd/csrc/ffn_ln.hpp
--- a/musicstyletransfer_amd/csrc/ffn_ln.hpp
+++ b/musicstyletransfer_amd/csrc/ffn_ln.hpp
@@ -5,10 +5,11 @@
 namespace mst {
 
 template <typename T, int BN, int WGM, int WGN, int MODE, bool LEAD, bool FULL, bool EXTRA, bool X_IN_LDS = false, bool KEEP_OUT = false,
-          bool PAR_READY = false, typename Hook>
+          bool PAR_READY = false, int GB = 0, typename Hook>
 __device__ __forceinline__ void ffn_ln_body(unsigned char* smem, mst_gemm_args g1, mst_gemm_args g2, const mst_ln_args ln,
                                             const mst_ln_bwd_in lead, mst_gemm_args gx, const mst_ln_args lnx, float* par,
-                                            Hook&& before_epilogue) {
+                                            Hook&& before_epilogue, unsigned char* lds_bits = nullptr) {
+  constexpr bool RRES = LEAD && GB == 1 && FULL;
   constexpr bool HEAD = EXTRA, FHEAD = EXTRA && MODE == 1, BHEAD = EXTRA && MODE == 2;
   static_assert(!(X_IN_LDS && (LEAD || EXTRA)), "a tile left in LDS is the block's own input");
   static_assert(!BHEAD || LEAD, "the backward form's head computes the gradient tile of the leading LayerNorm backward");
@@ -26,6 +27,7 @@
   T* sX = sH + BM * LDA;
   float* sBias1 = PAR_READY ? par : reinterpret_cast<float*>(sX + BM * LDA);
   float* sPar = sBias1 + g1.N;
+  unsigned char* sBits = GB == 2 ? lds_bits : reinterpret_cast<unsigned char*>(sPar + 6 * BN);
   const int tid = threadIdx.x, lane = tid & 63, wave = tid >> 6;
   const int wm = wave / WGN, wn = wave % WGN, frow = lane & 15, fq = lane >> 4;
   int64_t m0 = xcd_chunk(blockIdx.x, gridDim.x) * BM;
@@ -125,6 +127,7 @@
   u32x4 dyv[L_ITERS], xv[L_ITERS];
   float mean_r[L_ITERS], rstd_r[L_ITERS];
   u32x4 ha2[L_ITERS], hres[L_ITERS];
+  u32x4 dxr[RRES ? L_ITERS : 1];
   auto lead_loads = [&] {
     constexpr int RSTEP = L_RSTEP, ITERS = L_ITERS;
     const int nc = lnc, row0 = lrow0;
@@ -196,8 +199,9 @@
         ob.h[e] = f32_to_bits<T>(o);
         mb.h[e] = f32_to_bits<T>(o * k);
       }
+      if constexpr (RRES) dxr[it] = ob.u;
       if (m < Mg) {
-        *reinterpret_cast<u32x4*>(reinterpret_cast<T*>(lead.dx) + m * lead.ld_dx + nc) = ob.u;
+        if (!RRES || lead.dx) *reinterpret_cast<u32x4*>(reinterpret_cast<T*>(lead.dx) + m * lead.ld_dx + nc) = ob.u;
         if (lead.mask_mode == 1) *reinterpret_cast<u32x4*>(reinterpret_cast<T*>(lead.dx_masked) + m * lead.ld_dxm + nc) = mb.u;
       }
       *reinterpret_cast<u32x4*>(sX + row * LDA + nc) = (m < Mg) ? (lead.mask_mode == 1 ? mb.u : ob.u) : u32x4{0u, 0u, 0u, 0u};
@@ -370,8 +374,17 @@
 #pragma unroll
       for (int i = 0; i < TM; ++i) acc1[j][i] = f32x4{0.f, 0.f, 0.f, 0.f};
     constexpr int OUT_CH = BM * (BN / 8) / NT;
-    u32x4 gv[OUT_CH];
-    if constexpr (MODE == 2) {
+    u32x4 gv[GB == 0 ? OUT_CH : 1];
+    uint32_t gb[OUT_CH];
+    if constexpr (MODE == 2 && GB == 1) {
+      const uint8_t* Gb = g1.gate_bits;
+#pragma unroll
+      for (int i = 0; i < OUT_CH; ++i) {
+        const int cc = tid + i * NT, row = cc / (BN / 8), ch = cc % (BN / 8);
+        gb[i] = 0u;
+        if (m0 + row < Mg) gb[i] = Gb[(m0 + row) * g1.ldgb + pc * (BN / 8) + ch];
+      }
+    } else if constexpr (MODE == 2 && GB == 0) {
       const T* G = reinterpret_cast<const T*>(g1.gate);
 #pragma unroll
       for (int i = 0; i < OUT_CH; ++i) {
@@ -442,16 +455,42 @@
         FFN_STAMP(8 + (c * SPC + s) * 4 + 3);
         if constexpr (s == KST - 1) {
           constexpr int CPR = BN / 8;
+          if constexpr (MODE == 1 && GB != 0) {
+            u32x4 pv4[OUT_CH];
+#pragma unroll
+            for (int i = 0; i < OUT_CH; ++i) {
+              const int cc = tid + i * NT, row = cc / CPR, ch = cc % CPR;
+              pv4[i] = *reinterpret_cast<const u32x4*>(sH + row * LDA + ch * 8);
+            }
+#pragma unroll
+            for (int i = 0; i < OUT_CH; ++i) {
+              const int cc = tid + i * NT, row = cc / CPR, ch = cc % CPR;
+              sBits[row * (int)(F >> 3) + pc * (BN / 8) + ch] = (unsigned char)gate_byte<T>(pv4[i]);
+            }
+#pragma unroll
+            for (int i = 0; i < OUT_CH; ++i) {
+              const int cc = tid + i * NT, row = cc / CPR, ch = cc % CPR;
+              if (m0 + row < Mg) *reinterpret_cast<u32x4*>(Aout + (m0 + row) * g1.ldc + (int64_t)pc * BN + ch * 8) = pv4[i];
+            }
+          } else
 #pragma unroll
           for (int i = 0; i < BM * CPR / NT; ++i) {
             const int cc = tid + i * NT, row = cc / CPR, ch = cc % CPR;
             u32x4 v = *reinterpret_cast<const u32x4*>(sH + row * LDA + ch * 8);
             if constexpr (MODE == 2) {
               Pack8 pv, pg;
-              pv.u = v; pg.u = gv[i];
-#pragma unroll
-              for (int e = 0; e < 8; ++e)
-                if (!(bits_to_f32<T>(pg.h[e]) > 0.f)) pv.h[e] = 0;
+              pv.u = v;
+              if constexpr (GB == 0) {
+                pg.u = gv[i];
+#pragma unroll
+                for (int e = 0; e < 8; ++e)
+                  if (!(bits_to_f32<T>(pg.h[e]) > 0.f)) pv.h[e] = 0;
+              } else {
+                const uint32_t b8 = GB == 2 ? (uint32_t)sBits[row * (int)(F >> 3) + pc * (BN / 8) + ch] : gb[i];
+#pragma unroll
+                for (int e = 0; e < 8; ++e)
+                  if (!((b8 >> e) & 1u)) pv.h[e] = 0;
+              }
               v = pv.u;
               *reinterpret_cast<u32x4*>(sH + row * LDA + ch * 8) = v;
             }
@@ -467,11 +506,19 @@
     stage(std::integral_constant<int, 4>()); stage(std::integral_constant<int, 5>());
     stage(std::integral_constant<int, 6>()); stage(std::integral_constant<int, 7>());
   }
+  if constexpr (MODE == 1 && GB == 1) {
+    const int ppr = (int)(F >> 7);
+    for (int i = tid; i < BM * ppr; i += NT) {
+      const int row = i / ppr, pch = i % ppr;
+      if (m0 + row < Mg)
+        *reinterpret_cast<u32x4*>(g1.gate_bits + (m0 + row) * g1.ldgb + pch * 16) = *reinterpret_cast<const u32x4*>(sBits + row * (int)(F >> 3) + pch * 16);
+    }
+  }
   const bool resid_is_x = g2.resid == g1.A && g2.ldr == g1.lda;
   FFN_STAMP(2);
   before_epilogue();
   gemm_epilogue_ln<T, BM, BN, WGM, WGN, MODE>(g2, ln, smem, acc2, m0, resid_is_x ? sX : nullptr, LDA, KEEP_OUT ? sX : nullptr, KEEP_OUT ? LDA : 0,
-                                              sPar, &seed2);
+                                              sPar, &seed2, RRES ? dxr : nullptr, RRES && lead.resid_is_dx != 0);
   FFN_STAMP(3); FFN_RT(191);
 }
 
diff --git a/musicstyletransfer_amd/csrc/gemm_bce.hip b/musicstyletransfer_amd/csrc/gemm_bce.hip
--- a/musicstyletransfer_amd/csrc/gemm_bce.hip
+++ b/musicstyletransfer_amd/csrc/gemm_bce.hip
@@ -61,7 +61,7 @@
   MST_CHECK_ARG(a.N <= 256 || !q.downweight, "mst_gemm_sigmoid_bce: the label down-weighting counts a sample's positives in every workgroup — rows wider than "
                 "one tile (256) take mst_gemm_nt + mst_sigmoid_bce");
   MST_CHECK_ARG(q.T > 0 && q.T % 64 == 0 && a.M % q.T == 0, "mst_gemm_sigmoid_bce: T must be a multiple of 64 and divide M (a tile holds one sample's rows)");
-  MST_CHECK_ARG(!a.c_f32 && !a.resid && !a.gate && !a.rowadd && !a.grpadd && a.act == MST_ACT_NONE && a.dropout_p == 0.f && !a.self_resid &&
+  MST_CHECK_ARG(!a.c_f32 && !a.resid && !a.gate && !a.gate_bits && !a.rowadd && !a.grpadd && a.act == MST_ACT_NONE && a.dropout_p == 0.f && !a.self_resid &&
                 a.c_rows_per_group <= 0 && !a.a_u8, "mst_gemm_sigmoid_bce: only bias, alpha and an A row remap are supported");
   MST_CHECK_ARG(q.labels && q.loss && (uintptr_t)q.labels % 8 == 0, "mst_gemm_sigmoid_bce: labels / loss missing or labels not 8-byte aligned");
   MST_CHECK_ARG(!a.C || (a.ldc % 8 == 0 && a.ldc >= a.N && (uintptr_t)a.C % 16 == 0), "mst_gemm_sigmoid_bce: bad dlogits layout");
diff --git a/musicstyletransfer_amd/csrc/gemm_checks.hpp b/musicstyletransfer_amd/csrc/gemm_checks.hpp
--- a/musicstyletransfer_amd/csrc/gemm_checks.hpp
+++ b/musicstyletransfer_amd/csrc/gemm_checks.hpp
@@ -3,7 +3,7 @@
 
 namespace mst {
 
-int check_gemm_common(const mst_gemm_args& a);
+int check_gemm_common(const mst_gemm_args& a, bool gate_bits_ok = false);
 int check_gemm_ln(const mst_gemm_args& a, const mst_ln_args& l);
 int check_gemm_bce(const mst_gemm_args& a, const mst_bce_args& q);
 int check_ffn_ln(const char* who, const mst_gemm_args* first, const mst_gemm_args* second, const mst_ln_args* ln, int mode,
diff --git a/musicstyletransfer_amd/csrc/gemm_ln.hpp b/musicstyletransfer_amd/csrc/gemm_ln.hpp
--- a/musicstyletransfer_amd/csrc/gemm_ln.hpp
+++ b/musicstyletransfer_amd/csrc/gemm_ln.hpp
@@ -22,7 +22,8 @@
                                                  f32x4 (&acc)[(BN / WGN) / 16][(BM / WGM) / 16], int64_t m0,
                                                  const T* lds_resid = nullptr, int lds_resid_ld = 0,
                                                  T* lds_out = nullptr, int lds_out_ld = 0, const float* lds_par = nullptr,
-                                                 const uint64_t* dseed_pre = nullptr ) {
+                                                 const uint64_t* dseed_pre = nullptr ,
+                                                 const u32x4* reg_resid = nullptr, bool use_reg_resid = false) {
   constexpr int NT = WGM * WGN * 64;
   constexpr int WTM = BM / WGM, WTN = BN / WGN;
   constexpr int TM = WTM / 16, TN = WTN / 16;
@@ -76,7 +77,8 @@
     rv[it] = u32x4{0u, 0u, 0u, 0u}; xv[it] = rv[it]; mean_r[it] = 0.f; rstd_r[it] = 0.f;
     if (m < a.M) {
       const int64_t pm = phys_row(m);
-      if (lds_resid) rv[it] = *reinterpret_cast<const u32x4*>(lds_resid + (row0 + it * RSTEP) * lds_resid_ld + nc);
+      if (reg_resid && use_reg_resid) rv[it] = reg_resid[it];
+      else if (lds_resid) rv[it] = *reinterpret_cast<const u32x4*>(lds_resid + (row0 + it * RSTEP) * lds_resid_ld + nc);
       else if (resid) rv[it] = *reinterpret_cast<const u32x4*>(resid + m * a.ldr + nc);
       if (MODE == 2) {
         xv[it] = *reinterpret_cast<const u32x4*>(reinterpret_cast<const T*>(l.x) + pm * l.ld_x + nc);
@@ -110,7 +112,7 @@
           t[4 + e] = a.self_resid ? t[4 + e] + u1[e] : u1[e];
         }
       }
-      if (resid || lds_resid) {
+      if (resid || lds_resid || (reg_resid && use_reg_resid)) {
         Pack8 p8; p8.u = rv[it];
 #pragma unroll
         for (int e = 0; e < 8; ++e) t[e] += bits_to_f32<T>(p8.h[e]);
diff --git a/musicstyletransfer_amd/csrc/gemm_nt.hip b/musicstyletransfer_amd/csrc/gemm_nt.hip
--- a/musicstyletransfer_amd/csrc/gemm_nt.hip
+++ b/musicstyletransfer_amd/csrc/gemm_nt.hip
@@ -115,7 +115,8 @@
   return MST_OK;
 }
 
-int check_gemm_common(const mst_gemm_args& a) {
+int check_gemm_common(const mst_gemm_args& a, bool gate_bits_ok) {
+  MST_CHECK_ARG(gate_bits_ok || !a.gate_bits, "mst_gemm_nt: gate_bits belongs to the feed-forward block's launches (mst_ffn_ln_fwd / _bwd and their heads)");
   MST_CHECK_ARG(a.M > 0 && a.N > 0 && a.K > 0, "mst_gemm_nt: M,N,K must be positive (got %lld,%lld,%lld)",
                 (long long)a.M, (long long)a.N, (long long)a.K);
   MST_CHECK_ARG(a.K % 8 == 0 && a.lda % 8 == 0 && a.ldb % 8 == 0,
@@ -144,6 +145,7 @@
   MST_CHECK_ARG(a.A && a.B && a.C, "mst_gemm_nt: null operand");
   MST_CHECK_ARG(!a.resid || (a.ldr % 4 == 0 && a.ldr >= a.N), "mst_gemm_nt: ldr must be a multiple of 4 and >= N");
   MST_CHECK_ARG(!a.gate || (a.ldg % 4 == 0 && a.ldg >= a.N), "mst_gemm_nt: ldg must be a multiple of 4 and >= N");
+  MST_CHECK_ARG(!a.gate_bits, "mst_gemm_nt: gate_bits belongs to the feed-forward block's launches (mst_ffn_ln_fwd / _bwd and their heads)");
   MST_CHECK_ARG((!a.rowadd && !a.grpadd) || a.rowadd_period > 0, "mst_gemm_nt: rowadd_period must be > 0");
   MST_CHECK_ARG(!a.grpadd || a.grp_index, "mst_gemm_nt: grpadd needs grp_index");
   MST_CHECK_ARG(a.dropout_p >= 0.f && a.dropout_p < 1.f, "mst_gemm_nt: dropout_p must be in [0,1)");
@@ -188,7 +190,7 @@
   const mst_gemm_args &a0 = *args0, &a1 = *args1;
   auto plain = [](const mst_gemm_args& a) {
     return a.a_u8 && !a.c_f32 && a.M > 0 && a.N > 0 && a.K > 0 && a.K % 8 == 0 && a.lda % 8 == 0 && a.ldb % 8 == 0 && a.ldc >= a.N &&
-           a.A && a.B && a.C && (uintptr_t)a.A % 16 == 0 && (uintptr_t)a.B % 16 == 0 && (uintptr_t)a.C % 16 == 0 && !a.resid && !a.gate &&
+           a.A && a.B && a.C && (uintptr_t)a.A % 16 == 0 && (uintptr_t)a.B % 16 == 0 && (uintptr_t)a.C % 16 == 0 && !a.resid && !a.gate && !a.gate_bits &&
            a.act == 0 && a.dropout_p == 0.f && !a.self_resid && ((!a.rowadd && !a.grpadd) || a.rowadd_period > 0) &&
            (!a.grpadd || a.grp_index) && gemm_fast_form<64, 64>(a) && a.K % 64 == 0 && cdiv(a.M, 64) * cdiv(a.N, 64) < (1 << 20);
   };
diff --git a/musicstyletransfer_amd/csrc/row_tail.hip b/musicstyletransfer_amd/csrc/row_tail.hip
--- a/musicstyletransfer_amd/csrc/row_tail.hip
+++ b/musicstyletransfer_amd/csrc/row_tail.hip
@@ -704,7 +704,7 @@
   MST_CHECK_ARG(g.dtype == dtype && g.M > 0 && g.N > 0 && g.K > 0 && g.A && g.B && g.C, "%s: rider: bad GEMM", who);
   MST_CHECK_ARG(g.M % 128 == 0 && g.N % 128 == 0 && g.K % 64 == 0 && g.lda % 8 == 0 && g.ldb % 8 == 0 && g.ldc % 8 == 0 && g.M * (g.N / 128) < (1ll << 30),
                 "%s: rider: M and N must be multiples of 128, K of 64 (got %lld, %lld, %lld)", who, (long long)g.M, (long long)g.N, (long long)g.K);
-  MST_CHECK_ARG(!g.c_f32 && !g.a_u8 && !g.gate && !g.rowadd && !g.grpadd && g.act == MST_ACT_NONE && g.dropout_p == 0.f && !g.self_resid,
+  MST_CHECK_ARG(!g.c_f32 && !g.a_u8 && !g.gate && !g.gate_bits && !g.rowadd && !g.grpadd && g.act == MST_ACT_NONE && g.dropout_p == 0.f && !g.self_resid,
                 "%s: rider: bias, alpha, a residual and row remaps only", who);
   MST_CHECK_ARG((g.a_rows_per_group <= 0 || g.a_rows_per_group % 128 == 0) && (g.c_rows_per_group <= 0 || g.c_rows_per_group % 128 == 0),
                 "%s: rider: row-remap groups must be whole 128-row tiles", who);
diff --git a/musicstyletransfer_amd/csrc/runtime.hip b/musicstyletransfer_amd/csrc/runtime.hip
--- a/musicstyletransfer_amd/csrc/runtime.hip
+++ b/musicstyletransfer_amd/csrc/runtime.hip
@@ -14,7 +14,7 @@
 
 using namespace mst;
 
-extern "C" int mst_version(void) { return 122; }
+extern "C" int mst_version(void) { return 123; }
 extern "C" const char* mst_last_error(void) { return g_err; }
 
 #define HIP_TRY(expr)                                             \
diff --git a/musicstyletransfer_amd/engine.py b/musicstyletransfer_amd/engine.py
--- a/musicstyletransfer_amd/engine.py
+++ b/musicstyletransfer_amd/engine.py
@@ -428,7 +428,7 @@
 NO_DROPOUT = Dropout(0.0, None, 0)
 
 
-def row_block_fwd(P, L, x_in, rows, drop, form, row_groups=None, tail=None, launch=True):
+def row_block_fwd(P, L, x_in, rows, drop, form, row_groups=None, tail=None, launch=True, gate_bits=None):
     D, v = P.proj.w.shape[0], rows.view
     if form == "tail":
         o.row_tail_fwd(v(L.att), v(x_in), P.proj.w, P.proj.b, P.ln1.gamma, P.ln1.beta, P.ff1.w, P.ff1.b, P.ff2.w, P.ff2.b, P.ln2.gamma,
@@ -445,7 +445,7 @@
                   rstd=L.rstd2, ff1=ff1, ff2=ff2, proj=head, row_groups=row_groups)
         if not launch:
             return kw
-        o.ffn_ln_fwd(**kw)
+        o.ffn_ln_fwd(gate_bits=gate_bits, **kw)
         return L.x2
     o.gemm_nt(v(L.att), P.proj.w, L.h1, c_remap=rows.c_remap, **proj)
     o.layernorm_fwd(v(L.h1), P.ln1.gamma, P.ln1.beta, v(L.x1), L.mean1, L.rstd1, D=D, **rows.ln)
@@ -479,7 +479,7 @@
 
 
 def row_block_bwd(P, L, t, dy, rows, drop, form, partials, dy_done=False, row_groups=None, tail=None, launch=True, proj_dgrad=True,
-                  head=None):
+                  head=None, gate_bits=None, lead_dx_regs=False):
     D, v = P.proj.w.shape[0], rows.view
     if form == "tail":
         o.row_tail_bwd(v(dy), v(L.h2), v(L.h1), v(L.a), L.mean1, L.rstd1, L.mean2, L.rstd2, P.ln1.gamma, P.ln2.gamma, P.ff2.t, P.ff1.t,
@@ -507,7 +507,12 @@
         if head is not None and (lead is None or not launch):
             raise ValueError("row_block_bwd(head=) needs the one launch that starts with the leading LayerNorm backward")
         if launch:
-            o.ffn_ln_bwd(lead=lead, head=head, **ffn_bwd_kw(P, L, t, drop, buf, row_groups))
+            kw = ffn_bwd_kw(P, L, t, drop, buf, row_groups)
+            if lead_dx_regs and lead is not None and gate_bits is not None and kw["resid"] is t.dh and o.ffn_bwd_rows(M, row_groups) % 64 == 0:
+                lead["resid_is_dx"] = True
+                if lead.get("dx_masked") is not None:
+                    lead["dx"], kw["resid"] = None, None
+            o.ffn_ln_bwd(lead=lead, head=head, gate_bits=gate_bits, **kw)
         elif lead is not None:
             raise ValueError("row_block_bwd(launch=False) needs dy_done: the block that ran elsewhere has no leading LayerNorm backward")
     else:
@@ -603,7 +608,7 @@
 
 
 Forms = namedtuple("Forms", "tails riders shadows fuse_bce bce_dgrad skip_row0 cls_fold ffn_e ffn_d ln_bwd_e ln_bwd_d sched dec_tail gnorm ema "
-                            "attn_proj_e attn_proj_d kqv_head_e in_drop")
+                            "attn_proj_e attn_proj_d kqv_head_e gate_bits lead_dx_regs in_drop")
 
 
 def roll_scores(tp, pred, pos, cells):
@@ -760,6 +765,8 @@
         self.shadows_on_tail = True
         self.dec_tail = True
         self.kqv_head = True
+        self.gate_bits = True
+        self.lead_dx_regs = True
         self.n_cu = torch.cuda.get_device_properties(self.dev).multi_processor_count if self.dev.type == "cuda" else 0
         self.forms = self._resolve_forms()
         if cfg.kind == "token":
@@ -795,6 +802,7 @@
                 L = _Layer()
                 L.qkv, L.att, L.h1, L.x1 = act(M, 3 * D), act(M, D), act(M, D), act(M, D)
                 L.a, L.h2, L.x2 = act(M, 4 * D), act(M, D), act(M, D)
+                L.gbits = torch.zeros(M, 4 * D // 8, dtype=torch.uint8, device=dev) if o.ffn_fusion_pays(D, 4 * D) else None
                 L.lse = torch.zeros(2, B, H, S, **f32)
                 L.mean1, L.rstd1 = torch.zeros(M, **f32), torch.zeros(M, **f32)
                 L.mean2, L.rstd2 = torch.zeros(M, **f32), torch.zeros(M, **f32)
@@ -895,6 +903,8 @@
             gnorm=self.clip_global_norm > 0,
             ema=self.ema_decay > 0,
             attn_proj_e=self._attn_proj(T, cfg.e_heads, De), attn_proj_d=not cfg.d_causal and self._attn_proj(T + 1, cfg.d_heads, Dd),
+            gate_bits=bool(with_grad and not self._infer and self.gate_bits),
+            lead_dx_regs=bool(with_grad and not self._infer and self.gate_bits and self.lead_dx_regs),
             kqv_head_e=bool(self.kqv_head and cfg.e_layers >= 2 and o.ffn_fusion_pays(De, 4 * De) and not o.ln_bwd_fusion_pays(De) and
                             o.kqv_head_pays(self.adt, B * T, De)),
             in_drop=self.d_input_dropout > 0 and self._tick_adam and not self._infer)
@@ -1044,7 +1054,7 @@
         if F.dec_tail and side == "decoder" and i == self.cfg.d_layers - 1:
             return L.x2
         return row_block_fwd(P, L, x_in, ALL_ROWS, self._dropout(p, site0), "fused" if fused else "launches",
-                             row_groups=self._row0_groups(side, i))
+                             row_groups=self._row0_groups(side, i), gate_bits=L.gbits if fused and F.gate_bits else None)
 
     def _row0_groups(self, side, i):
         if side == "decoder" and i == self.cfg.d_layers - 1 and self.forms.skip_row0:
@@ -1205,7 +1215,8 @@
         proj = F.attn_proj_e if side == "encoder" else F.attn_proj_d
         dff, dproj = row_block_bwd(P, L, t, dy, ALL_ROWS, self._dropout(p, site0), "fused" if ffn else ("ln_fused" if ln else "launches"),
                                    self._ln_partials, dy_done=dy_done, row_groups=self._row0_groups(side, i), launch=not in_loss,
-                                   proj_dgrad=not proj, head=head)
+                                   proj_dgrad=not proj, head=head, gate_bits=L.gbits if ffn and F.gate_bits and not in_loss else None,
+                                   lead_dx_regs=F.lead_dx_regs)
         if side == "decoder" and self.cfg.d_causal:
             o.attn_causal_bwd(L.qkv, keymask, L.lse, t.datt, t.dqkv, t.delta, self.B, S, H, D // H, 0, D, 2 * D)
         elif proj:
diff --git a/musicstyletransfer_amd/ops.py b/musicstyletransfer_amd/ops.py
--- a/musicstyletransfer_amd/ops.py
+++ b/musicstyletransfer_amd/ops.py
@@ -230,8 +230,21 @@
     return (n_rows // stride) * rpg, (rpg, stride, off)
 
 
-def ffn_ln_fwd(x, W1, a_out, W2, h_out, gamma, beta, y_out, mean, rstd, eps=1e-5, ff1=None, ff2=None, proj=None, row_groups=None):
+def _gate_bits(g, gate_bits):
+    if gate_bits is not None:
+        assert gate_bits.dtype == torch.uint8 and gate_bits.dim() == 2 and gate_bits.stride(1) == 1 and gate_bits.shape[1] * 8 >= g.N
+        assert gate_bits.stride(0) % 16 == 0, "rows of gate bits are stored in 16-byte pieces"
+        g.gate_bits, g.ldgb = ptr(gate_bits), gate_bits.stride(0)
+
+
+def ffn_bwd_rows(n_rows, row_groups=None):
+    return n_rows if row_groups is None else _row_groups(n_rows, row_groups)[0]
+
+
+def ffn_ln_fwd(x, W1, a_out, W2, h_out, gamma, beta, y_out, mean, rstd, eps=1e-5, ff1=None, ff2=None, proj=None, row_groups=None,
+               gate_bits=None):
     g0, l0, g1, g2, l = _ffn_ln_fwd_args(x, W1, a_out, W2, h_out, gamma, beta, y_out, mean, rstd, eps, ff1, ff2, proj, row_groups)
+    _gate_bits(g1, gate_bits)
     if proj is None:
         call("mst_ffn_ln_fwd", C.byref(g1), C.byref(g2), C.byref(l), stream())
     else:
@@ -337,9 +350,10 @@
 
 
 def ffn_ln_bwd(dff, W2t, dpre_out, gate, W1t, dx_out, x, gamma, mean, rstd, dgamma, dbeta, alpha=1.0, dx_masked=None, mask_mode=0,
-               partials=None, lead=None, row_groups=None, head=None, **kw):
+               partials=None, lead=None, row_groups=None, head=None, gate_bits=None, **kw):
     g1, g2, l = _ffn_ln_bwd_args(dff, W2t, dpre_out, gate, W1t, dx_out, x, gamma, mean, rstd, dgamma, dbeta, alpha, dx_masked, mask_mode,
                                  partials, row_groups, **kw)
+    _gate_bits(g1, gate_bits)
     if lead is None:
         if head is not None:
             raise ValueError("ffn_ln_bwd(head=) computes lead's incoming gradient: it needs lead=")
@@ -350,7 +364,9 @@
     q.dy, q.ld_dy = ptr(dy), (ld(dy) if dy is not None else 0)
     q.x, q.ld_x = ptr(lead["x"]), ld(lead["x"])
     q.gamma, q.mean, q.rstd = ptr(lead["gamma"]), ptr(lead["mean"]), ptr(lead["rstd"])
-    q.dx, q.ld_dx = ptr(lead["dx"]), ld(lead["dx"])
+    dx = lead.get("dx")
+    q.dx, q.ld_dx = ptr(dx), (ld(dx) if dx is not None else 0)
+    q.resid_is_dx = 1 if lead.get("resid_is_dx") else 0
     dxm = lead.get("dx_masked")
     q.dx_masked, q.ld_dxm = ptr(dxm), (ld(dxm) if dxm is not None else 0)
     q.dgamma, q.dbeta, q.partials = ptr(lead.get("dgamma")), ptr(lead.get("dbeta")), ptr(lead.get("partials"))
```

Result: no change. 27.43 million frames/s (median of 4 runs) (+0.2%).
